# DecaYale/RNNPose

Hardware: AMD Instinct MI355X
Metric: pose-refine iters/sec (640x480, B=8, 3x8 recurrent) (higher is better)
Workload: dtype f32 (convolutions and volume build: fp16x3-split MFMA, fp32-class accuracy; LM: f64)

## Files before the change

include/rnnpose_hip.h:

```cpp
#ifndef RNNPOSE_HIP_H
#define RNNPOSE_HIP_H

#include <stddef.h>
#include <stdint.h>

#ifdef __cplusplus
extern "C" {
#endif

typedef void* rnnpose_stream_t;

#define RNNPOSE_ABI_VERSION 4
#define RNNPOSE_MAX_LEVELS 4

int rnnpose_abi_version(void);
const char* rnnpose_last_error(void);
int rnnpose_device_info(int dev, char* h_name, int name_len, int* h_cus);

int rnnpose_corr_pyramid_layout(int B, int h, int w, int levels, int64_t* h_offsets ,
                                int* h_hl , int* h_wl );
int rnnpose_corr_pyramid_f32(const float* fmap1, const float* fmap2, int B, int C, int h, int w,
                             int levels, float* pyramid, rnnpose_stream_t stream);
size_t rnnpose_corr_pyramid_f16x3_workspace_bytes(int B, int C, int h, int w);
int rnnpose_corr_pyramid_f16x3(const float* fmap1, const float* fmap2, int layout, int B, int C, int h, int w, int levels,
// ... 47 lines not shown
int rnnpose_lm_step_f32(const float* target, int target_mode, const float* weight, const float* depth,
                        float depth_eps, const float* K, float* G, int B, int H, int W, int num_iters,
                        double ep_lambda, double lm_lambda, double max_update, void* workspace,
                        size_t workspace_bytes, double* Hm, double* bv, float* xi, int* info,
                        rnnpose_stream_t stream);
int rnnpose_lm_step_io_f32(const float* target, int target_mode, const float* weight, const float* depth,
                           float depth_eps, const float* K, const float* G_in, float* G_out, int B, int H, int W,
                           int num_iters, double ep_lambda, double lm_lambda, double max_update, void* workspace,
                           size_t workspace_bytes, double* Hm, double* bv, float* xi, int* info,
                           rnnpose_stream_t stream);
int rnnpose_lm_normal_eq_rgbd_f64(const float* target, int target_mode, const float* weight, const float* depth,
                                  float depth_eps, const float* K, const float* G, int B, int H, int W,
                                  const float* obs_depth, const int* src_index, const float* theta, const float* K_obs,
                                  int S, int Ho, int Wo, float depth_weight, float depth_gate, float edge_tol,
                                  void* workspace, size_t workspace_bytes, double* Hm, double* bv, double* dstats,
                                  rnnpose_stream_t stream);
int rnnpose_lm_step_rgbd_io_f32(const float* target, int target_mode, const float* weight, const float* depth,
                                float depth_eps, const float* K, const float* G_in, float* G_out, int B, int H, int W,
                                int num_iters, double ep_lambda, double lm_lambda, double max_update,
                                const float* obs_depth, const int* src_index, const float* theta, const float* K_obs,
                                int S, int Ho, int Wo, float depth_weight, float depth_gate, float edge_tol,
                                void* workspace, size_t workspace_bytes, double* Hm, double* bv, float* xi, int* info,
                                double* dstats, rnnpose_stream_t stream);
int rnnpose_lm_step_views_io_f32(const float* target, int target_mode, const float* weight, const float* depth,
                                 float depth_eps, const float* K, const float* G_in, float* G_out, int B, int H, int W,
                                 int num_iters, double ep_lambda, double lm_lambda, double max_update,
                                 const float* obs_depth, const int* src_index, const float* theta, const float* K_obs,
                                 int S, int Ho, int Wo, float depth_weight, float depth_gate, float edge_tol,
                                 const int* group_start, int n_groups, const float* E,
                                 void* workspace, size_t workspace_bytes, double* Hm, double* bv, double* Hg, double* bg,
                                 float* xi, int* info, double* dstats, rnnpose_stream_t stream);
int rnnpose_lm_fused_tail(int enable);

int rnnpose_se3_exp_f32(const float* xi, int B, float* out, rnnpose_stream_t stream);
int rnnpose_se3_compose_f32(const float* A, const float* Bm, int B, float* out, rnnpose_stream_t stream);
int rnnpose_se3_inverse_f32(const float* A, int B, float* out, rnnpose_stream_t stream);
int rnnpose_se3_outer_update_f32(const float* Tij, const float* Ti, int B, int literal, float* Ti_out, float* Tij_out, rnnpose_stream_t stream);

int rnnpose_gru_gate_f32(const float* zr, const float* hcat, int B, int C, int Ctot, int hw, float* z_out,
                         float* rhx, rnnpose_stream_t stream);
int rnnpose_gru_update_f32(const float* z, const float* q_pre, const float* hcat, int B, int C, int Ctot_in,
                           int hw, float* hout, int Ctot_out, rnnpose_stream_t stream);

typedef struct {
  const float* ptr;
  int c_stride, c_offset, c_count;
} rnnpose_conv_src_t;

typedef struct {
  rnnpose_conv_src_t src[4];
  int n_src;
  int B, H, W;
  int kh, kw;
  int stride;
  const void* w_packed;
  const float* bias;
  int c_out;
  float a_scale, w_scale;
  int epilogue;
  float* dst;
  int dst_c_stride, dst_c_offset;
  const float* aux0;
  int aux0_c_stride, aux0_c_offset;
  const float* aux1;
  int aux1_c_stride, aux1_c_offset;
  float* dst2;
  int dst2_c_stride, dst2_c_offset;
  int gru_c;
  double* tile_stats;
  const float* add_map;
  int add_c_stride, add_c_offset;
  const float* src0_mean_rstd;
  int src_hl;
  int dst_hl;
  int dst2_hl;
  float* dst_split;
  int dst_split_c_stride, dst_split_c_offset;
  int src_bounded;
  int tile;
  void* ksplit_ws;
  size_t ksplit_ws_bytes;
  int single_product;
  int tile_stats_records;
} rnnpose_conv_desc_t;

size_t rnnpose_conv_ksplit_workspace_bytes(void);
int rnnpose_conv_ksplit(int enable);
int rnnpose_conv_ksplit_limits(int max_tiles, int max_splits);

int rnnpose_conv_tiles_per_image_desc(const rnnpose_conv_desc_t* h_desc);
int rnnpose_conv_products_desc(const rnnpose_conv_desc_t* h_desc);
int rnnpose_conv_spatial_tiles(int enable);
int rnnpose_conv_strip(int mode);
long long rnnpose_conv_packed_halfs(int c_out, int kh, int kw, const int* h_seg_counts, int n_seg);
int rnnpose_conv_pack_weights_f16x3(const float* w_oihw, int c_out, int c_in, int kh, int kw, const int* h_seg_counts,
                                    int n_seg, float w_scale, void* w_packed, rnnpose_stream_t stream);
int rnnpose_conv2d_nhwc_f16x3(const rnnpose_conv_desc_t* h_desc, rnnpose_stream_t stream);

int rnnpose_f16x3_saturation_check(int enable);
int rnnpose_f16x3_saturation_count(unsigned long long* h_count, int reset, rnnpose_stream_t stream);
int rnnpose_f16x3_saturation_peek(unsigned long long* d_count, rnnpose_stream_t stream);

long long rnnpose_stem_packed_halfs(void);
int rnnpose_stem_workgroups(int max_workgroups);
int rnnpose_stem_pack_weights_f16x3(const float* w_oihw, float w_scale, void* w_hi, void* w_lo, rnnpose_stream_t stream);
int rnnpose_stem_tiles(int H, int W, int* h_tiles_per_image, int* h_exact);
int rnnpose_stem_conv7x7_s2_f16x3(const float* img_nchw, int N, int H, int W, int normalize, const void* w_hi,
                                  const void* w_lo, const float* bias, float a_scale, float w_scale, float* out_nhwc,
                                  double* tile_stats, rnnpose_stream_t stream);

int rnnpose_corr_lookup_nhwc_f32(const float* pyramid, const float* coords, int B, int h, int w, int levels, int radius,
                                 float* out, rnnpose_stream_t stream);
int rnnpose_corr_lookup_nhwc_part_f32(const float* pyramid, const float* coords, int B, int b0, int b1, int h, int w,
                                      int levels, int radius, float* out, rnnpose_stream_t stream);
int rnnpose_corr_lookup_induced_nhwc_part_f32(const float* pyramid, const float* depth, const float* K, const float* G, int H, int W,
                                              float eps, int B, int b0, int b1, int h, int w, int levels, int radius, float* coords_out,
                                              float* out, rnnpose_stream_t stream);
int rnnpose_nchw_to_nhwc_f32(const float* src, int B, int C, int HW, float* dst, int dst_c_stride, int dst_c_offset,
                             rnnpose_stream_t stream);
int rnnpose_nhwc_to_nchw_f32(const float* src, int B, int C, int HW, int src_c_stride, int src_c_offset, float* dst,
                             rnnpose_stream_t stream);
int rnnpose_flow_prep_f32(const float* coords1, int subtract_grid, int B, int h, int w, float* flow4, float* motion,
                          int motion_c_stride, int motion_c_offset, rnnpose_stream_t stream);
int rnnpose_flow_conv7x7_relu_f32(const float* flow4, const float* w_t, const float* bias, int B, int h, int w, int c_out,
                                  float* out, int out_c_stride, int out_c_offset, rnnpose_stream_t stream);
int rnnpose_flow_features_f32(const float* coords1, int subtract_grid, const float* w_t, const float* bias, int B, int h, int w,
                              int c_out, float* out, int out_c_stride, int out_c_offset, float* motion, int motion_c_stride,
                              int motion_c_offset, int out_split, int motion_split, float a_scale, rnnpose_stream_t stream);
int rnnpose_flow_features_induced_f32(const float* depth, const float* K, const float* G, int H, int W, float eps, const float* w_t,
                                      const float* bias, int B, int h, int w, int c_out, float* out, int out_c_stride, int out_c_offset,
                                      float* motion, int motion_c_stride, int motion_c_offset, int out_split, int motion_split,
                                      float a_scale, rnnpose_stream_t stream);
int rnnpose_split_hl_f32(const float* src, int src_c_stride, int src_c_offset, long long n_pixels, int c_count, float a_scale,
                         float* dst, int dst_c_stride, int dst_c_offset, rnnpose_stream_t stream);
int rnnpose_flow_head_out_f32(const float* x, int x_c_stride, int x_c_offset, int c_in, const float* w_oihw,
                              const float* bias, const float* coords1, int B, int h, int w, float* delta,
                              float* coords1_out, float* flow_lr, rnnpose_stream_t stream);
int rnnpose_convex_upsample_nhwc_f32(const float* flow_lr, const float* mask, int B, int h, int w, float* flow_up,
                                     rnnpose_stream_t stream);
int rnnpose_maxpool2x2_nhwc_f32(const float* src, int B, int H, int W, int src_c_stride, int src_c_offset, int C, float* dst,
                                int dst_c_stride, int dst_c_offset, rnnpose_stream_t stream);
int rnnpose_upsample2x_bilinear_nhwc_f32(const float* src, int B, int h, int w, int src_c_stride, int src_c_offset, int C,
                                         const float* mean_rstd, int relu, float* dst, int dst_c_stride, int dst_c_offset,
                                         rnnpose_stream_t stream);
int rnnpose_pixel_head_nhwc_f32(const float* src, int B, int HW, int src_c_stride, int src_c_offset, int c_in,
                                const float* mean_rstd, int relu, const float* weight, const float* bias, int c_out, int mode,
                                float* dst_nchw, rnnpose_stream_t stream);
int rnnpose_point_row_sum_f32(const float* x, int n, int c, long long ldx, float* out, rnnpose_stream_t stream);
int rnnpose_kpconv_aggregate_f32(const float* q_pts, int n_q, const float* s_pts, int n_s, const int* neighbors, int width,
                                 const float* kernel_points, int K, float extent, const float* x, int c_in, long long ldx,
                                 const float* row_sum, float* wf, rnnpose_stream_t stream);
int rnnpose_point_linear_f32(const float* a, int n, int k, long long lda, const float* w, int m, const float* bias, float* out,
                             long long ldo, rnnpose_stream_t stream);
long long rnnpose_point_norm_workspace_bytes(int n, int c);
int rnnpose_point_norm_stats_f32(const float* x, int n, int c, long long ldx, float eps, void* workspace, long long workspace_bytes,
                                 float* mean_rstd, rnnpose_stream_t stream);
int rnnpose_point_norm_apply_f32(const float* x, int n, int c, long long ldx, const float* mean_rstd, const float* res, long long ldr,
                                 const float* res_mean_rstd, int leaky, float slope, float* out, long long ldo,
                                 rnnpose_stream_t stream);
int rnnpose_point_maxpool_f32(const float* x, int n_s, int c, long long ldx, const int* idx, int n_q, int width, float* out,
                              long long ldo, rnnpose_stream_t stream);
int rnnpose_point_gather_rows_f32(const float* x, int n_s, int c, long long ldx, const int* idx, int n_q, int idx_ld, float* out,
                                  long long ldo, rnnpose_stream_t stream);
int rnnpose_point_l2_normalize_f32(const float* x, int n, int c, long long ldx, float* out, long long ldo, rnnpose_stream_t stream);
int rnnpose_grid_voxel_keys_f32(const float* points, int n, float ox, float oy, float oz, float dl, long long nx, long long ny,
                                long long* keys, rnnpose_stream_t stream);
int rnnpose_radius_count_f32(const float* queries, int n_q, const float* supports, const int* q_start, const int* s_start,
                             int n_clouds, float radius, int* counts, rnnpose_stream_t stream);
int rnnpose_radius_neighbors_f32(const float* queries, int n_q, const float* supports, const int* q_start, const int* s_start,
                                 int n_clouds, float radius, const long long* offsets, int* cand_idx, float* cand_d2, int width,
                                 int* out, rnnpose_stream_t stream);
size_t rnnpose_conv1x1_resident_packed_bytes(int c_in);
int rnnpose_conv1x1_resident_pack_f16x3(const float* weight, int c_out, int c_in, float w_scale, void* packed,
                                        rnnpose_stream_t stream);
int rnnpose_conv1x1_resident_f16x3(const float* x, int x_c_stride, int x_c_offset, int c_in, const void* w_packed,
                                   const float* bias, float a_scale, float w_scale, int relu, long long n_pixels, float* dst,
                                   int dst_c_stride, int dst_c_offset, int dst_split, rnnpose_stream_t stream);
int rnnpose_corr_lookup_convc1_f16x3(const float* pyramid, const float* coords, int B, int b0, int b1, int h, int w, int levels,
                                     int radius, const void* w_packed, const float* bias, float a_scale, float w_scale, int relu,
                                     float* dst, int dst_c_stride, int dst_c_offset, int dst_split, rnnpose_stream_t stream);
size_t rnnpose_mask_upsample_packed_bytes(void);
int rnnpose_mask_upsample_pack_f16x3(const float* weight, float post_scale, float w_scale, void* packed, rnnpose_stream_t stream);
int rnnpose_mask_upsample_f16x3(const float* x, int x_c_stride, int x_c_offset, const void* w_packed, int c_out,
                                const float* bias, float a_scale, float w_scale, const float* flow_lr, int B, int h, int w,
                                float* flow_up, rnnpose_stream_t stream);

size_t rnnpose_instnorm_workspace_bytes(int B, int HW, int C);
int rnnpose_instnorm_nhwc_f32(const float* x, int B, int HW, int C, float eps, int relu, const float* residual,
                              void* workspace, size_t workspace_bytes, float* mean_rstd, float* out,
                              rnnpose_stream_t stream);
int rnnpose_instnorm_tiles_nhwc_f32(const float* x, int B, int HW, int C, float eps, int relu, const float* residual,
                                    const float* residual_mean_rstd, int residual_relu, const double* tile_stats,
                                    int tiles_per_image, float* mean_rstd, float* out,
                                    rnnpose_stream_t stream);

int rnnpose_nn_search_f32(const float* ref_pts, const float* que_pts, int* idxs, int b, int pn1, int pn2, int dim,
                          int exclude_self, rnnpose_stream_t stream);
void findNearestPointIdxLauncher(float* ref_pts, float* que_pts, int* idxs, int b, int pn1, int pn2, int dim,
                                 int exclude_self);

size_t rnnpose_pose_metrics_workspace_bytes(int B, int P);
int rnnpose_pose_metrics_f64(const float* model, int P, const float* pose_pred, const float* pose_gt, const float* K, int B,
                             int symmetric, void* workspace, size_t workspace_bytes, double* out, rnnpose_stream_t stream);

size_t rnnpose_bop_sym_dist_workspace_bytes(int B, int S);
int rnnpose_bop_sym_dist_f64(const float* model, int P, const float* sym, int S, const float* pose_est, const float* pose_gt,
                             const float* K, int B, void* workspace, size_t workspace_bytes, double* out, rnnpose_stream_t stream);
size_t rnnpose_bop_vsd_workspace_bytes(int B, int H, int W, int NT);
int rnnpose_bop_vsd_f64(const float* depth_est, const float* depth_gt, const float* depth_obs, int S_obs, const int* src_index,
                        const float* K, const float* diameter, int B, int H, int W, double delta, const double* taus, int NT,
                        void* workspace, size_t workspace_bytes, long long* counts, double* err, rnnpose_stream_t stream);

size_t rnnpose_pointcloud_depth_workspace_bytes(int B, int H, int W);
int rnnpose_pointcloud_depth_f32(const float* verts, const int* vert_offsets, int max_verts, const float* T, const float* K, int B,
                                 int H, int W, void* workspace, size_t workspace_bytes, float* out, rnnpose_stream_t stream);
int rnnpose_mask_bbox_f32(const float* depth, int B, int H, int W, int* bbox, rnnpose_stream_t stream);
int rnnpose_zoom_crop_params_f32(const int* bbox, const float* K, const float* T, int B, int H, int W, int crop_h, int crop_w,
                                 float margin_ratio, float* theta, float* K_crop, rnnpose_stream_t stream);
int rnnpose_zoom_crop_f32(const float* in, const float* theta, int B, int C, int H, int W, int crop_h, int crop_w, float* out,
                          float* grid_out, rnnpose_stream_t stream);
int rnnpose_zoom_crop_indexed_f32(const float* in, const int* src_index, const float* theta, int S, int B, int C, int H, int W,
                                  int crop_h, int crop_w, float* out, float* grid_out, rnnpose_stream_t stream);

size_t rnnpose_raster_workspace_bytes(int B, int H, int W);
int rnnpose_raster_mesh_f32(const float* verts, const int* faces, const int* vert_off, const int* face_off,
                            const int* face_cnt, int max_faces, const float* T, const float* K, int B, int H, int W,
                            float near, float pixel_center, int perspective_correct, void* workspace,
                            size_t workspace_bytes, rnnpose_stream_t stream);
int rnnpose_raster_resolve_f32(const float* verts, const int* faces, const int* vert_off, const int* face_off, const float* T,
                               const float* K, int B, int H, int W, float near, float pixel_center, int perspective_correct,
                               const void* workspace, const float* attr, const long long* attr_off, int C,
                               const float* colors, int with_color, int shade, float empty_depth, float* out_attr,
                               float* out_zbuf, float* out_vdepth, rnnpose_stream_t stream);
int rnnpose_raster_resolve_tex_f32(const float* verts, const int* faces, const int* vert_off, const int* face_off, const float* T,
                                   const float* K, int B, int H, int W, float near, float pixel_center, int perspective_correct,
                                   const void* workspace, const float* attr, const long long* attr_off, int C,
                                   const float* colors, const float* uvs, const int* face_uvs, const int* uv_off, const float* tex,
                                   const long long* tex_off, const int* tex_hw, const float* vnormals, int shade,
                                   float empty_depth, float* out_attr, float* out_zbuf, float* out_vdepth,
                                   rnnpose_stream_t stream);
int rnnpose_raster_occlusion_f32(const float* verts, const int* faces, const int* vert_off, const int* face_off,
                                 const int* face_cnt, int max_faces, const float* T, const float* K, int B, int H, int W,
                                 float near, float pixel_center, const int* pair_target, const int* pair_occluder, int P,
                                 float margin, const void* own_keys, void* workspace, size_t workspace_bytes, float* visible,
                                 int* occluder, float* depth_inout, rnnpose_stream_t stream);

#ifdef __cplusplus
}
#endif
#endif
```

rnnpose_amd/_lib.py:

```python
from __future__ import annotations

import ctypes as C
import os

_PKG = os.path.dirname(os.path.abspath(__file__))
ABI_VERSION = 4
LIB_PATH = os.environ.get("RNNPOSE_LIB") or os.path.join(_PKG, "lib", "librnnpose_hip.so")

_p = C.c_void_p
_i = C.c_int
_f = C.c_float
_d = C.c_double
_z = C.c_size_t
_ll = C.c_longlong

class ConvSrc(C.Structure):
    _fields_ = [("ptr", C.c_void_p), ("c_stride", C.c_int), ("c_offset", C.c_int), ("c_count", C.c_int)]


class ConvDesc(C.Structure):
    _fields_ = [("src", ConvSrc * 4), ("n_src", C.c_int), ("B", C.c_int), ("H", C.c_int), ("W", C.c_int),
                ("kh", C.c_int), ("kw", C.c_int), ("stride", C.c_int), ("w_packed", C.c_void_p), ("bias", C.c_void_p),
                ("c_out", C.c_int), ("a_scale", C.c_float), ("w_scale", C.c_float), ("epilogue", C.c_int),
                ("dst", C.c_void_p), ("dst_c_stride", C.c_int), ("dst_c_offset", C.c_int),
                ("aux0", C.c_void_p), ("aux0_c_stride", C.c_int), ("aux0_c_offset", C.c_int),
                ("aux1", C.c_void_p), ("aux1_c_stride", C.c_int), ("aux1_c_offset", C.c_int),
                ("dst2", C.c_void_p), ("dst2_c_stride", C.c_int), ("dst2_c_offset", C.c_int), ("gru_c", C.c_int),
                ("tile_stats", C.c_void_p), ("add_map", C.c_void_p), ("add_c_stride", C.c_int), ("add_c_offset", C.c_int),
                ("src0_mean_rstd", C.c_void_p), ("src_hl", C.c_int), ("dst_hl", C.c_int), ("dst2_hl", C.c_int),
                ("dst_split", C.c_void_p), ("dst_split_c_stride", C.c_int), ("dst_split_c_offset", C.c_int), ("src_bounded", C.c_int),
                ("tile", C.c_int), ("ksplit_ws", C.c_void_p), ("ksplit_ws_bytes", C.c_size_t), ("single_product", C.c_int),
                ("tile_stats_records", C.c_int)]


PROTOTYPES = {
    "rnnpose_abi_version": (_i, []),
    "rnnpose_last_error": (C.c_char_p, []),
    "rnnpose_device_info": (_i, [_i, C.c_char_p, _i, C.POINTER(_i)]),
    "rnnpose_corr_pyramid_layout": (_i, [_i, _i, _i, _i, C.POINTER(C.c_int64), C.POINTER(_i), C.POINTER(_i)]),
    "rnnpose_corr_pyramid_f32": (_i, [_p, _p, _i, _i, _i, _i, _i, _p, _p]),
    "rnnpose_corr_pyramid_f16x3_workspace_bytes": (_z, [_i, _i, _i, _i]),
    "rnnpose_corr_pyramid_f16x3": (_i, [_p, _p, _i, _i, _i, _i, _i, _i, _f, _p, _z, _p, _p]),
    "rnnpose_corr_pyramid_split": (_i, [_p, _p, _i, _i, _i, _i, _i, _f, _p, _p]),
    "rnnpose_corr_supertile": (_i, [_i]),
    "rnnpose_corr_variant": (_i, [_i]),
    "rnnpose_fmap_pyramid_floats": (_z, [_i, _i, _i, _i, _i]),
    "rnnpose_fmap_pyramid_f32": (_i, [_p, _i, _i, _i, _i, _i, _p, _p]),
    "rnnpose_corr_alt_lookup_f32": (_i, [_p, _p, _p, _p, _i, _i, _i, _i, _i, _i, _p, _i, _i, _p]),
    "rnnpose_corr_lookup_variant": (_i, [_i]),
    "rnnpose_corr_lookup_f32": (_i, [_p, _p, _i, _i, _i, _i, _i, _p, _p]),
    "rnnpose_context_prep_f32": (_i, [_p, _i, _i, _i, _i, _i, _i, _i, _p, _p, _p]),
    "rnnpose_flow_to_coords_f32": (_i, [_p, _i, _i, _i, _i, _i, _p, _p]),
    "rnnpose_convex_upsample_f32": (_i, [_p, _p, _i, _i, _i, _i, _p, _p]),
    "rnnpose_induced_flow_f32": (_i, [_p, _p, _p, _i, _i, _i, _f, _i, _p, _p, _p]),
    "rnnpose_induced_coords_lowres_f32": (_i, [_p, _p, _p, _i, _i, _i, _i, _i, _f, _p, _p]),
    "rnnpose_corr_weight_pairs": (_i, [_i]),
    "rnnpose_corr_weight_f32": (_i, [_p, _p, _p, _i, _p, _p, _i, _i, _i, _i, _p, _p]),
    "rnnpose_lm_workspace_bytes": (_z, [_i, _i, _i]),
    "rnnpose_lm_normal_eq_f64": (_i, [_p, _i, _p, _p, _f, _p, _p, _i, _i, _i, _p, _z, _p, _p, _p]),
    "rnnpose_lm_solve_update_f32": (_i, [_p, _p, _p, _i, _d, _d, _d, _p, _p, _p, _p]),
    "rnnpose_lm_step_f32": (_i, [_p, _i, _p, _p, _f, _p, _p, _i, _i, _i, _i, _d, _d, _d, _p, _z, _p, _p, _p, _p, _p]),
    "rnnpose_lm_step_io_f32": (_i, [_p, _i, _p, _p, _f, _p, _p, _p, _i, _i, _i, _i, _d, _d, _d, _p, _z, _p, _p, _p, _p, _p]),
    "rnnpose_lm_normal_eq_rgbd_f64": (_i, [_p, _i, _p, _p, _f, _p, _p, _i, _i, _i, _p, _p, _p, _p, _i, _i, _i, _f, _f, _f, _p, _z, _p, _p, _p, _p]),
    "rnnpose_lm_step_rgbd_io_f32": (_i, [_p, _i, _p, _p, _f, _p, _p, _p, _i, _i, _i, _i, _d, _d, _d, _p, _p, _p, _p, _i, _i, _i, _f, _f, _f,
                                         _p, _z, _p, _p, _p, _p, _p, _p]),
    "rnnpose_lm_step_views_io_f32": (_i, [_p, _i, _p, _p, _f, _p, _p, _p, _i, _i, _i, _i, _d, _d, _d, _p, _p, _p, _p, _i, _i, _i, _f, _f, _f,
                                          _p, _i, _p, _p, _z, _p, _p, _p, _p, _p, _p, _p, _p]),
    "rnnpose_lm_fused_tail": (_i, [_i]),
    "rnnpose_se3_exp_f32": (_i, [_p, _i, _p, _p]),
    "rnnpose_se3_compose_f32": (_i, [_p, _p, _i, _p, _p]),
    "rnnpose_se3_inverse_f32": (_i, [_p, _i, _p, _p]),
    "rnnpose_se3_outer_update_f32": (_i, [_p, _p, _i, _i, _p, _p, _p]),
    "rnnpose_gru_gate_f32": (_i, [_p, _p, _i, _i, _i, _i, _p, _p, _p]),
    "rnnpose_gru_update_f32": (_i, [_p, _p, _p, _i, _i, _i, _i, _p, _i, _p]),
    "rnnpose_conv_tiles_per_image_desc": (_i, [C.POINTER(ConvDesc)]),
    "rnnpose_conv_products_desc": (_i, [C.POINTER(ConvDesc)]),
    "rnnpose_conv_spatial_tiles": (_i, [_i]),
    "rnnpose_conv_strip": (_i, [_i]),
    "rnnpose_conv_ksplit": (_i, [_i]),
    "rnnpose_conv_ksplit_limits": (_i, [_i, _i]),
    "rnnpose_conv_ksplit_workspace_bytes": (_z, []),
    "rnnpose_conv_packed_halfs": (C.c_longlong, [_i, _i, _i, C.POINTER(_i), _i]),
    "rnnpose_conv_pack_weights_f16x3": (_i, [_p, _i, _i, _i, _i, C.POINTER(_i), _i, _f, _p, _p]),
    "rnnpose_conv2d_nhwc_f16x3": (_i, [C.POINTER(ConvDesc), _p]),
    "rnnpose_f16x3_saturation_check": (_i, [_i]),
    "rnnpose_f16x3_saturation_count": (_i, [C.POINTER(C.c_ulonglong), _i, _p]),
    "rnnpose_f16x3_saturation_peek": (_i, [_p, _p]),
    "rnnpose_stem_packed_halfs": (C.c_longlong, []),
    "rnnpose_stem_workgroups": (_i, [_i]),
    "rnnpose_stem_pack_weights_f16x3": (_i, [_p, _f, _p, _p, _p]),
    "rnnpose_stem_tiles": (_i, [_i, _i, C.POINTER(_i), C.POINTER(_i)]),
    "rnnpose_stem_conv7x7_s2_f16x3": (_i, [_p, _i, _i, _i, _i, _p, _p, _p, _f, _f, _p, _p, _p]),
    "rnnpose_corr_lookup_nhwc_f32": (_i, [_p, _p, _i, _i, _i, _i, _i, _p, _p]),
    "rnnpose_corr_lookup_nhwc_part_f32": (_i, [_p, _p, _i, _i, _i, _i, _i, _i, _i, _p, _p]),
    "rnnpose_nchw_to_nhwc_f32": (_i, [_p, _i, _i, _i, _p, _i, _i, _p]),
    "rnnpose_nhwc_to_nchw_f32": (_i, [_p, _i, _i, _i, _i, _i, _p, _p]),
    "rnnpose_flow_prep_f32": (_i, [_p, _i, _i, _i, _i, _p, _p, _i, _i, _p]),
    "rnnpose_flow_conv7x7_relu_f32": (_i, [_p, _p, _p, _i, _i, _i, _i, _p, _i, _i, _p]),
    "rnnpose_flow_features_f32": (_i, [_p, _i, _p, _p, _i, _i, _i, _i, _p, _i, _i, _p, _i, _i, _i, _i, _f, _p]),
    "rnnpose_flow_features_induced_f32": (_i, [_p, _p, _p, _i, _i, _f, _p, _p, _i, _i, _i, _i, _p, _i, _i, _p, _i, _i, _i, _i, _f, _p]),
    "rnnpose_corr_lookup_induced_nhwc_part_f32": (_i, [_p, _p, _p, _p, _i, _i, _f, _i, _i, _i, _i, _i, _i, _i, _p, _p, _p]),
    "rnnpose_split_hl_f32": (_i, [_p, _i, _i, _ll, _i, _f, _p, _i, _i, _p]),
    "rnnpose_maxpool2x2_nhwc_f32": (_i, [_p, _i, _i, _i, _i, _i, _i, _p, _i, _i, _p]),
    "rnnpose_upsample2x_bilinear_nhwc_f32": (_i, [_p, _i, _i, _i, _i, _i, _i, _p, _i, _p, _i, _i, _p]),
    "rnnpose_pixel_head_nhwc_f32": (_i, [_p, _i, _i, _i, _i, _i, _p, _i, _p, _p, _i, _i, _p, _p]),
    "rnnpose_point_row_sum_f32": (_i, [_p, _i, _i, _ll, _p, _p]),
    "rnnpose_kpconv_aggregate_f32": (_i, [_p, _i, _p, _i, _p, _i, _p, _i, _f, _p, _i, _ll, _p, _p, _p]),
    "rnnpose_point_linear_f32": (_i, [_p, _i, _i, _ll, _p, _i, _p, _p, _ll, _p]),
    "rnnpose_point_norm_workspace_bytes": (_ll, [_i, _i]),
    "rnnpose_point_norm_stats_f32": (_i, [_p, _i, _i, _ll, _f, _p, _ll, _p, _p]),
    "rnnpose_point_norm_apply_f32": (_i, [_p, _i, _i, _ll, _p, _p, _ll, _p, _i, _f, _p, _ll, _p]),
    "rnnpose_point_maxpool_f32": (_i, [_p, _i, _i, _ll, _p, _i, _i, _p, _ll, _p]),
    "rnnpose_point_gather_rows_f32": (_i, [_p, _i, _i, _ll, _p, _i, _i, _p, _ll, _p]),
    "rnnpose_point_l2_normalize_f32": (_i, [_p, _i, _i, _ll, _p, _ll, _p]),
    "rnnpose_grid_voxel_keys_f32": (_i, [_p, _i, _f, _f, _f, _f, _ll, _ll, _p, _p]),
    "rnnpose_radius_count_f32": (_i, [_p, _i, _p, _p, _p, _i, _f, _p, _p]),
    "rnnpose_radius_neighbors_f32": (_i, [_p, _i, _p, _p, _p, _i, _f, _p, _p, _p, _i, _p, _p]),
    "rnnpose_flow_head_out_f32": (_i, [_p, _i, _i, _i, _p, _p, _p, _i, _i, _i, _p, _p, _p, _p]),
    "rnnpose_convex_upsample_nhwc_f32": (_i, [_p, _p, _i, _i, _i, _p, _p]),
    "rnnpose_mask_upsample_f16x3": (_i, [_p, _i, _i, _p, _i, _p, _f, _f, _p, _i, _i, _i, _p, _p]),
    "rnnpose_mask_upsample_packed_bytes": (_z, []),
    "rnnpose_conv1x1_resident_packed_bytes": (_z, [_i]),
    "rnnpose_conv1x1_resident_pack_f16x3": (_i, [_p, _i, _i, _f, _p, _p]),
    "rnnpose_conv1x1_resident_f16x3": (_i, [_p, _i, _i, _i, _p, _p, _f, _f, _i, _ll, _p, _i, _i, _i, _p]),
    "rnnpose_corr_lookup_convc1_f16x3": (_i, [_p, _p, _i, _i, _i, _i, _i, _i, _i, _p, _p, _f, _f, _i, _p, _i, _i, _i, _p]),
    "rnnpose_mask_upsample_pack_f16x3": (_i, [_p, _f, _f, _p, _p]),
    "rnnpose_instnorm_workspace_bytes": (_z, [_i, _i, _i]),
    "rnnpose_instnorm_tiles_nhwc_f32": (_i, [_p, _i, _i, _i, _f, _i, _p, _p, _i, _p, _i, _p, _p, _p]),
    "rnnpose_instnorm_nhwc_f32": (_i, [_p, _i, _i, _i, _f, _i, _p, _p, _z, _p, _p, _p]),
    "rnnpose_nn_search_f32": (_i, [_p, _p, _p, _i, _i, _i, _i, _i, _p]),
    "findNearestPointIdxLauncher": (None, [_p, _p, _p, _i, _i, _i, _i, _i]),
    "rnnpose_pointcloud_depth_workspace_bytes": (_z, [_i, _i, _i]),
    "rnnpose_pointcloud_depth_f32": (_i, [_p, _p, _i, _p, _p, _i, _i, _i, _p, _z, _p, _p]),
    "rnnpose_mask_bbox_f32": (_i, [_p, _i, _i, _i, _p, _p]),
    "rnnpose_zoom_crop_params_f32": (_i, [_p, _p, _p, _i, _i, _i, _i, _i, _f, _p, _p, _p]),
    "rnnpose_zoom_crop_f32": (_i, [_p, _p, _i, _i, _i, _i, _i, _i, _p, _p, _p]),
    "rnnpose_zoom_crop_indexed_f32": (_i, [_p, _p, _p, _i, _i, _i, _i, _i, _i, _i, _p, _p, _p]),
    "rnnpose_raster_workspace_bytes": (_z, [_i, _i, _i]),
    "rnnpose_raster_mesh_f32": (_i, [_p, _p, _p, _p, _p, _i, _p, _p, _i, _i, _i, _f, _f, _i, _p, _z, _p]),
    "rnnpose_raster_resolve_f32": (_i, [_p, _p, _p, _p, _p, _p, _i, _i, _i, _f, _f, _i, _p, _p, _p, _i, _p, _i, _i, _f, _p, _p, _p, _p]),
    "rnnpose_raster_resolve_tex_f32": (_i, [_p, _p, _p, _p, _p, _p, _i, _i, _i, _f, _f, _i, _p, _p, _p, _i, _p, _p, _p, _p, _p, _p, _p, _p,
                                            _i, _f, _p, _p, _p, _p]),
    "rnnpose_raster_occlusion_f32": (_i, [_p, _p, _p, _p, _p, _i, _p, _p, _i, _i, _i, _f, _f, _p, _p, _i, _f, _p, _p, _z, _p, _p, _p, _p]),
    "rnnpose_pose_metrics_workspace_bytes": (_z, [_i, _i]),
    "rnnpose_pose_metrics_f64": (_i, [_p, _i, _p, _p, _p, _i, _i, _p, _z, _p, _p]),
    "rnnpose_bop_sym_dist_workspace_bytes": (_z, [_i, _i]),
    "rnnpose_bop_sym_dist_f64": (_i, [_p, _i, _p, _i, _p, _p, _p, _i, _p, _z, _p, _p]),
    "rnnpose_bop_vsd_workspace_bytes": (_z, [_i, _i, _i, _i]),
    "rnnpose_bop_vsd_f64": (_i, [_p, _p, _p, _i, _p, _p, _p, _i, _i, _i, _d, _p, _i, _p, _z, _p, _p, _p]),
}

_lib = None


def load() -> C.CDLL:
    global _lib
    if _lib is not None:
        return _lib
    if not os.path.exists(LIB_PATH):
        raise RuntimeError(
            f"{LIB_PATH} is missing: run `python -m rnnpose_amd.build` (hipcc, gfx950). "
            "rnnpose_amd has no CPU fallback for the refinement hot path.")
    import torch
    tl = os.path.join(os.path.dirname(torch.__file__), "lib", "libamdhip64.so")
    if os.path.exists(tl):
        C.CDLL(tl, mode=C.RTLD_GLOBAL)
    lib = C.CDLL(LIB_PATH)
    for name, (res, args) in PROTOTYPES.items():
        try:
            fn = getattr(lib, name)
        except AttributeError as e:
            raise RuntimeError(f"{LIB_PATH} does not export {name}; rebuild it") from e
        fn.restype = res
        fn.argtypes = args
    if lib.rnnpose_abi_version() != ABI_VERSION:
        raise RuntimeError("librnnpose_hip.so ABI version mismatch; rebuild it")
    _lib = lib
    return lib


def check(rc: int, name: str) -> None:
    if rc != 0:
        msg = load().rnnpose_last_error().decode(errors="replace")
        raise RuntimeError(f"{name} failed (code {rc}): {msg}")


def call(name: str, *args) -> None:
    check(getattr(load(), name)(*args), name)
```

rnnpose_amd/csrc/conv1x1_resident.hip:

```cpp
#include "resident_tile.cuh"

namespace {

using namespace rptile;
using rp::split4;

constexpr int MAX_NCB = 11;

struct RParams {
  const float* x;
  int cs, co, Cin;
  const uint4* wpk;
  TileOut out;
};

template <int NCB>
__global__ __launch_bounds__(8 * MQ) __attribute__((amdgpu_num_vgpr(160))) void conv1x1_resident_kernel(const RParams p) {
  constexpr int NCBL = NCB * 4096 >= MQ * RSF * 4 ? NCB : (MQ * RSF * 4 + 4095) / 4096;
  __shared__ __attribute__((aligned(16))) _Float16 sA[NCBL][2][MQ * 32];
  const int tid = threadIdx.x, lane = tid & 63, wave = tid >> 6;
  const long long m0 = static_cast<long long>(blockIdx.x) * MQ;

  const int c4 = tid & 7;
  float4 av[NCB];
  {
    const long long m = m0 + (tid >> 3);
    const long long mc = m < p.out.M ? m : p.out.M - 1;
    const float* src = p.x + mc * p.cs + p.co;
#pragma unroll
    for (int cb = 0; cb < NCB; ++cb) {
      const int c = cb * 32 + c4 * 4;
      av[cb] = *reinterpret_cast<const float4*>(src + (c < p.Cin ? c : 0));
    }
  }
  __builtin_amdgcn_sched_barrier(0);
  int sat_n = 0;
  const bool row_in = m0 + (tid >> 3) < p.out.M;
  {
    const int r = tid >> 3;
    const int chunk = (c4 >> 1) ^ (((r >> 2) & 1) << 1);
    const int off = r * 32 + chunk * 8 + (c4 & 1) * 4;
#pragma unroll
    for (int cb = 0; cb < NCB; ++cb) {
      const bool in = cb * 32 + c4 * 4 < p.Cin;
      const float4 v = in ? av[cb] : make_float4(0.f, 0.f, 0.f, 0.f);
      h4 hi, lo;
      split4(v, p.out.a_scale, hi, lo);
      if (p.out.sat && in && row_in) sat_n += rp::quad_saturates(v, p.out.a_scale) ? 1 : 0;
      *reinterpret_cast<h4*>(&sA[cb][0][off]) = hi;
      *reinterpret_cast<h4*>(&sA[cb][1][off]) = lo;
    }
  }
  if (p.out.sat && sat_n) atomicAdd(p.out.sat, static_cast<unsigned long long>(sat_n));
  __syncthreads();

  const int l15 = lane & 15, lq = lane >> 4;
  const int phys = lq ^ (((l15 >> 2) & 1) << 1);
  f32x4 acc[2][CT];
#pragma unroll
  for (int t = 0; t < 2; ++t)
#pragma unroll
    for (int j = 0; j < CT; ++j) acc[t][j] = f32x4{0.f, 0.f, 0.f, 0.f};
  uint4 bq[2][CT][2];
  load_weights(bq[0], p.wpk, 0, wave, lane);
  if (NCB > 1) load_weights(bq[1], p.wpk, 1, wave, lane);
  __builtin_amdgcn_sched_barrier(0);
#pragma unroll
  for (int cb = 0; cb < NCB; ++cb) {
    const int sl = cb & 1;
    block_step(acc, sA[cb][0], sA[cb][1], bq[sl], l15, phys);
    __builtin_amdgcn_sched_barrier(0);
    if (cb + 2 < NCB) load_weights(bq[sl], p.wpk, cb + 2, wave, lane);
    __builtin_amdgcn_sched_barrier(0);
  }

  __syncthreads();
  tile_epilogue(p.out, acc, reinterpret_cast<float*>(&sA[0][0][0]), m0, tid);
}

__global__ void resident_pack_kernel(const float* __restrict__ w, int Cin, int ncb, float scale, _Float16* __restrict__ pk) {
  const int i = blockIdx.x * blockDim.x + threadIdx.x;
  if (i >= ncb * 16 * 1024) return;
  const int j = i & 7, ln = (i >> 3) & 63, part = (i >> 9) & 1, ct = (i >> 10) & 15, cb = i >> 14;
  const int col = 16 * ct + (ln & 15), ch = cb * 32 + 8 * (ln >> 4) + j;
  const float v = ch < Cin ? w[col * Cin + ch] * scale : 0.f;
  const _Float16 h = static_cast<_Float16>(v);
  pk[i] = part == 0 ? h : static_cast<_Float16>(v - static_cast<float>(h));
}

}

extern "C" size_t rnnpose_conv1x1_resident_packed_bytes(int c_in) {
  if (c_in <= 0 || c_in > 32 * MAX_NCB) return 0;
  return static_cast<size_t>(rp::cdiv(c_in, 32)) * 16 * 1024 * sizeof(_Float16);
}

extern "C" int rnnpose_conv1x1_resident_pack_f16x3(const float* weight, int c_out, int c_in, float w_scale, void* packed,
                                                   rnnpose_stream_t stream) {
  const char* fn = "rnnpose_conv1x1_resident_pack_f16x3";
  RP_REQUIRE(weight && packed && reinterpret_cast<uintptr_t>(packed) % 16 == 0, fn, "null or misaligned pointer");
  RP_REQUIRE(c_out == 256 && c_in > 0 && c_in <= 32 * MAX_NCB && c_in % 4 == 0, fn, "needs c_out = 256 and c_in <= 352, c_in % 4 == 0");
  RP_REQUIRE(w_scale > 0.f, fn, "w_scale must be positive");
  const int ncb = rp::cdiv(c_in, 32), total = ncb * 16 * 1024;
  hipLaunchKernelGGL(resident_pack_kernel, dim3(rp::cdiv(total, 256)), dim3(256), 0, rp::as_stream(stream), weight, c_in, ncb, w_scale,
                     static_cast<_Float16*>(packed));
  return rp::check_launch(fn);
}

extern "C" int rnnpose_conv1x1_resident_f16x3(const float* x, int x_c_stride, int x_c_offset, int c_in, const void* w_packed,
                                              const float* bias, float a_scale, float w_scale, int relu, long long n_pixels,
                                              float* dst, int dst_c_stride, int dst_c_offset, int dst_split, rnnpose_stream_t stream) {
  const char* fn = "rnnpose_conv1x1_resident_f16x3";
  RP_REQUIRE(x && w_packed && bias && dst, fn, "null pointer");
  RP_REQUIRE(c_in > 0 && c_in <= 32 * MAX_NCB && c_in % 4 == 0, fn, "c_in must be a multiple of 4, at most 352");
  RP_REQUIRE(n_pixels > 0 && n_pixels < (1LL << 31), fn, "bad pixel count");
  RP_REQUIRE(x_c_offset >= 0 && x_c_offset % 4 == 0 && x_c_stride % 4 == 0 && x_c_offset + c_in <= x_c_stride, fn,
             "input channels must lie inside the row, 16-byte aligned");
  RP_REQUIRE(reinterpret_cast<uintptr_t>(x) % 16 == 0 && reinterpret_cast<uintptr_t>(w_packed) % 16 == 0, fn, "x / weights must be 16-byte aligned");
  if (int e = check_tile_out(fn, dst, dst_c_stride, dst_c_offset, dst_split, a_scale, w_scale)) return e;
  RParams p{};
  p.x = x; p.cs = x_c_stride; p.co = x_c_offset; p.Cin = c_in;
  p.wpk = static_cast<const uint4*>(w_packed);
  p.out = tile_out(bias, a_scale, w_scale, relu, dst, dst_c_stride, dst_c_offset, dst_split, n_pixels);
  const dim3 grid(static_cast<unsigned>(rp::cdiv(n_pixels, MQ))), block(8 * MQ);
  hipStream_t st = rp::as_stream(stream);
  switch (rp::cdiv(c_in, 32)) {
#define R_CASE(N_) case N_: hipLaunchKernelGGL(conv1x1_resident_kernel<N_>, grid, block, 0, st, p); break;
    R_CASE(1) R_CASE(2) R_CASE(3) R_CASE(4) R_CASE(5) R_CASE(6) R_CASE(7) R_CASE(8) R_CASE(9) R_CASE(10) R_CASE(11)
#undef R_CASE
    default: return rp::fail_arg(fn, "unsupported c_in");
  }
  return rp::check_launch(fn);
}
```

rnnpose_amd/csrc/conv_common.cuh:

```cuda
#pragma once
#include "common.hpp"
#include "f16x3.cuh"

namespace rpconv {

constexpr int BK = 32;
constexpr int MAX_CB = 24;

using rp::h8; using rp::h4; using rp::h2; using rp::f32x2; using rp::f32x16; using rp::u32x2; using rp::split4;

struct Seg {
  const float* ptr;
  int cstride, coff, ccount;
};

struct KParams {
  Seg seg0, seg1, seg2, seg3;
  int cb1, cb2, cb3;
  int ncb;
  int B, U, V, su, sv;
  int G, T, du0, dv0;
  int stride, Uin, Vin, gkw, dvg0;
  const uint4* wpk;
  int Npad;
  const float* bias;
  int Cout;
  float a_scale, out_scale;
  int epi;
  float* dst;
  int dst_cs, dst_co;
  const float* aux0;
  int aux0_cs, aux0_co;
  const float* aux1;
  int aux1_cs, aux1_co;
  float* dst2;
  int dst2_cs, dst2_co;
  int gru_c;
  double* tstats;
  const float* addm;
  int addm_cs, addm_co;
  int tpi;
  const float* in_mr;
  int n_mt, n_nt;
  unsigned long long* sat;
  int sp_tx, sp_ty;
  int dst_hl, dst2_hl;
  float* dsth;
  int dsth_cs, dsth_co;
  int ksplit;
  float* ks_ws;
  unsigned* ks_cnt;
  const uint4* wpk_strip;
  int single_product;
  int off32;
  int stagger;
  int n_tiles;
};

__device__ __forceinline__ void store_quad_hl(float* row, int ch, float y0, float y1, float y2, float y3, int nv, float a_scale,
                                              int& sat_n) {
  h4 hi, lo;
  const float4 v = make_float4(y0, nv > 1 ? y1 : 0.f, nv > 2 ? y2 : 0.f, nv > 3 ? y3 : 0.f);
  split4(v, a_scale, hi, lo);
  sat_n += rp::quad_saturates(v, a_scale) ? 1 : 0;
  float* ph = row + (ch & ~7) + ((ch >> 2) & 1) * 2;
  if (nv == 4) {
    *reinterpret_cast<h4*>(ph) = hi;
    *reinterpret_cast<h4*>(ph + 4) = lo;
  } else {
    _Float16* hh = reinterpret_cast<_Float16*>(ph);
    _Float16* ll = reinterpret_cast<_Float16*>(ph + 4);
    if (nv > 0) { hh[0] = hi.x; ll[0] = lo.x; }
    if (nv > 1) { hh[1] = hi.y; ll[1] = lo.y; }
    if (nv > 2) { hh[2] = hi.z; ll[2] = lo.z; }
  }
}

__device__ __forceinline__ float sigmoidf_(float v) { return 1.f / (1.f + expf(-v)); }

struct PackParams {
  int Cout, Cin, kh, kw, G, T, ncb, Npad, vertical;
  unsigned char cb_seg[MAX_CB];
  short cb_c0[MAX_CB];
  short seg_start[4];
  short seg_count[4];
  float w_scale;
};

struct ConvPolicy {
  bool spatial = true;
  bool strip = true;
  bool two_wave = true;
  int ni = 1;
  bool small = true;
  bool s2 = true;
  bool small32 = true;
  bool persist = false;
  bool ksplit = true;
  int ks_max_tiles = 24, ks_max_splits = 4;
};

struct ConvPlan {
  int rows;
  int ni, nw;
  bool spatial, wide, wide22, deep;
  int U, V, su, sv, G, T, du0, dv0, stride, Uin, Vin, gkw, dvg0;
  int Ho, Wo;
  bool per_image;
  int tiles_per_image;
  int sp_tx, sp_ty;
  int n_mt, n_nt;
  unsigned nwg;
  int products;
  bool persist;
  int ksplit;
};

int strip_waves(int c_out, int ni);
long long strip_s2_halfs(int c_in, int kh, int kw, int ncb, int Npad, int n_seg);
// ... 9 lines not shown
```

rnnpose_amd/csrc/conv_igemm.hip:

```cpp
#include "common.hpp"
#include "f16x3.cuh"
#include "conv_common.cuh"

#include <cstdlib>

namespace {

constexpr int BM = 128, BN = 128, NT = 256;
constexpr int HALO = 4;
constexpr int AROWS = BM + 2 * HALO;
constexpr int PROWS = AROWS + 1;
constexpr int RS = 40;

using namespace rpconv;


constexpr int SPR = 180, SPW = 18;
template <int NI, bool STRIDED, bool COLS4 = false, int TTS = 0, bool NORM = false, bool HLIN = false, bool DEEP = false,
          bool SPATIAL = false>
#ifndef RP_COLS4_WAVES
#define RP_COLS4_WAVES 2
#endif
#ifndef RP_SP_SINGLE
#define RP_SP_SINGLE 0
// ... 599 lines not shown
        double* t = TS + (wave * F4 + lane) * 8;
        t[0] = ts0; t[1] = ts1; t[2] = ts2; t[3] = ts3; t[4] = tq0; t[5] = tq1; t[6] = tq2; t[7] = tq3;
      }
      __syncthreads();
      if (wm == 0 && lane < F4) {
        const double* t0 = TS + (wave * F4 + lane) * 8;
        const double* t1 = TS + ((wave + 2) * F4 + lane) * 8;
        const int col = colw + lane * 4;
#pragma unroll
        for (int e = 0; e < 4; ++e)
          if (col + e < p.Cout) {
            double* o = p.tstats + (static_cast<long long>(mt_i) * p.Cout + col + e) * 2;
            o[0] = t0[e] + t1[e];
            o[1] = t0[4 + e] + t1[4 + e];
          }
      }
    }
  }
}

__global__ void pack_weights_kernel(const float* __restrict__ w, _Float16* __restrict__ pk, const PackParams q) {
  const long long total = static_cast<long long>(q.G) * q.T * q.ncb * q.Npad * BK * 2;
  const long long i = static_cast<long long>(blockIdx.x) * blockDim.x + threadIdx.x;
  if (i >= total) return;
  const int j8 = static_cast<int>(i % 8);
  const int ln = static_cast<int>((i / 8) % 64);
  const int part = static_cast<int>((i / 512) % 4);
  const int kk = part & 1;
  const int nt32 = q.Npad / 32;
  const int ntl = static_cast<int>((i / 2048) % nt32);
  const long long st = i / (2048LL * nt32);
  const int t = static_cast<int>(st % q.T);
  const int cb = static_cast<int>((st / q.T) % q.ncb);
  const int g = static_cast<int>(st / (static_cast<long long>(q.T) * q.ncb));
  const int k = kk * 16 + (ln >> 5) * 8 + j8;
  const int n = ntl * 32 + (ln & 31);
  const int s = q.cb_seg[cb];
  const int cl = q.cb_c0[cb] + k;
  float v = 0.f;
  if (n < q.Cout && cl < q.seg_count[s]) {
    const int ci = q.seg_start[s] + cl;
    const int ky = q.vertical ? t : g, kx = q.vertical ? 0 : t;
    v = w[((static_cast<long long>(n) * q.Cin + ci) * q.kh + ky) * q.kw + kx] * q.w_scale;
  }
  const _Float16 h = static_cast<_Float16>(v);
  pk[i] = part < 2 ? h : static_cast<_Float16>(v - static_cast<float>(h));
}

int fill_cb_tables(const int* counts, int n, unsigned char* cb_seg, short* cb_c0) {
  int ncb = 0;
  for (int s = 0; s < n; ++s)
    for (int c = 0; c < counts[s]; c += BK) {
      if (ncb >= MAX_CB) return -1;
      cb_seg[ncb] = static_cast<unsigned char>(s);
      cb_c0[ncb] = static_cast<short>(c);
      ++ncb;
    }
  return ncb;
}

}

using namespace rpconv;

static ConvPolicy g_policy;
constexpr int KS_MAX_WG = 192;
constexpr size_t KS_CNT_BYTES = 1024;

extern "C" {

static bool plan_conv(const rnnpose_conv_desc_t* d, const ConvPolicy& pol, ConvPlan* out) {
  ConvPlan& pl = *out;
  pl = ConvPlan{};
  if (!d || d->H <= 0 || d->W <= 0 || (d->stride != 1 && d->stride != 2) || d->c_out <= 0 || d->B < 1 || d->n_src < 1 || d->n_src > 4) return false;
  const bool tile_ok = d->tile >= 0 && d->tile <= 7;
  const bool k33 = d->kh == 3 && d->kw == 3, k11 = d->kh == 1 && d->kw == 1, vertical = d->kw == 1 && d->kh > 1;
  const bool norm = d->src0_mean_rstd != nullptr, hlin = d->src_hl != 0;
  const int H = d->H, W = d->W, Npad = rp::cdiv(d->c_out, BN) * BN;
  int ncb = 0;
  for (int s = 0; s < d->n_src; ++s) ncb += rp::cdiv(d->src[s].c_count, BK);
  pl.stride = d->stride;
  pl.Ho = d->stride == 2 ? (H + 1) / 2 : H; pl.Wo = d->stride == 2 ? (W + 1) / 2 : W;
  pl.products = 3; pl.ksplit = 1;
  if (tile_ok && (d->tile >= 5 || (d->tile == 0 && pol.strip))) {
    const bool s2_ok = d->n_src == 1 && d->src[0].c_count % 32 == 0 && !hlin && !norm && 4 * (d->src[0].c_count / 32) <= MAX_CB && (k33 || k11);
    if (d->stride == 1 || s2_ok)
      pl.rows = strip_rows(pol, H, W, d->kh, d->kw, d->stride, d->c_out, d->B, d->tile == 5 ? 160 : d->tile == 6 ? 32 : d->tile == 7 ? 96 : 0);
    if (d->tile == 0) {
      for (int s = 0; s < d->n_src; ++s)
        if (d->src[s].c_count % 32 != 0) pl.rows = 0;
      if (norm && !k33) pl.rows = 0;
    }
  }
  if (pl.rows) {
    const int cfg = strip_waves(d->c_out, pol.ni);
    pl.ni = cfg >> 4; pl.nw = cfg & 15;
    pl.spatial = k33 || d->stride == 2;
    if (d->stride == 2) {
      pl.U = pl.Ho; pl.V = pl.Wo; pl.su = 2 * W; pl.sv = 2; pl.Uin = H; pl.Vin = W;
      pl.G = 1; pl.T = 4; pl.du0 = 0; pl.dv0 = 0; pl.gkw = d->kw; pl.dvg0 = -(d->kw / 2);
    } else if (vertical) {
      pl.U = pl.Uin = W; pl.V = pl.Vin = H; pl.su = 1; pl.sv = W;
      pl.G = 1; pl.T = d->kh; pl.du0 = 0; pl.dv0 = -(d->kh / 2);
    } else {
      pl.U = pl.Uin = H; pl.V = pl.Vin = W; pl.su = W; pl.sv = 1;
      pl.G = d->kh; pl.T = k33 ? 9 : d->kw; pl.du0 = -(d->kh / 2); pl.dv0 = k33 ? 0 : -(d->kw / 2);
    }
    pl.per_image = pl.spatial || d->tile_stats || norm;
    if (pl.spatial) {
      pl.sp_tx = rp::cdiv(pl.Wo, 16); pl.sp_ty = rp::cdiv(pl.Ho, pl.rows / 16);
      pl.tiles_per_image = pl.sp_tx * pl.sp_ty;
    } else {
      pl.tiles_per_image = rp::cdiv(static_cast<long long>(H) * W, pl.rows);
    }
    pl.n_mt = pl.per_image ? d->B * pl.tiles_per_image : rp::cdiv(static_cast<long long>(d->B) * H * W, pl.rows);
    pl.n_nt = rp::cdiv(d->c_out, 32 * pl.ni * pl.nw);
    pl.nwg = static_cast<unsigned>(pl.n_mt) * pl.n_nt;
    if (d->single_product && pl.rows == 160 && pl.ni == 1 && d->stride == 1) pl.products = 1;
    pl.persist = pol.persist && !hlin && pl.ni == 1 && pl.spatial && d->stride == 1 && pl.rows == 160 && !d->single_product;
    return true;
  }
  pl.spatial = pol.spatial && k33 && d->stride == 1;
  if (d->stride == 2) {
    pl.U = pl.Ho; pl.V = pl.Wo; pl.su = W; pl.sv = 1; pl.Uin = H; pl.Vin = W;
    pl.G = d->kh * d->kw; pl.T = 1; pl.du0 = -(d->kh / 2); pl.dv0 = 0; pl.gkw = d->kw; pl.dvg0 = -(d->kw / 2);
  } else if (vertical) {
    pl.U = pl.Uin = W; pl.V = pl.Vin = H; pl.su = 1; pl.sv = W;
    pl.G = 1; pl.T = d->kh; pl.du0 = 0; pl.dv0 = -(d->kh / 2);
  } else {
    pl.U = pl.Uin = H; pl.V = pl.Vin = W; pl.su = W; pl.sv = 1;
    pl.G = pl.spatial ? 1 : d->kh; pl.T = pl.spatial ? 9 : d->kw; pl.du0 = pl.spatial ? 0 : -(d->kh / 2); pl.dv0 = pl.spatial ? 0 : -(d->kw / 2);
  }
  pl.per_image = pl.spatial || d->tile_stats || norm;
  if (pl.spatial) {
    pl.sp_tx = rp::cdiv(W, 16); pl.sp_ty = rp::cdiv(H, 8);
    pl.tiles_per_image = pl.sp_tx * pl.sp_ty;
  } else {
    pl.tiles_per_image = rp::cdiv(static_cast<long long>(pl.Ho) * pl.Wo, BM);
  }
  pl.n_mt = pl.per_image ? d->B * pl.tiles_per_image : rp::cdiv(static_cast<long long>(d->B) * pl.Ho * pl.Wo, BM);
  pl.wide22 = d->tile == 3 && hlin && !pl.spatial;
  pl.deep = d->tile == 4 && hlin && !pl.spatial && (pl.T == 3 || pl.T == 5);
  if (pl.spatial) pl.wide = d->tile == 2 && d->c_out % 128 == 0 && !norm;
  else if (d->tile == 2) pl.wide = !norm;
  else pl.wide = d->tile != 1 && d->tile != 4 && !pl.wide22 && !norm && (d->c_out % 128 == 0) && (static_cast<long long>(pl.n_mt) * (d->c_out / 128) >= 512);
  pl.n_nt = pl.wide || pl.wide22 ? Npad / 128 : rp::cdiv(d->c_out, 64);
  const int tiles = pl.n_mt * pl.n_nt, nit = pl.G * ncb;
  if (!pl.wide && !pl.wide22 && !pl.deep && d->stride == 1 && pol.ksplit && d->ksplit_ws && tiles <= pol.ks_max_tiles && nit >= 4) {
    int ksn = pol.ks_max_splits;
    if (ksn > nit / 2) ksn = nit / 2;
    if (ksn * tiles > KS_MAX_WG) ksn = KS_MAX_WG / tiles;
    const size_t need = KS_CNT_BYTES + static_cast<size_t>(tiles) * ksn * (NT * 32) * sizeof(float);
    if (ksn >= 2 && d->ksplit_ws_bytes >= need && reinterpret_cast<uintptr_t>(d->ksplit_ws) % 16 == 0) pl.ksplit = ksn;
  }
  pl.nwg = static_cast<unsigned>(pl.n_mt) * pl.n_nt * pl.ksplit;
  return tile_ok && d->tile < 5;
}

int rnnpose_conv_spatial_tiles(int enable) {
  g_policy.spatial = enable != 0;
  return 0;
}

int rnnpose_conv_strip(int mode) {
  if (mode < 0 || mode > 7) {
    rp::set_error("rnnpose_conv_strip: mode 0..7");
    return 1;
  }
  static const struct { bool strip, two_wave; int ni; bool small, s2, small32, persist; } modes[8] = {
      {false, true, 1, true, true, true, false},
      {true, true, 1, true, true, true, false},
      {true, false, 1, true, true, true, false},
      {true, true, 2, true, true, true, false},
      {true, true, 1, false, true, true, false},
      {true, true, 1, true, false, true, false},
      {true, true, 1, true, true, false, false},
      {true, true, 1, true, true, true, true}};
  const auto& m = modes[mode];
  g_policy.strip = m.strip; g_policy.two_wave = m.two_wave; g_policy.ni = m.ni; g_policy.small = m.small;
  g_policy.s2 = m.s2; g_policy.small32 = m.small32; g_policy.persist = m.persist;
  return 0;
}

int rnnpose_conv_ksplit(int enable) {
  g_policy.ksplit = enable != 0;
  return 0;
}

int rnnpose_conv_ksplit_limits(int max_tiles, int max_splits) {
  if (max_tiles < 1 || max_tiles > 96 || max_splits < 2 || max_splits > 8) {
    rp::set_error("rnnpose_conv_ksplit_limits: max_tiles 1..96, max_splits 2..8");
    return 1;
  }
  g_policy.ks_max_tiles = max_tiles; g_policy.ks_max_splits = max_splits;
  return 0;
}

size_t rnnpose_conv_ksplit_workspace_bytes(void) {
  return KS_CNT_BYTES + static_cast<size_t>(KS_MAX_WG) * (NT * 32) * sizeof(float);
}

int rnnpose_conv_tiles_per_image_desc(const rnnpose_conv_desc_t* d) {
  ConvPlan pl;
  return plan_conv(d, g_policy, &pl) ? pl.tiles_per_image : -1;
}

int rnnpose_conv_products_desc(const rnnpose_conv_desc_t* d) {
  ConvPlan pl;
  return plan_conv(d, g_policy, &pl) ? pl.products : -1;
}

long long rnnpose_conv_packed_halfs(int c_out, int kh, int kw, const int* h_seg_counts, int n_seg) {
  if (c_out <= 0 || kh <= 0 || kw <= 0 || !h_seg_counts || n_seg < 1 || n_seg > 4) return -1;
  unsigned char cs[MAX_CB];
  short c0[MAX_CB];
  const int ncb = fill_cb_tables(h_seg_counts, n_seg, cs, c0);
  if (ncb < 0) return -1;
  const long long Npad = static_cast<long long>(rp::cdiv(c_out, BN)) * BN;
  return 2 * static_cast<long long>(kh) * kw * ncb * Npad * BK * 2 + strip_s2_halfs(h_seg_counts[0], kh, kw, ncb, static_cast<int>(Npad), n_seg);
}

int rnnpose_conv_pack_weights_f16x3(const float* w_oihw, int c_out, int c_in, int kh, int kw, const int* h_seg_counts,
                                    int n_seg, float w_scale, void* w_packed, rnnpose_stream_t stream) {
  const char* fn = "rnnpose_conv_pack_weights_f16x3";
  RP_REQUIRE(w_oihw && w_packed && h_seg_counts, fn, "null pointer");
  RP_REQUIRE(n_seg >= 1 && n_seg <= 4, fn, "1..4 source segments");
  RP_REQUIRE((kh & 1) && (kw & 1) && kh <= 7 && kw <= 7, fn, "odd kernel sizes up to 7");
  PackParams q{};
  int tot = 0;
  for (int s = 0; s < n_seg; ++s) {
    RP_REQUIRE(h_seg_counts[s] > 0 && h_seg_counts[s] % 4 == 0, fn, "segment channel counts must be positive multiples of 4");
    q.seg_start[s] = static_cast<short>(tot);
    q.seg_count[s] = static_cast<short>(h_seg_counts[s]);
    tot += h_seg_counts[s];
  }
  RP_REQUIRE(tot == c_in, fn, "segment channel counts must sum to c_in");
  q.ncb = fill_cb_tables(h_seg_counts, n_seg, q.cb_seg, q.cb_c0);
  RP_REQUIRE(q.ncb > 0, fn, "too many channel blocks");
  q.Cout = c_out; q.Cin = c_in; q.kh = kh; q.kw = kw;
  q.vertical = (kw == 1 && kh > 1) ? 1 : 0;
  q.G = q.vertical ? 1 : kh;
  q.T = q.vertical ? kh : kw;
  q.Npad = rp::cdiv(c_out, BN) * BN;
  q.w_scale = w_scale;
  const long long total = static_cast<long long>(q.G) * q.T * q.ncb * q.Npad * BK * 2;
  hipLaunchKernelGGL(pack_weights_kernel, dim3(rp::cdiv(total, 256)), dim3(256), 0, rp::as_stream(stream), w_oihw,
                     static_cast<_Float16*>(w_packed), q);
  strip_pack(w_oihw, static_cast<_Float16*>(w_packed) + total, q, rp::as_stream(stream));
  return rp::check_launch(fn);
}

int rnnpose_conv2d_nhwc_f16x3(const rnnpose_conv_desc_t* d, rnnpose_stream_t stream) {
  const char* fn = "rnnpose_conv2d_nhwc_f16x3";
  RP_REQUIRE(d, fn, "null descriptor");
  RP_REQUIRE(d->n_src >= 1 && d->n_src <= 4, fn, "1..4 sources");
  RP_REQUIRE(d->B > 0 && d->H > 0 && d->W > 0 && d->c_out > 0, fn, "bad size");
  RP_REQUIRE((d->kh & 1) && (d->kw & 1) && d->kh <= 7 && d->kw <= 7, fn, "odd kernel sizes up to 7");
  RP_REQUIRE(d->w_packed && d->bias && d->dst, fn, "null pointer");
  RP_REQUIRE(reinterpret_cast<uintptr_t>(d->w_packed) % 16 == 0, fn, "packed weights must be 16-byte aligned");
  RP_REQUIRE(d->epilogue >= 0 && d->epilogue <= 3, fn, "epilogue must be 0..3");
  RP_REQUIRE(d->stride == 1 || d->stride == 2, fn, "stride must be 1 or 2");
  RP_REQUIRE(d->a_scale > 0.f && d->w_scale > 0.f, fn, "scales must be positive");
  if (d->epilogue == 2) RP_REQUIRE(d->aux0 && d->dst2 && d->gru_c > 0 && d->c_out == 2 * d->gru_c, fn, "gru_zr needs aux0 (h), dst2 (r*h), c_out == 2*gru_c");
  if (d->epilogue == 3) RP_REQUIRE(d->aux0 && d->aux1, fn, "gru_q needs aux0 (h) and aux1 (z)");
  RP_REQUIRE(d->dst_c_stride % 4 == 0 && d->dst_c_offset % 4 == 0 && reinterpret_cast<uintptr_t>(d->dst) % 16 == 0, fn,
             "dst: 16-byte aligned, channel stride/offset multiples of 4");
  if (d->epilogue >= 2) {
    RP_REQUIRE(d->c_out % 4 == 0 && d->gru_c % 4 == 0, fn, "GRU epilogues need c_out % 4 == 0");
    RP_REQUIRE(d->aux0_c_stride % 4 == 0 && d->aux0_c_offset % 4 == 0 && reinterpret_cast<uintptr_t>(d->aux0) % 16 == 0, fn,
               "aux0: 16-byte aligned, channel stride/offset multiples of 4");
  }
  if (d->epilogue == 2) RP_REQUIRE(d->dst2_c_stride % 4 == 0 && d->dst2_c_offset % 4 == 0 && reinterpret_cast<uintptr_t>(d->dst2) % 16 == 0, fn, "dst2 alignment");
  if (d->epilogue == 3) RP_REQUIRE(d->aux1_c_stride % 4 == 0 && d->aux1_c_offset % 4 == 0 && reinterpret_cast<uintptr_t>(d->aux1) % 16 == 0, fn, "aux1 alignment");
  KParams p{};
  int counts[4];
  for (int s = 0; s < d->n_src; ++s) {
    const rnnpose_conv_src_t& sr = d->src[s];
    RP_REQUIRE(sr.ptr && sr.c_count > 0 && sr.c_count % 4 == 0 && sr.c_stride % 4 == 0 && sr.c_offset % 4 == 0 &&
                   sr.c_offset + sr.c_count <= sr.c_stride && reinterpret_cast<uintptr_t>(sr.ptr) % 16 == 0,
               fn, "source: 16-byte aligned pointer, channel stride/offset/count multiples of 4");
    RP_REQUIRE(static_cast<long long>(d->B) * d->H * d->W * sr.c_stride < (1LL << 31), fn,
               "source tensor too large for 32-bit element offsets (B*H*W*c_stride must be < 2^31)");
    const Seg sg{sr.ptr, sr.c_stride, sr.c_offset, sr.c_count};
    (s == 0 ? p.seg0 : s == 1 ? p.seg1 : s == 2 ? p.seg2 : p.seg3) = sg;
    counts[s] = sr.c_count;
  }
  {
    unsigned char cs[MAX_CB];
    short c0[MAX_CB];
    p.ncb = fill_cb_tables(counts, d->n_src, cs, c0);
    RP_REQUIRE(p.ncb > 0, fn, "too many channel blocks");
    int st[5] = {0, p.ncb, p.ncb, p.ncb, p.ncb};
    for (int s = 1; s < d->n_src; ++s) st[s] = st[s - 1] + rp::cdiv(counts[s - 1], BK);
    p.cb1 = st[1]; p.cb2 = st[2]; p.cb3 = st[3];
  }
  ConvPlan pl;
  const bool planned = plan_conv(d, g_policy, &pl);
  const bool hlin = d->src_hl != 0;
  RP_REQUIRE(pl.spatial || (pl.T / 2 <= HALO && (pl.stride == 2 || pl.T == 1 || pl.T == 3 || pl.T == 5 || pl.T == 7)), fn, "kernel too wide for the staged halo");
  if (d->add_map) RP_REQUIRE(d->c_out % 4 == 0 && d->add_c_stride % 4 == 0 && d->add_c_offset % 4 == 0 &&
                                 reinterpret_cast<uintptr_t>(d->add_map) % 16 == 0, fn, "add_map: c_out % 4 == 0, 16-byte aligned, stride/offset multiples of 4");
  if (hlin) {
    RP_REQUIRE(d->stride == 1 && !d->src0_mean_rstd && (pl.T == 1 || pl.T == 3 || pl.T == 5 || pl.spatial), fn,
               "split-tensor sources: stride 1, 1/3/5 taps per group, no fused normalisation");
    for (int s = 0; s < d->n_src; ++s)
      RP_REQUIRE(d->src[s].c_count % 8 == 0 && d->src[s].c_offset % 8 == 0 && d->src[s].c_stride % 8 == 0 &&
                     reinterpret_cast<uintptr_t>(d->src[s].ptr) % 32 == 0, fn,
                 "split-tensor source: channel stride/offset/count multiples of 8, 32-byte aligned");
  }
  if (d->dst_hl) RP_REQUIRE(d->dst_c_stride % 8 == 0 && reinterpret_cast<uintptr_t>(d->dst) % 32 == 0 && !d->tile_stats, fn,
                            "split-form dst: channel stride multiple of 8, 32-byte aligned, no tile statistics");
  if (d->dst2_hl) RP_REQUIRE(d->epilogue == 2 && d->dst2_c_stride % 8 == 0 && reinterpret_cast<uintptr_t>(d->dst2) % 32 == 0, fn,
                             "split-form dst2: GRU z|r epilogue, channel stride multiple of 8, 32-byte aligned");
  if (d->dst_split) RP_REQUIRE(d->epilogue != 2 && d->dst_split_c_stride % 8 == 0 && d->dst_split_c_offset % 4 == 0 &&
                                   reinterpret_cast<uintptr_t>(d->dst_split) % 32 == 0, fn,
                               "dst_split: not with the GRU z|r epilogue; channel stride multiple of 8, offset of 4, 32-byte aligned");
  RP_REQUIRE(d->tile >= 0 && d->tile <= 7, fn, "tile must be 0 (auto), 1 (128x64), 2 (128x128, 4 column waves), 3 (128x128, 2x2 waves), 4 (128x64, deep pipeline), 5 / 6 / 7 (strips of 160 / 32 / 96 rows)");
  if (d->tile_stats) RP_REQUIRE(d->epilogue == 0, fn, "tile_stats needs the linear epilogue");
  RP_REQUIRE(static_cast<long long>(d->B) * pl.Ho * pl.Wo < (1LL << 31) - 256 && static_cast<long long>(d->B) * d->H * d->W < (1LL << 31) - 256, fn, "too many pixels");
  if (d->tile_stats)
    RP_REQUIRE(planned && static_cast<long long>(d->tile_stats_records) == static_cast<long long>(d->B) * pl.tiles_per_image, fn,
               "tile_stats_records must equal B * rnnpose_conv_tiles_per_image_desc(desc) (a consumer derives the tiling from the record count: "
               "an oversized buffer would make it sum records this launch never writes): size the statistics buffer with that call");
  if (d->tile >= 5) RP_REQUIRE(planned, fn, "strip kernels: stride 1, 3x3 / 1x5 / 5x1, c_out > 32 (32-row strips: one column tile per wave)");
  p.B = d->B;
  p.U = pl.U; p.V = pl.V; p.su = pl.su; p.sv = pl.sv;
  p.G = pl.G; p.T = pl.T; p.du0 = pl.du0; p.dv0 = pl.dv0;
  p.stride = pl.stride; p.Uin = pl.Uin; p.Vin = pl.Vin; p.gkw = pl.gkw; p.dvg0 = pl.dvg0;
  p.tpi = pl.per_image ? pl.tiles_per_image : 0;
  p.n_mt = pl.n_mt; p.n_nt = pl.n_nt; p.sp_tx = pl.sp_tx; p.sp_ty = pl.sp_ty;
  p.wpk = static_cast<const uint4*>(d->w_packed);
  p.Npad = rp::cdiv(d->c_out, BN) * BN;
  p.bias = d->bias; p.Cout = d->c_out;
  p.a_scale = d->a_scale;
  p.out_scale = 1.0f / (d->a_scale * d->w_scale);
  p.epi = d->epilogue;
  p.dst = d->dst; p.dst_cs = d->dst_c_stride; p.dst_co = d->dst_c_offset;
  p.aux0 = d->aux0; p.aux0_cs = d->aux0_c_stride; p.aux0_co = d->aux0_c_offset;
  p.aux1 = d->aux1; p.aux1_cs = d->aux1_c_stride; p.aux1_co = d->aux1_c_offset;
  p.dst2 = d->dst2; p.dst2_cs = d->dst2_c_stride; p.dst2_co = d->dst2_c_offset;
  p.gru_c = d->gru_c;
  p.tstats = d->tile_stats;
  p.in_mr = d->src0_mean_rstd;
  p.addm = d->add_map; p.addm_cs = d->add_c_stride; p.addm_co = d->add_c_offset;
  p.sat = d->src_bounded ? nullptr : rp::sat_counter();
  p.dst_hl = d->dst_hl; p.dst2_hl = d->dst2_hl;
  p.dsth = d->dst_split; p.dsth_cs = d->dst_split_c_stride; p.dsth_co = d->dst_split_c_offset;
  p.single_product = d->single_product != 0;
  p.ksplit = pl.ksplit; p.ks_ws = nullptr; p.ks_cnt = nullptr;
  if (pl.ksplit > 1) {
    p.ks_cnt = static_cast<unsigned*>(d->ksplit_ws);
    p.ks_ws = reinterpret_cast<float*>(static_cast<char*>(d->ksplit_ws) + KS_CNT_BYTES);
  }
  const long long first = static_cast<long long>(d->kh) * d->kw * p.ncb * p.Npad * BK * 2;
  p.wpk_strip = reinterpret_cast<const uint4*>(static_cast<const _Float16*>(d->w_packed) + first);
  if (pl.rows) {
    if (d->stride == 2 && d->kh == 3) {
      const rnnpose_conv_src_t& sr = d->src[0];
      const int nb = sr.c_count / BK;
      for (int k = 0; k < 4; ++k) {
        const Seg sg{sr.ptr + (static_cast<long long>(k >> 1) * d->W + (k & 1)) * sr.c_stride, sr.c_stride, sr.c_offset, sr.c_count};
        (k == 0 ? p.seg0 : k == 1 ? p.seg1 : k == 2 ? p.seg2 : p.seg3) = sg;
      }
      p.cb1 = nb; p.cb2 = 2 * nb; p.cb3 = 3 * nb; p.ncb = 4 * nb;
      p.wpk_strip = reinterpret_cast<const uint4*>(reinterpret_cast<const _Float16*>(p.wpk_strip) + static_cast<long long>(nb) * 2 * 9 * p.Npad * 32);
    }
    return strip_launch(p, pl, d->kh, d->kw, hlin, rp::as_stream(stream));
  }
  if (d->src0_mean_rstd)
    RP_REQUIRE(d->n_src == 1 && d->stride == 1 && d->kh == 3 && d->kw == 3 && reinterpret_cast<uintptr_t>(d->src0_mean_rstd) % 16 == 0,
               fn, "src0_mean_rstd (fused instance norm + ReLU of the input) needs one source, a 3x3 stride-1 kernel, 16-byte alignment");
  const dim3 block(NT), grid(pl.nwg);
  hipStream_t st = rp::as_stream(stream);
#define RP_LAUNCH_T(NI_, COLS4_, HL_)                                                                                   \
  switch (p.T) {                                                                                                         \
    case 1: hipLaunchKernelGGL((conv_igemm_f16x3_kernel<NI_, false, COLS4_, 1, false, HL_>), grid, block, 0, st, p); break;    \
    case 3: hipLaunchKernelGGL((conv_igemm_f16x3_kernel<NI_, false, COLS4_, 3, false, HL_>), grid, block, 0, st, p); break;    \
    case 5: hipLaunchKernelGGL((conv_igemm_f16x3_kernel<NI_, false, COLS4_, 5, false, HL_>), grid, block, 0, st, p); break;    \
    default:                                                                                                             \
      if constexpr (!(HL_)) hipLaunchKernelGGL((conv_igemm_f16x3_kernel<NI_, false, COLS4_, 7, false, false>), grid, block, 0, st, p); \
      break;                                                                                                             \
  }
  if (pl.spatial) {
    if (pl.wide) {
      if (hlin) hipLaunchKernelGGL((conv_igemm_f16x3_kernel<1, false, true, 9, false, true, false, true>), grid, block, 0, st, p);
      else hipLaunchKernelGGL((conv_igemm_f16x3_kernel<1, false, true, 9, false, false, false, true>), grid, block, 0, st, p);
    } else {
      if (d->src0_mean_rstd && p.sat) hipLaunchKernelGGL((conv_igemm_f16x3_kernel<1, false, false, -9, true, false, false, true>), grid, block, 0, st, p);
      else if (d->src0_mean_rstd) hipLaunchKernelGGL((conv_igemm_f16x3_kernel<1, false, false, 9, true, false, false, true>), grid, block, 0, st, p);
      else if (hlin) hipLaunchKernelGGL((conv_igemm_f16x3_kernel<1, false, false, 9, false, true, false, true>), grid, block, 0, st, p);
      else hipLaunchKernelGGL((conv_igemm_f16x3_kernel<1, false, false, 9, false, false, false, true>), grid, block, 0, st, p);
    }
  } else if (pl.deep) {
    if (p.T == 3) hipLaunchKernelGGL((conv_igemm_f16x3_kernel<1, false, false, 3, false, true, true>), grid, block, 0, st, p);
    else hipLaunchKernelGGL((conv_igemm_f16x3_kernel<1, false, false, 5, false, true, true>), grid, block, 0, st, p);
  } else if (pl.wide22) {
    RP_LAUNCH_T(2, false, true)
  } else if (pl.wide) {
    if (p.stride == 2) {
      hipLaunchKernelGGL((conv_igemm_f16x3_kernel<1, true, true>), grid, block, 0, st, p);
    } else if (hlin) {
      RP_LAUNCH_T(1, true, true)
    } else {
      RP_LAUNCH_T(1, true, false)
    }
  } else {
    if (p.stride == 2) {
      hipLaunchKernelGGL((conv_igemm_f16x3_kernel<1, true, false>), grid, block, 0, st, p);
    } else if (d->src0_mean_rstd && p.sat) {
      hipLaunchKernelGGL((conv_igemm_f16x3_kernel<1, false, false, -3, true>), grid, block, 0, st, p);
    } else if (d->src0_mean_rstd) {
      hipLaunchKernelGGL((conv_igemm_f16x3_kernel<1, false, false, 3, true>), grid, block, 0, st, p);
    } else if (hlin) {
      RP_LAUNCH_T(1, false, true)
    } else {
      RP_LAUNCH_T(1, false, false)
    }
  }
#undef RP_LAUNCH_T
  return rp::check_launch(fn);
}

}
```

rnnpose_amd/csrc/conv_strip_kernel.cuh:

```cuda
#pragma once
#include "common.hpp"
#include "f16x3.cuh"
#include "conv_common.cuh"

namespace {

using namespace rpconv;

constexpr int SHALO = 4;
constexpr int SPW = 16;
constexpr int SHW = SPW + 2;

__device__ __attribute__((aligned(64))) const unsigned char g_zero_page[64] = {0};

__device__ __forceinline__ void glds16(const void* g, unsigned dst) {
  unsigned keep;
  asm volatile(
      "s_mov_b32 %0, m0\n\t"
      "s_mov_b32 m0, %2\n\t"
      "s_nop 0\n\t"
      "global_load_lds_dwordx4 %1, off\n\t"
      "s_mov_b32 m0, %0"
      : "=&s"(keep)
      : "v"(g), "s"(dst)
// ... 157 lines not shown
    if constexpr (EV == 1) {
      ts0 += static_cast<double>((y[0].x + y[1].x) + (y[2].x + y[3].x));
      ts1 += static_cast<double>((y[0].y + y[1].y) + (y[2].y + y[3].y));
      ts2 += static_cast<double>((y[0].z + y[1].z) + (y[2].z + y[3].z));
      ts3 += static_cast<double>((y[0].w + y[1].w) + (y[2].w + y[3].w));
      tq0 += static_cast<double>(fmaf(y[0].x, y[0].x, y[1].x * y[1].x) + fmaf(y[2].x, y[2].x, y[3].x * y[3].x));
      tq1 += static_cast<double>(fmaf(y[0].y, y[0].y, y[1].y * y[1].y) + fmaf(y[2].y, y[2].y, y[3].y * y[3].y));
      tq2 += static_cast<double>(fmaf(y[0].z, y[0].z, y[1].z * y[1].z) + fmaf(y[2].z, y[2].z, y[3].z * y[3].z));
      tq3 += static_cast<double>(fmaf(y[0].w, y[0].w, y[1].w * y[1].w) + fmaf(y[2].w, y[2].w, y[3].w * y[3].w));
    }
    if constexpr (EV <= 2) {
#pragma unroll
      for (int k = 0; k < 4; ++k) y[k] = make_float4(fmaxf(y[k].x, lo_), fmaxf(y[k].y, lo_), fmaxf(y[k].z, lo_), fmaxf(y[k].w, lo_));
    } else if constexpr (EV == 3) {
      if (zside) {
#pragma unroll
        for (int k = 0; k < 4; ++k) y[k] = make_float4(fast_sigmoid(y[k].x), fast_sigmoid(y[k].y), fast_sigmoid(y[k].z), fast_sigmoid(y[k].w));
      } else {
#pragma unroll
        for (int k = 0; k < 4; ++k)
          y[k] = make_float4(fast_sigmoid(y[k].x) * hv[k].x, fast_sigmoid(y[k].y) * hv[k].y, fast_sigmoid(y[k].z) * hv[k].z, fast_sigmoid(y[k].w) * hv[k].w);
      }
    } else {
#pragma unroll
      for (int k = 0; k < 4; ++k) {
        const float4 z = zv[k], h = hv[k];
        y[k] = make_float4((1.f - z.x) * h.x + z.x * fast_tanh(y[k].x), (1.f - z.y) * h.y + z.y * fast_tanh(y[k].y),
                           (1.f - z.z) * h.z + z.z * fast_tanh(y[k].z), (1.f - z.w) * h.w + z.w * fast_tanh(y[k].w));
      }
    }
    if (mi + 1 < NBLK) {
#pragma unroll
      for (int k = 0; k < 4; ++k) pixn[k] = pixel(mi + 1, k);
      request(pixn);
    }
    if constexpr (EV == 0 || EV == 1 || EV == 4) {
#pragma unroll
      for (int k = 0; k < 4; ++k) *reinterpret_cast<float4*>(p.dst + eoff(pix[k], p.dst_cs, p.dst_co + colq)) = y[k];
    }
    if constexpr (EV == 2) {
#pragma unroll
      for (int k = 0; k < 4; ++k) store_quad_hl(p.dst + eoff(pix[k], p.dst_cs, 0), p.dst_co + colq, y[k].x, y[k].y, y[k].z, y[k].w, 4, p.a_scale, sat_n);
    }
    if constexpr (EV == 3) {
      if (zside) {
#pragma unroll
        for (int k = 0; k < 4; ++k) *reinterpret_cast<float4*>(p.dst + eoff(pix[k], p.dst_cs, p.dst_co + colq)) = y[k];
      } else {
#pragma unroll
        for (int k = 0; k < 4; ++k) store_quad_hl(p.dst2 + eoff(pix[k], p.dst2_cs, 0), p.dst2_co + c2, y[k].x, y[k].y, y[k].z, y[k].w, 4, p.a_scale, sat_n);
      }
    }
    if constexpr (EV == 4) {
#pragma unroll
      for (int k = 0; k < 4; ++k) store_quad_hl(p.dsth + eoff(pix[k], p.dsth_cs, 0), p.dsth_co + colq, y[k].x, y[k].y, y[k].z, y[k].w, 4, p.a_scale, sat_n);
    }
#pragma unroll
    for (int k = 0; k < 4; ++k) pix[k] = pixn[k];
  }
}

#ifndef RS_MINW3
#define RS_MINW3 0
#endif
template <int NW, int TT, int MODE, int NI, int SMI, bool P1 = false, bool PERSIST = false>
__global__ __launch_bounds__(NW * 64, NI == 2 ? 1 : ((RS_MINW3 && NW == 2 && SMI == 3 && TT == 9) ? 3 : 2)) void conv_strip_f16x3_kernel(const KParams p) {
  constexpr bool SPATIAL = TT == 9 || TT == 4;
  constexpr bool S2 = TT == 4;
  constexpr int SM = 32 * SMI;
  constexpr int SPH = 2 * SMI;
  constexpr int SHR = (SPH + 2) * SHW;
  constexpr int BREC = 2048 * NI;
  constexpr bool RING3 = RS_RING3 && TT == 9 && NW == 2 && NI == 1 && (SMI == 5 || (RS_MINW3 && SMI == 3));
  constexpr int NBST = SPATIAL ? (RING3 ? 3 : (S2 ? 4 : 6)) : 5;
  static_assert((2 * TT) % NBST == 0 && NBST - 2 < TT - 1, "ring period");
  constexpr int NT_ = NW * 64;
  constexpr int ARV = SPATIAL ? SHR : SM + 2 * SHALO;
  constexpr int AR = (ARV + 31) / 32 * 32;
  constexpr int PLANE = AR * 32;
  constexpr int ASLOT = 2 * PLANE;
  constexpr int NPP = AR / 32, NPIECE = 2 * NPP;
  constexpr int PA = (NPIECE + NW - 1) / NW;
  constexpr int NQ = (ARV * 4 + NT_ - 1) / NT_;
  constexpr int PAW = MODE == 0 ? PA : (MODE == 1 ? NQ : NQ + 2);
  constexpr int ZROW = ARV * 32;
  constexpr int BOFF = 2 * ASLOT;
  constexpr int LDSB = BOFF + NW * NBST * BREC;
  static_assert(PAW + 2 * NI * (NBST - 3) <= 63, "vmcnt is a 6-bit counter");
  static_assert(ZROW + 32 <= PLANE, "a zero row behind the data rows");
  __shared__ __attribute__((aligned(1024))) unsigned char lds[LDSB];

  const int tid = threadIdx.x, lane = tid & 63;
  const int wave = __builtin_amdgcn_readfirstlane(tid >> 6);
  const int l31 = lane & 31, lh = lane >> 5;
  RS_CLK(0)

  const int t_ntl = PERSIST ? p.n_tiles : static_cast<int>(gridDim.x);
  const int t_per = t_ntl >> 3, t_rem = t_ntl & 7, t_xcd = static_cast<int>(blockIdx.x) & 7;
  const int t_base = t_xcd * t_per + (t_xcd < t_rem ? t_xcd : t_rem), t_cnt = t_per + (t_xcd < t_rem ? 1 : 0);
  const int t_step = PERSIST ? static_cast<int>(gridDim.x) >> 3 : 0x40000000;
  int t_idx = static_cast<int>(blockIdx.x) >> 3;
  if constexpr (PERSIST) {
    if (p.stagger > 0) {
      const unsigned long long t_end = wall_clock64() + static_cast<unsigned long long>(((static_cast<int>(blockIdx.x) >> 3) >> 5) * p.stagger);
      while (wall_clock64() < t_end) __builtin_amdgcn_s_sleep(32);
    }
  }
  const int UV = p.U * p.V;
  const int Mtot = p.B * UV;
  int nt_i, mt_i, img_, py0_, px0_, m0, mend, ct32;
  int e_mt_i, e_img, e_py0, e_px0, e_m0, e_mend, e_ct32;
#define RS_TILE_GEOM(BID_)                                                                                   \
  {                                                                                                          \
    const int bid_ = (BID_);                                                                                 \
    nt_i = bid_ % p.n_nt; mt_i = bid_ / p.n_nt;                                                              \
    img_ = p.tpi > 0 ? mt_i / p.tpi : 0;                                                                     \
    const int pt_ = p.tpi > 0 ? mt_i - img_ * p.tpi : 0;                                                     \
    py0_ = SPATIAL ? (pt_ / p.sp_tx) * SPH : 0; px0_ = SPATIAL ? (pt_ % p.sp_tx) * SPW : 0;                  \
    m0 = p.tpi > 0 ? img_ * UV + pt_ * SM : mt_i * SM;                                                       \
    mend = p.tpi > 0 ? (img_ + 1) * UV : Mtot;                                                               \
    ct32 = (nt_i * NW + wave) * NI;                                    \
  }
  RS_TILE_GEOM(t_base + t_idx)
  const int ntiles32 = p.Npad >> 5;
  unsigned char* const sB = lds + BOFF + wave * (NBST * BREC);
  const unsigned lds0 = static_cast<unsigned>(reinterpret_cast<size_t>((__attribute__((address_space(3))) unsigned char*)lds));
  const unsigned sB0 = lds0 + BOFF + wave * (NBST * BREC);

#define RS_ROW_PIXEL(OUT_, J_)                                                                               \
  {                                                                                                          \
    const int j_ = (J_);                                                                                     \
    if (SPATIAL) {                                                                                           \
      const int hy_ = j_ / SHW, y_ = py0_ - 1 + hy_, x_ = px0_ - 1 + (j_ - hy_ * SHW);                       \
      const bool ok_ = j_ < SHR && static_cast<unsigned>(y_) < static_cast<unsigned>(p.U) &&                 \
                       static_cast<unsigned>(x_) < static_cast<unsigned>(p.V);                               \
      OUT_ = ok_ ? img_ * (p.Uin * p.Vin) + y_ * p.su + x_ * p.sv : -1;     \
    } else {                                                                                                 \
      const int m_ = m0 - SHALO + j_;                                                                        \
      const bool ok_ = j_ < ARV && m_ >= 0 && m_ < Mtot;                                                     \
      const int mm_ = ok_ ? m_ : 0;                                                                          \
      const int q_ = mm_ / p.V, v_ = mm_ - q_ * p.V;                                                         \
      const int b_ = q_ / p.U, u_ = q_ - b_ * p.U;                                                           \
      OUT_ = ok_ ? b_ * UV + u_ * p.su + v_ * p.sv : -1;                                                     \
    }                                                                                                        \
  }
#define RS_SWZ(J_) (SPATIAL ? (((J_) / SHW) & 1) : (((J_) >> 3) & 1))
  int apix[PA > NQ ? PA : NQ];
  int asrc[MODE == 0 ? PA : 1];
#define RS_TILE_ROWS()                                                                                       \
  {                                                                                                          \
    if constexpr (MODE == 0) {                                                                               \
      _Pragma("unroll") for (int i = 0; i < PA; ++i) {                                                       \
        const int q = wave + NW * i < NPIECE ? wave + NW * i : NPIECE - 1;       \
        const int plane = q / NPP, j = (q - plane * NPP) * 32 + (lane >> 1);                                 \
        RS_ROW_PIXEL(apix[i], j)                                                                             \
        asrc[i] = (((lane & 1) ^ RS_SWZ(j)) << 5) + (plane << 4);                                            \
      }                                                                                                      \
    } else {         \
      _Pragma("unroll") for (int i = 0; i < NQ; ++i) {                                                       \
        const int idx = tid + NT_ * i;                                                                       \
        RS_ROW_PIXEL(apix[i], idx >> 2)                                                                      \
      }                                                                                                      \
    }                                                                                                        \
  }
  RS_TILE_ROWS()
  int aad[SMI][SPATIAL ? 2 : TT];
#define RS_TILE_FRAG_ADDR()      \
  {                                                                                                          \
    _Pragma("unroll") for (int mi = 0; mi < SMI; ++mi) {                                                     \
      const int r = mi * 32 + l31;                                                                           \
      if constexpr (SPATIAL) {                                                                               \
        const int hyc = (r >> 4) + 1, xc = (r & 15) + 1;                                                     \
        aad[mi][0] = ((hyc - 1) * SHW + xc - 1) * 32 + ((lh ^ ((hyc - 1) & 1)) << 4);                        \
        aad[mi][1] = (hyc * SHW + xc - 1) * 32 + ((lh ^ (hyc & 1)) << 4);                                    \
      } else {                                                                                               \
        const int m = m0 + r;                                                                                \
        const int fv = m < mend ? m % p.V : -1000;                                 \
        _Pragma("unroll") for (int t = 0; t < TT; ++t) {                                                     \
          const int dv = p.dv0 + t, row = r + SHALO + dv;                                                    \
          const bool ok = static_cast<unsigned>(fv + dv) < static_cast<unsigned>(p.V);                       \
          aad[mi][t] = ok ? row * 32 + ((lh ^ ((row >> 3) & 1)) << 4) : ZROW + (lh << 4);                    \
        }                                                                                                    \
      }                                                                                                      \
    }                                                                                                        \
  }
  RS_TILE_FRAG_ADDR()
  const int boff = l31 * 32 + ((lh ^ ((l31 >> 3) & 1)) << 4);
  const unsigned lane16 = lane * 16;

  f32x16 acc[SMI][NI];

  const int NHB = 2 * p.ncb;
  const int S = NHB * TT;
  float4 areg[MODE == 0 ? 1 : NQ];
  float4 nrm01 = make_float4(0.f, 1.f, 0.f, 1.f), nrm23 = nrm01;
  int sat_n = 0;
  bool sat_here = MODE != 0 && p.sat != nullptr && nt_i == 0;

  int a_next = 0;
  int a_seg_end = 0;
  const unsigned char* asp[MODE == 0 ? PA : NQ];
  unsigned ainc[MODE == 0 ? PA : NQ];
  const float* nsp = p.in_mr;
#define RS_A_REBUILD()                                                                                       \
  {                                                                                                          \
    Seg sg_ = p.seg0;                                                                                        \
    int cb0_ = 0, cbe_ = p.cb1;                                                                              \
    const int blk_ = a_next >> 1;                                                                            \
    if (blk_ >= p.cb1) { sg_ = p.seg1; cb0_ = p.cb1; cbe_ = p.cb2; }                                         \
    if (blk_ >= p.cb2) { sg_ = p.seg2; cb0_ = p.cb2; cbe_ = p.cb3; }                                         \
    if (blk_ >= p.cb3) { sg_ = p.seg3; cb0_ = p.cb3; cbe_ = p.ncb; }                                         \
    a_seg_end = 2 * (cbe_ < p.ncb ? cbe_ : p.ncb);                                                           \
    const int cl_ = (blk_ - cb0_) * BK + (a_next & 1) * 16 + (MODE == 0 ? 0 : (tid & 3) * 4);                \
    const unsigned char* sb_ = reinterpret_cast<const unsigned char*>(sg_.ptr + sg_.coff + cl_);            \
    _Pragma("unroll") for (int i = 0; i < (MODE == 0 ? PA : NQ); ++i) {                                      \
      const bool ok_ = apix[i] >= 0;                                                                         \
      const unsigned eo_ = static_cast<unsigned>(apix[i]) * static_cast<unsigned>(sg_.cstride);              \
      if (MODE == 0) asp[i] = ok_ ? sb_ + (static_cast<size_t>(eo_) * 4 + asrc[i]) : g_zero_page + ((lane & 3) << 4); \
      else asp[i] = ok_ ? sb_ + static_cast<size_t>(eo_) * 4 : g_zero_page;                                  \
      ainc[i] = ok_ ? 64u : 0u;                                                                              \
    }                                                                                                        \
    if (MODE == 2) nsp = p.in_mr + (static_cast<long long>(img_) * sg_.cstride + sg_.coff + cl_) * 2;        \
  }
#define RS_A_ADVANCE()                                                                                       \
  {                                                                                                          \
    if (a_next + 1 < NHB) {                                                                                  \
      ++a_next;                                                                                              \
      if (a_next == a_seg_end) {                                                                             \
        RS_A_REBUILD()                                                                                       \
      } else {                                                                                               \
        _Pragma("unroll") for (int i = 0; i < (MODE == 0 ? PA : NQ); ++i) asp[i] += ainc[i];                 \
        if (MODE == 2) nsp += 32;                                                                            \
      }                                                                                                      \
    }                                                                                                        \
  }
#define RS_ISSUE_A(SLOT_)                                                                                    \
  {                                                                                                          \
    _Pragma("unroll") for (int i = 0; i < PA; ++i) {                                                         \
      const int q_ = wave + NW * i < NPIECE ? wave + NW * i : NPIECE - 1;                                    \
      glds16(asp[i], __builtin_amdgcn_readfirstlane(lds0 + (SLOT_) * ASLOT + q_ * 1024));                    \
    }                                                                                                        \
    RS_A_ADVANCE()                                                                                           \
  }
#define RS_LOAD_A()                                                                                          \
  {                                                                                                          \
    if (MODE == 2) {                                                                                         \
      nrm01 = *reinterpret_cast<const float4*>(nsp);                                                         \
      nrm23 = *reinterpret_cast<const float4*>(nsp + 4);                                                     \
    }                                                                                                        \
    _Pragma("unroll") for (int i = 0; i < NQ; ++i) areg[i] = *reinterpret_cast<const float4*>(asp[i]);       \
    RS_A_ADVANCE()                                                                                           \
  }
#define RS_STORE_A(SLOT_)                                                                                    \
  {                                                                                                          \
    _Pragma("unroll") for (int i = 0; i < NQ; ++i) {                                                         \
      const int idx_ = tid + NT_ * i, row_ = idx_ >> 2, quad_ = idx_ & 3;                                    \
      if (row_ < ARV) {                                                                                      \
        float4 xv_ = areg[i];                                                                                \
        if (MODE == 2) xv_ = make_float4(fmaxf((xv_.x - nrm01.x) * nrm01.y, 0.f), fmaxf((xv_.y - nrm01.z) * nrm01.w, 0.f), \
                                         fmaxf((xv_.z - nrm23.x) * nrm23.y, 0.f), fmaxf((xv_.w - nrm23.z) * nrm23.w, 0.f)); \
        const bool in_ = apix[i] >= 0;                                                                       \
        if (sat_here) sat_n += (in_ && rp::quad_saturates(xv_, p.a_scale)) ? 1 : 0;                          \
        h4 hi_, lo_;                                                                                         \
        split4(in_ ? xv_ : make_float4(0.f, 0.f, 0.f, 0.f), p.a_scale, hi_, lo_);                            \
        const int ad_ = (SLOT_) * ASLOT + row_ * 32 + (((quad_ >> 1) ^ RS_SWZ(row_)) << 4) + (quad_ & 1) * 8; \
        *reinterpret_cast<h4*>(lds + ad_) = hi_;                                                             \
        *reinterpret_cast<h4*>(lds + ad_ + PLANE) = lo_;                                                     \
      }                                                                                                      \
    }                                                                                                        \
  }
  const unsigned char* wptr;
  const size_t wstep = static_cast<size_t>(ntiles32) * 2048;
  int b_left;
#define RS_ISSUE_B(SL_)                                                                                      \
  {                                                                                                          \
    glds_rec<NI>(wptr, lane16, __builtin_amdgcn_readfirstlane(sB0 + (SL_) * BREC));                          \
    if (b_left > 0) { wptr += wstep; --b_left; }                                                             \
  }
  h8 fa_h[2][SMI], fa_l[2][SMI], fb_h[2][NI], fb_l[2][NI];
  constexpr int NRD = P1 ? NI + SMI : 2 * NI + 2 * SMI;
  constexpr int NMM = (P1 ? 1 : 3) * SMI * NI;
#define RS_READ1(K_, SET_, TN_, AS_, BS_)                                                                    \
  {                                                                                                          \
    if ((K_) < NI) fb_h[SET_][(K_)] = *reinterpret_cast<const h8*>(sB + (BS_) * BREC + (K_) * 2048 + boff);  \
    else if (P1) {                                  \
      const int mi_ = (K_) - NI;                                                                             \
      const int tn9_ = S2 ? ((TN_) >> 1) * 3 + ((TN_) & 1) : (TN_);      \
      const int dyq_ = tn9_ / 3;                                                                             \
      const int ad_ = SPATIAL ? aad[mi_][dyq_ == 1 ? 1 : 0] + (dyq_ == 2 ? 2 * SHW * 32 : 0) + (tn9_ - 3 * dyq_) * 32 \
                              : aad[mi_][SPATIAL ? 0 : (TN_)];                                               \
      fa_h[SET_][mi_] = *reinterpret_cast<const h8*>(lds + (AS_) * ASLOT + ad_);                             \
    }                                                                                                        \
    else if ((K_) >= NI + SMI && (K_) < 2 * NI + SMI)                                                        \
      fb_l[SET_][(K_) - NI - SMI] = *reinterpret_cast<const h8*>(sB + (BS_) * BREC + ((K_) - NI - SMI) * 2048 + 1024 + boff); \
    else {                                                                                                   \
      const bool lo_ = (K_) < NI + SMI;                                                                      \
      const int mi_ = lo_ ? (K_) - NI : (K_) - 2 * NI - SMI;                                                 \
      const int tn9_ = S2 ? ((TN_) >> 1) * 3 + ((TN_) & 1) : (TN_);                                          \
      const int dyq_ = tn9_ / 3;                                                                             \
      const int ad_ = SPATIAL ? aad[mi_][dyq_ == 1 ? 1 : 0] + (dyq_ == 2 ? 2 * SHW * 32 : 0) + (tn9_ - 3 * dyq_) * 32 \
                              : aad[mi_][SPATIAL ? 0 : (TN_)];                                               \
      if (lo_) fa_l[SET_][mi_] = *reinterpret_cast<const h8*>(lds + (AS_) * ASLOT + PLANE + ad_);            \
      else fa_h[SET_][mi_] = *reinterpret_cast<const h8*>(lds + (AS_) * ASLOT + ad_);                        \
    }                                                                                                        \
  }
#define RS_MMA1(K_, SET_)                                                                                    \
  {                                                                                                          \
    const int term_ = P1 ? 2 : (K_) / (SMI * NI), idx_ = (K_) % (SMI * NI), mi_ = idx_ % SMI, ni_ = idx_ / SMI; \
    if (term_ == 0) acc[mi_][ni_] = __builtin_amdgcn_mfma_f32_32x32x16_f16(fa_l[SET_][mi_], fb_h[SET_][ni_], acc[mi_][ni_], 0, 0, 0);       \
    else if (term_ == 1) acc[mi_][ni_] = __builtin_amdgcn_mfma_f32_32x32x16_f16(fa_h[SET_][mi_], fb_l[SET_][ni_], acc[mi_][ni_], 0, 0, 0);  \
    else acc[mi_][ni_] = __builtin_amdgcn_mfma_f32_32x32x16_f16(fa_h[SET_][mi_], fb_h[SET_][ni_], acc[mi_][ni_], 0, 0, 0);  \
  }

  float4 areg0[MODE == 0 ? 1 : NQ];
  float4 n01 = nrm01, n23 = nrm23;
#define RS_PRO_LOADS()                                                                                       \
  {                                                                                                          \
    RS_LOAD_A()                                                                                              \
    n01 = nrm01; n23 = nrm23;                                                                                \
    _Pragma("unroll") for (int i = 0; i < NQ; ++i) areg0[i] = areg[i];                                       \
    RS_LOAD_A()                                                                                              \
  }
  bool first_tile = true;
  for (;;) {
#pragma unroll
  for (int i = 0; i < SMI; ++i)
#pragma unroll
    for (int j = 0; j < NI; ++j)
#pragma unroll
      for (int r = 0; r < 16; ++r) acc[i][j][r] = 0.f;
  wptr = reinterpret_cast<const unsigned char*>(p.wpk_strip) + static_cast<size_t>(ct32) * 2048;
  b_left = S - 1;
  e_mt_i = mt_i; e_img = img_; e_py0 = py0_; e_px0 = px0_; e_m0 = m0; e_mend = mend; e_ct32 = ct32;
  RS_CLK(5)
  if (!first_tile) wg_barrier();
  if constexpr (MODE != 0) {
    if (tid < 8) *reinterpret_cast<uint4*>(lds + (tid >> 2) * ASLOT + ((tid >> 1) & 1) * PLANE + ZROW + (tid & 1) * 16) = make_uint4(0u, 0u, 0u, 0u);
  }
  a_next = 0;
  RS_A_REBUILD()
  if constexpr (MODE == 0) {
    RS_ISSUE_A(0)
    RS_ISSUE_A(1)
  }
#pragma unroll
  for (int i = 0; i < NBST - 1; ++i) RS_ISSUE_B(i)
  if constexpr (MODE != 0) {
    RS_PRO_LOADS()
    {
      float4 areg1[NQ];
      const float4 m01 = nrm01, m23 = nrm23;
#pragma unroll
      for (int i = 0; i < NQ; ++i) { areg1[i] = areg[i]; areg[i] = areg0[i]; }
      nrm01 = n01; nrm23 = n23;
      RS_STORE_A(0)
#pragma unroll
      for (int i = 0; i < NQ; ++i) areg[i] = areg1[i];
      nrm01 = m01; nrm23 = m23;
      RS_STORE_A(1)
    }
  }
  RS_CLK(6)
  wait_vm<0>();
  wg_barrier();
  RS_CLK(1)
#pragma unroll
  for (int k = 0; k < NRD; ++k) RS_READ1(k, 0, 0, 0, 0)

#define RS_STEP(H_, T_)                                                                                      \
  {                                                                                                          \
    constexpr int q_ = (H_) * TT + (T_);                        \
    constexpr int set_ = q_ & 1, sl_ = q_ % NBST;                                                            \
    constexpr bool last_ = (T_) == TT - 1;                                                                   \
    constexpr int tn_ = last_ ? 0 : (T_) + 1, asn_ = last_ ? 1 - (H_) : (H_);                                \
     \
    if (!(RS_ABL & 64)) wait_vm<RING3 ? ((T_) == 0 ? PAW : 0) : 2 * NI * (NBST - 3) + ((T_) <= NBST - 4 ? PAW : 0)>();  \
    if constexpr (MODE != 0 && (T_) == NBST - 2) { RS_STORE_A(1 - (H_)) }     \
    if constexpr (last_ && !(RS_VAR & 8)) {                                                                  \
      wait_lds();                                                                                            \
      if (!(RS_ABL & 32)) wg_barrier();                                                                      \
      if (RS_VAR & 16) {           \
        unsigned long long t_;                                                                               \
        asm volatile("s_memrealtime %0\n\ts_waitcnt lgkmcnt(0)" : "=s"(t_)::"memory");                       \
        if (((static_cast<unsigned>(t_) >> RS_SLICE_BITS) ^ slotpar_) & 1u) __builtin_amdgcn_s_setprio(2);   \
        else __builtin_amdgcn_s_setprio(0);                                                                  \
      }                                                                                                      \
      if constexpr (RING3) { RS_ISSUE_B((sl_ + NBST - 1) % NBST) }      \
      if (!(RS_ABL & 2)) { if constexpr (MODE == 0) { RS_ISSUE_A(H_) } else { RS_LOAD_A() } }    \
    }                                                                                                        \
    if (!(RS_ABL & 1) && !(RS_VAR & 8) && !(RING3 && last_)) RS_ISSUE_B((sl_ + NBST - 1) % NBST)             \
    __builtin_amdgcn_sched_barrier(0);                                                                       \
    if (RS_VAR & 2) {                  \
      _Pragma("unroll") for (int k = 0; k < NRD; ++k) RS_READ1(k, 1 - set_, tn_, asn_, (sl_ + 1) % NBST)     \
      __builtin_amdgcn_sched_barrier(0);                                                                     \
    }                                                                                                        \
    if (RS_VAR & 1) __builtin_amdgcn_s_setprio(1);                                                           \
     \
    if (S2 && RS_S2_SKIP) {                                                                                  \
      _Pragma("unroll") for (int k = 0; k < NRD; ++k) RS_READ1(k, 1 - set_, tn_, asn_, (sl_ + 1) % NBST)     \
      __builtin_amdgcn_sched_barrier(0);                                                                     \
    }                                                                                                        \
    if (!(S2 && RS_S2_SKIP) || ((s2_taps_ >> (T_)) & 1u)) {                                                  \
    _Pragma("unroll") for (int k = 0; k < NMM; ++k) {                                                        \
      if (!(RS_ABL & 8)) RS_MMA1(k, set_)                                                                    \
      if (RS_VAR & 8) {             \
        if (last_ && k == 2 * SMI * NI) { if (!(RS_ABL & 32)) wg_barrier(); }        \
        if (last_ && k == 2 * SMI * NI + 1) { if (!(RS_ABL & 2)) { if constexpr (MODE == 0) { RS_ISSUE_A(H_) } else { RS_LOAD_A() } } } \
        if (k == 2 * SMI * NI + 2) { if (!(RS_ABL & 1)) RS_ISSUE_B((sl_ + NBST - 1) % NBST) }                \
      }                                                                                                      \
      if (!(RS_VAR & 2) && !(S2 && RS_S2_SKIP)) {                                                           \
        constexpr int kr0_ = (RS_VAR & 4) ? 2 : 0;         \
        const bool isb_ = (k - kr0_ < NI) || (k - kr0_ >= NI + SMI && k - kr0_ < 2 * NI + SMI);              \
        if (k >= kr0_ && k - kr0_ < NRD && !(RS_ABL & 4) && !((RS_ABL & 128) && !isb_) && !((RS_ABL & 256) && isb_)) \
          RS_READ1(k - kr0_, 1 - set_, tn_, asn_, (sl_ + 1) % NBST)                                          \
      }                                                                                                      \
      __builtin_amdgcn_sched_barrier(0);                                                                     \
    }                                                                                                        \
    }                                                                                                        \
    if constexpr (NRD > NMM && !(RS_VAR & 2) && !(S2 && RS_S2_SKIP)) {         \
      _Pragma("unroll") for (int k = NMM; k < NRD; ++k) { if (!(RS_ABL & 4)) RS_READ1(k, 1 - set_, tn_, asn_, (sl_ + 1) % NBST) } \
      __builtin_amdgcn_sched_barrier(0);                                                                     \
    }                                                                                                        \
    if (RS_VAR & 1) __builtin_amdgcn_s_setprio(0);                                                           \
  }
  const unsigned slotpar_ = __builtin_amdgcn_s_getreg(6148) & 1u;
  unsigned s2_taps_ = 15u;
  const int s2_nb_ = S2 ? (p.cb1 < p.ncb ? p.cb1 : p.ncb) : 1;
  for (int hbp = 0; hbp < NHB; hbp += 2) {
    if constexpr (S2) {
      const int plane_ = (hbp >> 1) / s2_nb_;
      const unsigned rows_ = (plane_ >> 1) ? 3u : 2u, cols_ = (plane_ & 1) ? 3u : 2u;
      s2_taps_ = p.gkw == 1 ? 8u : ((((rows_ & 1u) && (cols_ & 1u)) ? 1u : 0u) | ((rows_ & 1u) ? 2u : 0u) | ((cols_ & 1u) ? 4u : 0u) | 8u);
    }
    if constexpr (TT == 5) {
      RS_STEP(0, 0) RS_STEP(0, 1) RS_STEP(0, 2) RS_STEP(0, 3) RS_STEP(0, 4)
      RS_STEP(1, 0) RS_STEP(1, 1) RS_STEP(1, 2) RS_STEP(1, 3) RS_STEP(1, 4)
    } else if constexpr (TT == 4) {
      RS_STEP(0, 0) RS_STEP(0, 1) RS_STEP(0, 2) RS_STEP(0, 3)
      RS_STEP(1, 0) RS_STEP(1, 1) RS_STEP(1, 2) RS_STEP(1, 3)
    } else {
      RS_STEP(0, 0) RS_STEP(0, 1) RS_STEP(0, 2) RS_STEP(0, 3) RS_STEP(0, 4) RS_STEP(0, 5) RS_STEP(0, 6) RS_STEP(0, 7) RS_STEP(0, 8)
      RS_STEP(1, 0) RS_STEP(1, 1) RS_STEP(1, 2) RS_STEP(1, 3) RS_STEP(1, 4) RS_STEP(1, 5) RS_STEP(1, 6) RS_STEP(1, 7) RS_STEP(1, 8)
    }
  }
  wait_vm<0>();
  wait_lds();
  RS_CLK(2)
  constexpr int ES = 32 * NI + 4, F4 = 8 * NI, KG = 4 * NI;
  int tid_e_ = tid;
  if constexpr (PERSIST) asm volatile("" : "+v"(tid_e_));
  bool more_ = false;
  {
  const int tid = tid_e_, lane = tid & 63, l31 = lane & 31, lh = lane >> 5;
  (void)l31; (void)lh;
  float* S_ = reinterpret_cast<float*>(sB);
  constexpr bool EPI_IN_ASLOTS = NBST * BREC < 2 * 32 * ES * 4;
  if constexpr (EPI_IN_ASLOTS) {
    wg_barrier();
    S_ = reinterpret_cast<float*>(lds + wave * (2 * 32 * ES * 4));
    static_assert(!EPI_IN_ASLOTS || NW * 2 * 32 * (32 * NI + 4) * 4 <= LDSB, "epilogue staging inside the workgroup's LDS block");
// ... 126 lines not shown
      const float4 a4 = *reinterpret_cast<const float4*>(S_ + rl * ES + c);
      float y[4] = {a4.x, a4.y, a4.z, a4.w};
#pragma unroll
      for (int e = 0; e < 4; ++e) y[e] += (e < nv) ? bq[e] : 0.f;
      if (p.addm) { y[0] += am[k].x; y[1] += am[k].y; y[2] += am[k].z; y[3] += am[k].w; }
      float* drow = p.dst + pix * p.dst_cs;
      int dch = p.dst_co + colq;
      int dhl = p.dst_hl;
      if (p.tstats) {
        const double y0 = y[0], y1 = y[1], y2 = y[2], y3 = y[3];
        if (nv > 0) { ts0 += y0; tq0 += y0 * y0; }
        if (nv > 1) { ts1 += y1; tq1 += y1 * y1; }
        if (nv > 2) { ts2 += y2; tq2 += y2 * y2; }
        if (nv > 3) { ts3 += y3; tq3 += y3 * y3; }
      }
      if (p.epi == 1) {
#pragma unroll
        for (int e = 0; e < 4; ++e) y[e] = fmaxf(y[e], 0.f);
      } else if (p.epi == 2) {
        if (colq < p.gru_c) {
#pragma unroll
          for (int e = 0; e < 4; ++e) y[e] = sigmoidf_(y[e]);
        } else {
          y[0] = sigmoidf_(y[0]) * hv[k].x; y[1] = sigmoidf_(y[1]) * hv[k].y;
          y[2] = sigmoidf_(y[2]) * hv[k].z; y[3] = sigmoidf_(y[3]) * hv[k].w;
          drow = p.dst2 + pix * p.dst2_cs;
          dch = p.dst2_co + c2;
          dhl = p.dst2_hl;
        }
      } else if (p.epi == 3) {
        const float4 z = zv[k], h4_ = hv[k];
        y[0] = (1.f - z.x) * h4_.x + z.x * tanhf(y[0]); y[1] = (1.f - z.y) * h4_.y + z.y * tanhf(y[1]);
        y[2] = (1.f - z.z) * h4_.z + z.z * tanhf(y[2]); y[3] = (1.f - z.w) * h4_.w + z.w * tanhf(y[3]);
      }
      if (dhl) {
        store_quad_hl(drow, dch, y[0], y[1], y[2], y[3], nv, p.a_scale, sat_n);
      } else if (nv == 4) {
        *reinterpret_cast<float4*>(drow + dch) = make_float4(y[0], y[1], y[2], y[3]);
      } else {
#pragma unroll
        for (int e = 0; e < 3; ++e)
          if (e < nv) drow[dch + e] = y[e];
      }
      if (p.dsth) store_quad_hl(p.dsth + pix * p.dsth_cs, p.dsth_co + colq, y[0], y[1], y[2], y[3], nv, p.a_scale, sat_n);
    }
  }
  }
  if (p.tstats) {
#pragma unroll
    for (int o = F4; o < 64; o <<= 1) {
      ts0 += rp::shfl_xor_f64(ts0, o); ts1 += rp::shfl_xor_f64(ts1, o); ts2 += rp::shfl_xor_f64(ts2, o); ts3 += rp::shfl_xor_f64(ts3, o);
      tq0 += rp::shfl_xor_f64(tq0, o); tq1 += rp::shfl_xor_f64(tq1, o); tq2 += rp::shfl_xor_f64(tq2, o); tq3 += rp::shfl_xor_f64(tq3, o);
    }
    if (lane < F4) {
      const int col = colw + lane * 4;
      const double ts[4] = {ts0, ts1, ts2, ts3}, tq[4] = {tq0, tq1, tq2, tq3};
#pragma unroll
      for (int e = 0; e < 4; ++e)
        if (col + e < p.Cout) {
          double* o = p.tstats + (static_cast<long long>(e_mt_i) * p.Cout + col + e) * 2;
          o[0] = ts[e];
          o[1] = tq[e];
        }
    }
  }
  RS_CLK(3)
  }
  first_tile = false;
  if constexpr (!PERSIST) break;
  if (!more_) break;
  RS_TILE_GEOM(t_base + t_idx)
  RS_TILE_ROWS()
  if constexpr (!SPATIAL) { RS_TILE_FRAG_ADDR() }
  sat_here = MODE != 0 && p.sat != nullptr && nt_i == 0;
  }
  if (p.sat && sat_n) atomicAdd(p.sat, static_cast<unsigned long long>(sat_n));
}

template <int SMI_, bool P1_ = false>
int strip_launch_height(const KParams& p, int nw, int ni, bool spatial, bool hlin, bool norm, unsigned nwg, hipStream_t st) {
  const dim3 grid(nwg), block(nw * 64);
  if (p.stride == 2) {
    if constexpr (!P1_) {
      if (ni != 1 || hlin || norm || !spatial) return 1;
      if (nw == 2) hipLaunchKernelGGL((conv_strip_f16x3_kernel<2, 4, 1, 1, SMI_, false>), grid, block, 0, st, p);
      else if (nw == 3) hipLaunchKernelGGL((conv_strip_f16x3_kernel<3, 4, 1, 1, SMI_, false>), grid, block, 0, st, p);
      else hipLaunchKernelGGL((conv_strip_f16x3_kernel<4, 4, 1, 1, SMI_, false>), grid, block, 0, st, p);
      return 0;
    } else {
      return 1;
    }
  }
#define RS_LAUNCH(NW_, NI_)                                                                                               \
  if (spatial) {                                                                                                          \
    if (norm) {                                                                                                           \
      if constexpr (NI_ == 1 && SMI_ == 5 && !P1_) {                                                                      \
        if (p.n_tiles > 0) hipLaunchKernelGGL((conv_strip_f16x3_kernel<NW_, 9, 2, NI_, SMI_, P1_, true>), grid, block, 0, st, p);   \
        else hipLaunchKernelGGL((conv_strip_f16x3_kernel<NW_, 9, 2, NI_, SMI_, P1_>), grid, block, 0, st, p);             \
      } else hipLaunchKernelGGL((conv_strip_f16x3_kernel<NW_, 9, 2, NI_, SMI_, P1_>), grid, block, 0, st, p);             \
    }                                                                                                                     \
    else if (hlin) hipLaunchKernelGGL((conv_strip_f16x3_kernel<NW_, 9, 0, NI_, SMI_, P1_>), grid, block, 0, st, p);            \
    else {                                                                                                                \
      if constexpr (NI_ == 1 && SMI_ == 5 && !P1_) {                                                                      \
        if (p.n_tiles > 0) hipLaunchKernelGGL((conv_strip_f16x3_kernel<NW_, 9, 1, NI_, SMI_, P1_, true>), grid, block, 0, st, p);   \
        else hipLaunchKernelGGL((conv_strip_f16x3_kernel<NW_, 9, 1, NI_, SMI_, P1_>), grid, block, 0, st, p);             \
      } else hipLaunchKernelGGL((conv_strip_f16x3_kernel<NW_, 9, 1, NI_, SMI_, P1_>), grid, block, 0, st, p);             \
    }                                                                                                                     \
  } else {                                                                                                                \
    if (hlin) hipLaunchKernelGGL((conv_strip_f16x3_kernel<NW_, 5, 0, NI_, SMI_, P1_>), grid, block, 0, st, p);                 \
    else hipLaunchKernelGGL((conv_strip_f16x3_kernel<NW_, 5, 1, NI_, SMI_, P1_>), grid, block, 0, st, p);                      \
  }
  if (ni == 2) {
    if constexpr (SMI_ == 5 && !P1_) {
      if (nw == 4) { RS_LAUNCH(4, 2) } else if (nw == 3) { RS_LAUNCH(3, 2) } else { RS_LAUNCH(2, 2) }
    } else {
      return 1;
    }
  } else {
    if (nw == 2) { RS_LAUNCH(2, 1) } else if (nw == 3) { RS_LAUNCH(3, 1) } else { RS_LAUNCH(4, 1) }
  }
#undef RS_LAUNCH
  return 0;
}

}
```

rnnpose_amd/engine.py:

```python
from __future__ import annotations

import torch

from . import env, ops, streams


class UpdateEngine:
    def __init__(self, update_block):
        self.blk = update_block
        self._key = None
        self._w = None
        self._buf_key = None
        self._b = None
        self._sets = {}
        self.epoch = 0
        self._ksws = {}
        self.split_batch = env.flag("RNNPOSE_SPLIT_BATCH", True)
        self.side_stream = env.flag("RNNPOSE_SIDE_STREAM", False)
        self.parts = env.number("RNNPOSE_PARTS", 2)
        self.parts_forced = env.text("RNNPOSE_PARTS") is not None
        self.fused_mask = env.flag("RNNPOSE_FUSED_MASK", True)
        self.resident_1x1 = env.flag("RNNPOSE_RESIDENT_1X1", True)
        self.fused_lookup = env.flag("RNNPOSE_FUSED_LOOKUP", False)
        self.fused_induced = env.flag("RNNPOSE_FUSED_INDUCED", False)
# ... 179 lines not shown
        tl = self.tile.get
        R = ops.EPI_RELU

        ks_main = b.get("_ksws")
        ks_side = b.get("_ksws_side") if side is not None else ks_main

        def c(name, srcs, dst, epi, hl_out=False, ks=None, **kw):
            ops.conv2d_nhwc(W[name], srcs, dst, epi, src_hl=hl, dst_hl=hl and hl_out, tile=tl(name, 0),
                            ksplit_ws=ks_main if ks is None else ks, single_product=self.single_product, **kw)
        def flow_chain():
            if induced is not None:
                ops.flow_features_induced(induced, W["convf1_wt"], W["convf1_b"], b["flo1"], b["motion"], 126, out_split=hl, motion_split=hl,
                                          a_scale=ops.A_SCALE)
            else:
                ops.flow_features(coords1, W["convf1_wt"], W["convf1_b"], b["flo1"], b["motion"], 126, subtract_grid=not flow_is_delta,
                                  out_split=hl, motion_split=hl, a_scale=ops.A_SCALE)
            yield
            c("convf2", [(b["flo1"], 0)], (b["corflo"], 192), R, hl_out=True, ks=ks_side)
            yield

        join = None
        if side is None:
            yield from flow_chain()
        else:
            join = streams.side_branch(main, side, lambda: streams.drain(flow_chain()))
        if have_cor1:
            pass
        elif self.resident_1x1 and W["convc1r"] is not None:
            ops.conv1x1_resident(W["convc1r"], (b["corr"], 0), (b["cor1"], 0), relu=True, dst_split=hl)
            yield
        else:
            ops.conv2d_nhwc(W["convc1"], [(b["corr"], 0)], (b["cor1"], 0), R, dst_hl=hl, single_product=self.single_product)
            yield
        c("convc2", [(b["cor1"], 0)], (b["corflo"], 0), R, hl_out=True)
        yield
        if join is not None:
            main.wait_event(join)
        c("conv", [(b["corflo"], 0)], (b["motion"], 0), R, hl_out=True)
        yield
        hs = (lambda k: b[k + "_s"]) if hl else (lambda k: b[k])
        hx = lambda hbuf: [(hbuf, 0), (b["motion"], 0)]
        sp = (lambda k: dict(dst_split=(b[k + "_s"], 0))) if hl else (lambda k: {})
        c("zr", hx(hs("hA")), (b["z"], 0), ops.EPI_GRU_ZR, aux0=(b["hA"], 0), dst2=(b["rh"], 0), dst2_hl=hl, gru_c=128, add_map=(b["inp1"], 0))
        yield
        c("q", hx(b["rh"]), (b["hB"], 0), ops.EPI_GRU_Q, aux0=(b["hA"], 0), aux1=(b["z"], 0), add_map=(b["inp1"], 256), **sp("hB"))
        yield
        c("zr2", hx(hs("hB")), (b["z"], 0), ops.EPI_GRU_ZR, aux0=(b["hB"], 0), dst2=(b["rh"], 0), dst2_hl=hl, gru_c=128, add_map=(b["inp2"], 0))
        yield
        c("q2", hx(b["rh"]), (b["hA"], 0), ops.EPI_GRU_Q, aux0=(b["hB"], 0), aux1=(b["z"], 0), add_map=(b["inp2"], 256), **sp("hA"))
        yield
        c("heads", [(hs("hA"), 0)], (b["heads"], 0), R)
        yield
        head = lambda: ops.flow_head_out(b["heads"], 0, 256, W["flow2_w"], W["flow2_b"], coords1, b["delta"], b["coords1"],
                                         b["flow_lr"])
        if side is None:
            head()
            yield
            if mask_here:
                ops.conv2d_nhwc(W["mask2"], [(b["heads"], 256)], (b["mask"], 0), ops.EPI_LINEAR, single_product=self.single_product)
                yield
            return
        join2 = streams.side_branch(main, side, head)
        if mask_here:
            ops.conv2d_nhwc(W["mask2"], [(b["heads"], 256)], (b["mask"], 0), ops.EPI_LINEAR, single_product=self.single_product)
        main.wait_event(join2)
        yield


class EncoderEngine:

    def __init__(self, fnet):
        self.fnet = fnet
        self._key = None
        self._w = None
        self._ksws = {}
        self.resident_1x1 = env.flag("RNNPOSE_RESIDENT_1X1", True)
        self.ksplit = env.flag("RNNPOSE_KSPLIT", True)
        self.single_product = False
        self.split_batch = env.flag("RNNPOSE_SPLIT_ENCODER", True)
        self.parts = env.number("RNNPOSE_ENCODER_PARTS", 1)
        self.merge_sets = env.flag("RNNPOSE_ENCODER_MERGE", None)

    MIN_SET_PIXELS = 800_000

    def _mine(self):
        f = self.fnet
        convs = {}
        for li, layer in enumerate((f.layer1, f.layer2, f.layer3), start=1):
            for bi, blk in enumerate(layer):
                convs[f"l{li}.{bi}.c1"] = blk.conv1
                convs[f"l{li}.{bi}.c2"] = blk.conv2
                if blk.downsample is not None:
                    convs[f"l{li}.{bi}.down"] = blk.downsample[0]
        convs["out"] = f.conv2
        return convs

    def refresh(self):
        self._weights()
        return self._key

    def _weights(self):
        convs = self._mine()
        convs["stem"] = self.fnet.conv1
        key = ops.param_key(convs.values())
        if key != self._key:
            stem = convs.pop("stem")
            self._w = {k: ops.PackedConv(m.weight, m.bias, [m.weight.shape[1]]) for k, m in convs.items()}
            self._w["stem"] = ops.PackedStem(stem.weight, stem.bias)
            oc = convs["out"]
            self._w["outr"] = ops.PackedConv1x1(oc.weight, oc.bias) if ops.PackedConv1x1.fits(oc.weight) else None
            self._key = key
        return self._w

    @staticmethod
    def _conv(pc, x, stride=1, stats=True, in_norm=None, ks=None, sp=False):
        return ops.conv2d_nhwc_new(pc, x, ops.EPI_LINEAR, stride, stats, in_norm, src_bounded=True, ksplit_ws=ks, single_product=sp)

    @staticmethod
    def _block_gen(W, name, blk, x, x_norm=None, ks=None, sp=False):
        E = EncoderEngine
        st = blk.conv1.stride[0]
        c1, ts1 = E._conv(W[name + ".c1"], x, st, in_norm=None if x_norm is None else x_norm[0], ks=ks, sp=sp)
        yield
        mr1 = ops.instnorm_tiles_nhwc(c1, ts1, stats_only=True)
        yield
        res, res_norm = x, x_norm
        if blk.downsample is not None:
            assert x_norm is None
            res, tsd = E._conv(W[name + ".down"], x, st, ks=ks, sp=sp)
            yield
            res_norm = (ops.instnorm_tiles_nhwc(res, tsd, stats_only=True), False)
            yield
        c2, ts2 = E._conv(W[name + ".c2"], c1, in_norm=mr1, ks=ks, sp=sp)
        yield
        out = ops.instnorm_tiles_nhwc(c2, ts2, relu=True, residual=res, residual_norm=None if res_norm is None else res_norm[0],
                                      residual_relu=bool(res_norm and res_norm[1]))
        yield
        return out

    @torch.no_grad()
    def __call__(self, images, normalize=True, split_out=False):
        W = self._weights()
        imgs = [images] if torch.is_tensor(images) else list(images)
        imgs = [ops._chk(t, "image") for t in imgs]
        merge = self.merge_sets
        if merge is None and len(imgs) > 1:
            merge = min(t.shape[0] * t.shape[2] * t.shape[3] for t in imgs) < self.MIN_SET_PIXELS
        if merge and len(imgs) > 1:
            imgs = [torch.cat(imgs, 0)]
        _, _, H, Wd = imgs[0].shape
        N = sum(t.shape[0] for t in imgs)
        dev = imgs[0].device
        H8, W8 = ((H + 1) // 2 + 1) // 2, ((Wd + 1) // 2 + 1) // 2
        H8, W8 = (H8 + 1) // 2, (W8 + 1) // 2
        if split_out:
            out = torch.empty(N, H8, W8, self.fnet.conv2.out_channels, device=dev, dtype=torch.float32)
        else:
            out = torch.empty(N, self.fnet.conv2.out_channels, H8, W8, device=dev, dtype=torch.float32)
        if len(imgs) > 1:
            cuts = [sum(t.shape[0] for t in imgs[:i]) for i in range(len(imgs) + 1)]
            jobs = [(t, a, b) for t, a, b in zip(imgs, cuts[:-1], cuts[1:])]
        else:
            parts = max(1, min(self.parts if self.split_batch else 1, N))
            cuts = [N * i // parts for i in range(parts + 1)]
            jobs = [(imgs[0][a:b], a, b) for a, b in zip(cuts[:-1], cuts[1:])]
        main = torch.cuda.current_stream()

        def job(x_part, b0, b1, ji):
            yield from self._forward_gen(W, x_part, out[b0:b1], normalize, split_out, ks=self._ksplit_ws(ji, x_part))

        streams.run_interleaved([(job(x_part, b0, b1, i), main if i == 0 else streams.helper_stream(dev, (i - 1) % 3))
                                 for i, (x_part, b0, b1) in enumerate(jobs)], main)
        return ops.SplitTensor(out, ops.A_SCALE) if split_out else out

    def _ksplit_ws(self, ji, x_part):
        n, _, H, Wd = x_part.shape
        return ops.ksplit_workspace_in(self._ksws, (ji, str(x_part.device)), self.ksplit, n * ((H + 7) // 8) * ((Wd + 7) // 8), x_part.device)

    def _forward_gen(self, W, x_nchw, out, normalize, split_out=False, ks=None):
        E = EncoderEngine
        f = self.fnet
        x, ts = ops.stem_conv(W["stem"], x_nchw, normalize)
        yield
        if ts is not None:
            x_norm = (ops.instnorm_tiles_nhwc(x, ts, stats_only=True), True)
        else:
            x, x_norm = ops.instnorm_nhwc(x, relu=True), None
        yield
        for li, layer in enumerate((f.layer1, f.layer2, f.layer3), start=1):
            for bi, blk in enumerate(layer):
                x = yield from E._block_gen(W, f"l{li}.{bi}", blk, x, x_norm, ks=ks, sp=self.single_product)
                x_norm = None
        if W["outr"] is not None and self.resident_1x1:
            if split_out:
                ops.conv1x1_resident(W["outr"], (x, 0), (out, 0), relu=False, dst_split=True)
                yield
                return
            o = torch.empty(*x.shape[:3], 256, device=x.device, dtype=torch.float32)
            ops.conv1x1_resident(W["outr"], (x, 0), (o, 0), relu=False)
        else:
            o, _ = E._conv(W["out"], x, stats=False, ks=ks, sp=self.single_product)
        yield
        if split_out:
            ops.split_hl(o, dst=out, a_scale=ops.A_SCALE)
        else:
            ops.nhwc_to_nchw(o, out=out)
        yield
```

rnnpose_amd/ops.py:

```python
from __future__ import annotations

import ctypes as C
from contextlib import contextmanager

import torch

from . import _lib, env

F32 = torch.float32
F64 = torch.float64

_prof = None


_event_pool = []


@contextmanager
def profile(names=None):
    global _prof
    prev = _prof
    rec = {"_only": set(names) if names else None, "_next": 0}
    _prof = rec
    try:
        yield rec
    finally:
        _prof = prev


def profile_begin(names=None):
    global _prof
    rec = {"_only": set(names) if names else None, "_next": 0, "_prev": _prof}
    _prof = rec
    return rec


def profile_end(rec):
    global _prof
    _prof = rec.get("_prev")


def profiling() -> bool:
    return _prof is not None


def summarize(rec) -> dict:
    torch.cuda.synchronize()
    out = {}
    for k, evs in rec.items():
        if k.startswith("_"):
            continue
        ms = [a.elapsed_time(b) for a, b, _, _ in evs]
        out[k] = (len(ms), sum(ms) / max(len(ms), 1), sum(ms), sum(w for _, _, w, _ in evs), sum(n for _, _, _, n in evs))
    return out


def _launch(name, *args, work=0, nbytes=0, products=3):
    rec = _prof
    if rec is not None and (rec["_only"] is None or name in rec["_only"]):
        ex = rec.setdefault("_exec", {})
        ex[name] = ex.get(name, 0.0) + products * work
        i = rec["_next"]
        rec["_next"] = i + 2
        while len(_event_pool) < i + 2:
            _event_pool.append(torch.cuda.Event(enable_timing=True))
        a, b = _event_pool[i], _event_pool[i + 1]
        a.record()
        _lib.call(name, *args)
        b.record()
        rec.setdefault(name, []).append((a, b, work, nbytes))
    else:
        _lib.call(name, *args)


def _stream():
    return C.c_void_p(torch.cuda.current_stream().cuda_stream)


def _chk(t: torch.Tensor, name: str, dtype=F32) -> torch.Tensor:
    if not isinstance(t, torch.Tensor):
        raise TypeError(f"{name} must be a torch.Tensor")
    if not t.is_cuda:
        raise RuntimeError(f"{name} must live on the GPU (got {t.device}); rnnpose_amd has no CPU path")
    if t.dtype != dtype:
        t = t.to(dtype)
    return t.contiguous()
# ... 554 lines not shown
    return out.reshape(*sh, 4, 4)


def se3_compose(A, Bm):
    A, Bm = _chk(A, "A"), _chk(Bm, "B")
    if A.shape != Bm.shape:
        raise ValueError("se3_compose needs equal shapes")
    out = torch.empty_like(A)
    _launch("rnnpose_se3_compose_f32", _ptr(A), _ptr(Bm), A.numel() // 16, _ptr(out), _stream())
    return out


def se3_outer_update(Tij, Ti, literal: bool = True):
    Tij, Ti = _chk(Tij, "Tij"), _chk(Ti, "Ti")
    if Tij.shape != Ti.shape:
        raise ValueError("se3_outer_update needs equal shapes")
    Ti_new, Tij_new = torch.empty_like(Ti), torch.empty_like(Tij)
    _launch("rnnpose_se3_outer_update_f32", _ptr(Tij), _ptr(Ti), Ti.numel() // 16, int(bool(literal)), _ptr(Ti_new), _ptr(Tij_new), _stream())
    return Ti_new, Tij_new


def se3_inverse(A):
    A = _chk(A, "A")
    out = torch.empty_like(A)
    _launch("rnnpose_se3_inverse_f32", _ptr(A), A.numel() // 16, _ptr(out), _stream())
    return out


def gru_gate(zr, hcat, z_out, rhx, C: int = 128):
    B, Ctot = hcat.shape[0], hcat.shape[1]
    hw = hcat.shape[2] * hcat.shape[3]
    _launch("rnnpose_gru_gate_f32", _ptr(zr), _ptr(hcat), B, C, Ctot, hw, _ptr(z_out), _ptr(rhx), _stream())


def gru_update(z, q_pre, hcat, hout, C: int = 128):
    B = hcat.shape[0]
    hw = hcat.shape[2] * hcat.shape[3]
    _launch("rnnpose_gru_update_f32", _ptr(z), _ptr(q_pre), _ptr(hcat), B, C, hcat.shape[1], hw, _ptr(hout), hout.shape[1],
            _stream())


EPI_LINEAR, EPI_RELU, EPI_GRU_ZR, EPI_GRU_Q = 0, 1, 2, 3
A_SCALE = 8.0


class PackedConv:

    def __init__(self, weight, bias, seg_counts=None, post_scale: float = 1.0, a_scale: float = A_SCALE):
        import math
        range_guard_arm(weight.device)
        w = _chk(weight.detach(), "weight") * post_scale
        b = _chk(bias.detach(), "bias") * post_scale
        self.c_out, self.c_in, self.kh, self.kw = w.shape
        self.c_in_real = self.c_in
        self.seg_counts = [int(c) for c in (seg_counts or [self.c_in])]
        if sum(self.seg_counts) != self.c_in:
            raise ValueError("seg_counts must sum to the input channels")
        wmax = float(w.abs().max())
        self.w_scale = float(2.0 ** math.floor(math.log2(1024.0 / wmax))) if wmax > 0 else 1.0
        self.a_scale = float(a_scale)
        segs = (C.c_int * len(self.seg_counts))(*self.seg_counts)
        n = int(_lib.load().rnnpose_conv_packed_halfs(self.c_out, self.kh, self.kw, segs, len(self.seg_counts)))
        if n <= 0:
            raise ValueError("unsupported convolution shape")
        self.w_packed = torch.empty(n, device=w.device, dtype=torch.float16)
        self.bias = b.contiguous()
        _lib.call("rnnpose_conv_pack_weights_f16x3", _ptr(w), self.c_out, self.c_in, self.kh, self.kw, segs,
                  len(self.seg_counts), self.w_scale, _ptr(self.w_packed), _stream())


def param_key(modules):
    return tuple((m.weight._version, m.weight.data_ptr(), m.bias._version, m.bias.data_ptr()) for m in modules)


def _nhwc(t, name):
    if not (t.is_cuda and t.dtype == F32 and t.is_contiguous() and t.dim() == 4):
        raise ValueError(f"{name} must be a contiguous fp32 CUDA tensor shaped (B,H,W,C)")
    return t


def conv2d_nhwc(pc: PackedConv, srcs, dst, epilogue: int = EPI_LINEAR, aux0=None, aux1=None, dst2=None, gru_c: int = 0,
                stride: int = 1, tile_stats=None, add_map=None, in_norm=None, src_hl: bool = False, dst_hl: bool = False,
                dst2_hl: bool = False, dst_split=None, tile: int = 0, src_bounded: bool = False, ksplit_ws=None,
                single_product=None):
    _apply_conv_env()
    d = _lib.ConvDesc()
    if len(srcs) != len(pc.seg_counts):
        raise ValueError("number of sources differs from the packed segment list")
    B, H, W, _ = srcs[0][0].shape
    for i, ((t, off), cnt) in enumerate(zip(srcs, pc.seg_counts)):
        _nhwc(t, f"src{i}")
        if t.shape[:3] != (B, H, W):
            raise ValueError("sources must share (B,H,W)")
        d.src[i] = _lib.ConvSrc(t.data_ptr(), t.shape[3], off, cnt)
    d.n_src = len(srcs)
    d.B, d.H, d.W, d.kh, d.kw, d.stride = B, H, W, pc.kh, pc.kw, stride
    d.w_packed, d.bias = pc.w_packed.data_ptr(), pc.bias.data_ptr()
    d.c_out, d.a_scale, d.w_scale, d.epilogue = pc.c_out, pc.a_scale, pc.w_scale, epilogue

    def put(prefix, spec):
        if spec is None:
            return
        t, off = spec
        _nhwc(t, prefix)
        setattr(d, prefix, t.data_ptr())
        setattr(d, prefix + "_c_stride", t.shape[3])
        setattr(d, prefix + "_c_offset", off)

    put("dst", dst)
    put("aux0", aux0)
    put("aux1", aux1)
    put("dst2", dst2)
    if add_map is not None:
        t, off = add_map
        _nhwc(t, "add_map")
        d.add_map, d.add_c_stride, d.add_c_offset = t.data_ptr(), t.shape[3], off
    d.gru_c = gru_c
    if in_norm is not None:
        if not (in_norm.is_cuda and in_norm.dtype == F32 and in_norm.is_contiguous() and tuple(in_norm.shape) == (B, srcs[0][0].shape[3], 2)):
            raise ValueError("in_norm must be a contiguous fp32 CUDA tensor of (B, C_source, 2)")
        d.src0_mean_rstd = in_norm.data_ptr()
    d.src_hl, d.dst_hl, d.dst2_hl, d.tile = int(bool(src_hl)), int(bool(dst_hl)), int(bool(dst2_hl)), int(tile)
    if tile_stats is not None:
        tpi = int(_lib.load().rnnpose_conv_tiles_per_image_desc(C.byref(d)))
        if not (tile_stats.is_cuda and tile_stats.dtype == F64 and tile_stats.is_contiguous()
                and tile_stats.numel() == B * tpi * pc.c_out * 2):
            raise ValueError("tile_stats must be a contiguous FP64 CUDA tensor of (B * conv_tiles_per_image(H, W, kh, kw, stride, c_out, tile, B, "
                             f"src_counts, fused_norm) = {B * tpi}, c_out, 2): the tile count depends on the kernel the launch takes")
        d.tile_stats, d.tile_stats_records = tile_stats.data_ptr(), B * tpi
    d.src_bounded = int(bool(src_bounded))
    if dst_split is not None:
        t, off = dst_split
        _nhwc(t, "dst_split")
        d.dst_split, d.dst_split_c_stride, d.dst_split_c_offset = t.data_ptr(), t.shape[3], off
    if ksplit_ws is not None:
        d.ksplit_ws, d.ksplit_ws_bytes = ksplit_ws.data_ptr(), ksplit_ws.numel() * ksplit_ws.element_size()
    d.single_product = int(_single_product if single_product is None else bool(single_product))
    Ho, Wo = -(-H // stride), -(-W // stride)
    nb = B * H * W * pc.c_in_real + pc.c_out * pc.c_in_real * pc.kh * pc.kw + B * Ho * Wo * pc.c_out
    nb += B * Ho * Wo * pc.c_out * (add_map is not None) + B * Ho * Wo * (gru_c if epilogue == EPI_GRU_ZR else 0)
    nb += 2 * B * Ho * Wo * pc.c_out * (epilogue == EPI_GRU_Q) + B * Ho * Wo * pc.c_out * (dst_split is not None)
    products = 3
    if d.single_product and _prof is not None:
        products = int(_lib.load().rnnpose_conv_products_desc(C.byref(d)))
    _launch("rnnpose_conv2d_nhwc_f16x3", C.byref(d), _stream(),
            work=2.0 * B * Ho * Wo * pc.c_out * pc.c_in_real * pc.kh * pc.kw, nbytes=4.0 * nb, products=products)


_single_product = False


def single_product(enable=None) -> bool:
    global _single_product
    if enable is not None:
        _single_product = bool(enable)
    return _single_product


def conv_tiles_per_image(H, W, kh, kw, stride=1, c_out=None, tile: int = 0, batch: int = 1, src_counts=None, fused_norm: bool = False) -> int:
    _apply_conv_env()
    if c_out is None:
        c_out, tile = 64, 1
    elif src_counts is None and stride == 2 and tile not in (1, 2, 3, 4):
        raise ValueError("conv_tiles_per_image: whether a stride-2 launch takes the strip kernels depends on its sources: pass src_counts")
    d = _lib.ConvDesc()
    for i, c in enumerate(src_counts or [32]):
        d.src[i] = _lib.ConvSrc(None, int(c), 0, int(c))
    d.n_src = len(src_counts or [32])
    d.B, d.H, d.W, d.kh, d.kw, d.stride, d.c_out, d.tile = int(batch), int(H), int(W), int(kh), int(kw), int(stride), int(c_out), int(tile)
    d.src0_mean_rstd = 16 if fused_norm else None
    return int(_lib.load().rnnpose_conv_tiles_per_image_desc(C.byref(d)))


_conv_env_applied = False


def _apply_conv_env():
    global _conv_env_applied
    if not _conv_env_applied:
        _conv_env_applied = True
        for name, entry, read in (("RNNPOSE_SPATIAL_TILES", "rnnpose_conv_spatial_tiles", env.flag),
                                  ("RNNPOSE_KSPLIT", "rnnpose_conv_ksplit", env.flag),
                                  ("RNNPOSE_LOOKUP_VARIANT", "rnnpose_corr_lookup_variant", env.flag),
                                  ("RNNPOSE_STRIP", "rnnpose_conv_strip", env.number),
                                  ("RNNPOSE_CORR_VARIANT", "rnnpose_corr_variant", env.number)):
            v = read(name, None)
            if v is not None:
                _lib.call(entry, int(v))
        v = env.text("RNNPOSE_KSPLIT_LIMITS")
        if v:
            a, b = (int(t) for t in v.split(","))
            _lib.call("rnnpose_conv_ksplit_limits", a, b)


def conv_spatial_tiles(enable: bool = True):
    _lib.call("rnnpose_conv_spatial_tiles", int(bool(enable)))


def conv_strip(mode=True):
    _apply_conv_env()
    _lib.call("rnnpose_conv_strip", int(mode))


def conv_ksplit(enable: bool = True):
    _lib.call("rnnpose_conv_ksplit", int(bool(enable)))


def conv_ksplit_workspace(device):
    n = int(_lib.load().rnnpose_conv_ksplit_workspace_bytes())
    return torch.zeros((n + 3) // 4, device=device, dtype=torch.int32)


KSPLIT_MAX_PIXELS = 96 * 128


def ksplit_workspace_in(reg, key, enabled, pixels, device, keep=None):
    if not enabled or pixels > KSPLIT_MAX_PIXELS:
        return None
    if key not in reg:
        for k in [k for k in reg if keep is not None and not keep(k)]:
            del reg[k]
        reg[key] = conv_ksplit_workspace(device)
    return reg[key]


def conv2d_nhwc_new(pc: PackedConv, x, epilogue: int = EPI_LINEAR, stride: int = 1, stats: bool = False, in_norm=None, tile: int = 0, **kw):
    B, H, W, _ = x.shape
    out = torch.empty(B, -(-H // stride), -(-W // stride), pc.c_out, device=x.device, dtype=F32)
    ts = None
    if stats:
        tpi = conv_tiles_per_image(H, W, pc.kh, pc.kw, stride, pc.c_out, tile, B, src_counts=pc.seg_counts, fused_norm=in_norm is not None)
        ts = torch.empty(B * tpi, pc.c_out, 2, device=x.device, dtype=F64)
    conv2d_nhwc(pc, [(x, 0)], (out, 0), epilogue, stride=stride, tile_stats=ts, in_norm=in_norm, tile=tile, **kw)
    return out, ts


_nchw_pc = {}


def conv2d_nchw(weight, bias, x, relu: bool = False):
    x = _chk(x, "x")
    B, Cin, H, W = x.shape
    Cout, Cin_w, kh, kw = weight.shape
    if Cin_w != Cin:
        raise ValueError(f"weight expects {Cin_w} input channels, got {Cin}")
    cin_p, cout_p = -(-Cin // 4) * 4, -(-Cout // 4) * 4
    key = (weight.data_ptr(), weight._version, bias.data_ptr(), bias._version, tuple(weight.shape))
    ent = _nchw_pc.get(key)
    pc = ent[0] if (ent is not None and ent[1] is weight and ent[2] is bias) else None
    if pc is None:
        w = _chk(weight.detach(), "weight")
        if cin_p != Cin:
            w = torch.nn.functional.pad(w, (0, 0, 0, 0, 0, cin_p - Cin))
        pc = PackedConv(w, bias, [cin_p])
        pc.c_in_real = Cin
        if len(_nchw_pc) >= 64:
            _nchw_pc.pop(next(iter(_nchw_pc)))
        _nchw_pc[key] = (pc, weight, bias)
    xn = (torch.zeros if cin_p != Cin else torch.empty)(B, H, W, cin_p, device=x.device, dtype=F32)
    nchw_to_nhwc(x, xn)
    out = torch.empty(B, H, W, cout_p, device=x.device, dtype=F32)
    conv2d_nhwc(pc, [(xn, 0)], (out, 0), EPI_RELU if relu else EPI_LINEAR)
    return nhwc_to_nchw(out, 0, Cout)


def corr_lookup_nhwc(pyramid_buf, coords, out=None, levels: int = 4, radius: int = 4):
    coords = _chk(coords, "coords")
    B, _, h, w = coords.shape
    if out is None:
        out = torch.empty(B, h, w, levels * (2 * radius + 1) ** 2, device=coords.device, dtype=F32)
    _launch("rnnpose_corr_lookup_nhwc_f32", _ptr(pyramid_buf), _ptr(coords), B, h, w, levels, radius, _ptr(out), _stream(),
            nbytes=_lookup_bytes(B, h, w, levels, radius))
    return out


def corr_lookup_nhwc_part(pyramid_buf, coords, out, B, b0, b1, levels: int = 4, radius: int = 4):
    coords = _chk(coords, "coords")
    n, _, h, w = coords.shape
    if n != b1 - b0:
        raise ValueError("coords must hold the b1 - b0 images of the part")
    _launch("rnnpose_corr_lookup_nhwc_part_f32", _ptr(pyramid_buf), _ptr(coords), B, b0, b1, h, w, levels, radius, _ptr(out),
            _stream(), nbytes=_lookup_bytes(b1 - b0, h, w, levels, radius))
    return out


class InducedCoords:

    def __init__(self, depth, K, G, h, w, eps, out):
        self.depth, self.K, self.G = _chk(depth, "depth"), _chk(K, "K"), _chk(G, "G")
        self.h, self.w, self.eps, self.out = int(h), int(w), float(eps), out
        self.H, self.W = int(depth.shape[-2]), int(depth.shape[-1])
        n = depth.shape[0]
        if tuple(K.shape[-2:]) != (3, 3) or tuple(G.shape[-2:]) != (4, 4) or K.reshape(-1, 3, 3).shape[0] != n or G.reshape(-1, 4, 4).shape[0] != n:
            raise ValueError("K (n,3,3) and G (n,4,4) must match depth (n,1,H,W)")
        if tuple(out.shape) != (n, 2, self.h, self.w) or not out.is_contiguous():
            raise ValueError("out must be a contiguous (n,2,h,w) tensor")


def corr_lookup_induced_nhwc_part(pyramid_buf, ic: InducedCoords, out, B, b0, b1, levels: int = 4, radius: int = 4):
    if ic.depth.shape[0] != b1 - b0:
        raise ValueError("the coordinate source must hold the b1 - b0 images of the part")
    _launch("rnnpose_corr_lookup_induced_nhwc_part_f32", _ptr(pyramid_buf), _ptr(ic.depth), _ptr(ic.K), _ptr(ic.G), ic.H, ic.W, ic.eps, B, b0, b1,
            ic.h, ic.w, levels, radius, _ptr(ic.out), _ptr(out), _stream(), nbytes=_lookup_bytes(b1 - b0, ic.h, ic.w, levels, radius))
    return out


def flow_features_induced(ic: InducedCoords, w_t, bias, out, motion, motion_c_offset, out_c_offset=0, out_split: bool = False,
                          motion_split: bool = False, a_scale: float = 8.0):
    B, c_out = ic.depth.shape[0], w_t.shape[1]
    _launch("rnnpose_flow_features_induced_f32", _ptr(ic.depth), _ptr(ic.K), _ptr(ic.G), ic.H, ic.W, ic.eps, _ptr(w_t), _ptr(bias), B, ic.h, ic.w,
            c_out, _ptr(out), out.shape[-1], out_c_offset, _ptr(motion), motion.shape[3], motion_c_offset, int(bool(out_split)),
            int(bool(motion_split)), float(a_scale), _stream(), work=2.0 * 98 * c_out * B * ic.h * ic.w)
    return out

# ... 14 lines not shown
    _launch("rnnpose_nhwc_to_nchw_f32", _ptr(src), B, c_count, H * W, Cs, c_offset, _ptr(dst), _stream())
    return dst


def flow_prep(coords1, flow4, motion, motion_c_offset, subtract_grid: bool = True):
    B, _, h, w = coords1.shape
    _launch("rnnpose_flow_prep_f32", _ptr(coords1), int(subtract_grid), B, h, w, _ptr(flow4), _ptr(motion), motion.shape[3],
            motion_c_offset, _stream())


def flow_conv7x7_relu(flow4, w_t, bias, out, out_c_offset=0):
    B, h, w, _ = flow4.shape
    c_out = w_t.shape[1]
    _launch("rnnpose_flow_conv7x7_relu_f32", _ptr(flow4), _ptr(w_t), _ptr(bias), B, h, w, c_out, _ptr(out), out.shape[-1],
            out_c_offset, _stream(), work=2.0 * 98 * c_out * B * h * w)
    return out


def flow_features(coords1, w_t, bias, out, motion, motion_c_offset, out_c_offset=0, subtract_grid: bool = True,
                  out_split: bool = False, motion_split: bool = False, a_scale: float = 8.0):
    B, _, h, w = coords1.shape
    c_out = w_t.shape[1]
    _launch("rnnpose_flow_features_f32", _ptr(coords1), int(subtract_grid), _ptr(w_t), _ptr(bias), B, h, w, c_out, _ptr(out),
            out.shape[-1], out_c_offset, _ptr(motion), motion.shape[3], motion_c_offset, int(bool(out_split)), int(bool(motion_split)),
            float(a_scale), _stream(), work=2.0 * 98 * c_out * B * h * w)
    return out


def split_hl(src, dst=None, src_c_offset: int = 0, c_count: int | None = None, dst_c_offset: int = 0, a_scale: float = 8.0):
    _nhwc(src, "src")
    B, H, W, Cs = src.shape
    c_count = Cs - src_c_offset if c_count is None else c_count
    if dst is None:
        dst = torch.empty(B, H, W, c_count, device=src.device, dtype=F32)
    _lib.call("rnnpose_split_hl_f32", _ptr(src), Cs, int(src_c_offset), B * H * W, int(c_count), float(a_scale), _ptr(dst),
              dst.shape[3], int(dst_c_offset), _stream())
    return dst


def unsplit_hl(t, a_scale: float = 8.0):
    sh = t.shape
    v = t.contiguous().view(torch.float16).view(*sh[:-1], sh[-1] // 8, 2, 8).float()
    return ((v[..., 0, :] + v[..., 1, :]) / a_scale).reshape(sh)


def flow_head_out(x, x_c_offset, c_in, weight, bias, coords1, delta, coords1_out, flow_lr):
    B, h, w, cs = x.shape
    _launch("rnnpose_flow_head_out_f32", _ptr(x), cs, x_c_offset, c_in, _ptr(weight), _ptr(bias), _ptr(coords1), B, h, w,
            _ptr(delta), _ptr(coords1_out), _ptr(flow_lr), _stream())


def convex_upsample_nhwc(flow_lr, mask, out=None):
    B, h, w, _ = mask.shape
    if out is None:
        out = torch.empty(B, 2, 8 * h, 8 * w, device=mask.device, dtype=F32)
    _launch("rnnpose_convex_upsample_nhwc_f32", _ptr(flow_lr), _ptr(mask), B, h, w, _ptr(out), _stream(),
            nbytes=4.0 * B * h * w * (576 + 2 + 128))
    return out


class PackedConv1x1:

    @staticmethod
    def fits(weight) -> bool:
        s = tuple(weight.shape)
        return len(s) == 4 and s[0] == 256 and s[2:] == (1, 1) and s[1] % 4 == 0 and s[1] <= 352

    def __init__(self, weight, bias, a_scale: float = A_SCALE):
        import math
        range_guard_arm(weight.device)
        w = _chk(weight.detach(), "weight")
        if not self.fits(w):
            raise ValueError("needs a (256, c_in <= 352, 1, 1) weight with c_in % 4 == 0")
        self.c_in = int(w.shape[1])
        wmax = float(w.abs().max())
        self.w_scale = float(2.0 ** math.floor(math.log2(1024.0 / wmax))) if wmax > 0 else 1.0
        self.a_scale = float(a_scale)
        self.bias = _chk(bias.detach(), "bias").contiguous()
        n = int(_lib.load().rnnpose_conv1x1_resident_packed_bytes(self.c_in))
        self.w_packed = torch.empty(n // 2, device=w.device, dtype=torch.float16)
        _lib.call("rnnpose_conv1x1_resident_pack_f16x3", _ptr(w), 256, self.c_in, self.w_scale, _ptr(self.w_packed), _stream())


def conv1x1_resident(pc: PackedConv1x1, src, dst, relu: bool = True, dst_split: bool = False):
    x, xo = src
    y, yo = dst
    _nhwc(x, "src"); _nhwc(y, "dst")
    n = x.shape[0] * x.shape[1] * x.shape[2]
    if y.shape[:3] != x.shape[:3]:
        raise ValueError("src and dst must share (B,h,w)")
    _launch("rnnpose_conv1x1_resident_f16x3", _ptr(x), x.shape[3], int(xo), pc.c_in, _ptr(pc.w_packed), _ptr(pc.bias), pc.a_scale,
            pc.w_scale, int(bool(relu)), n, _ptr(y), y.shape[3], int(yo), int(bool(dst_split)), _stream(), work=2.0 * n * 256 * pc.c_in)


def corr_lookup_convc1(pc: PackedConv1x1, pyramid_buf, coords, dst, B_total, b0, b1, levels=4, radius=4, relu: bool = True,
                       dst_split: bool = False):
    y, yo = dst
    _nhwc(y, "dst")
    coords = _chk(coords, "coords")
    nb, two, h, w = coords.shape
    if pc.c_in != 324 or two != 2 or nb != b1 - b0 or tuple(y.shape[:3]) != (nb, h, w):
        raise ValueError("corr_lookup_convc1: weights packed for c_in = 324, coords (b1-b0,2,h,w), dst (b1-b0,h,w,C)")
    n = nb * h * w
    _launch("rnnpose_corr_lookup_convc1_f16x3", _ptr(pyramid_buf), _ptr(coords), int(B_total), int(b0), int(b1), h, w, int(levels), int(radius),
            _ptr(pc.w_packed), _ptr(pc.bias), pc.a_scale, pc.w_scale, int(bool(relu)), _ptr(y), y.shape[3], int(yo), int(bool(dst_split)),
            _stream(), work=2.0 * n * 256 * 324, nbytes=4.0 * n * (levels * 100 + 2 + 256))


class PackedMaskHead:

    def __init__(self, weight, bias, post_scale: float = 0.25, a_scale: float = A_SCALE):
        import math
        range_guard_arm(weight.device)
        w = _chk(weight.detach(), "weight")
        if tuple(w.shape) != (576, 256, 1, 1):
            raise ValueError("mask.2 weight must be (576,256,1,1)")
        wmax = float(w.abs().max()) * post_scale
        self.w_scale = float(2.0 ** math.floor(math.log2(1024.0 / wmax))) if wmax > 0 else 1.0
        self.a_scale = float(a_scale)
        self.bias = (_chk(bias.detach(), "bias") * post_scale).contiguous()
        n = int(_lib.load().rnnpose_mask_upsample_packed_bytes())
        self.w_packed = torch.empty(n // 2, device=w.device, dtype=torch.float16)
        _lib.call("rnnpose_mask_upsample_pack_f16x3", _ptr(w), float(post_scale), self.w_scale, _ptr(self.w_packed), _stream())


def mask_upsample(pm: PackedMaskHead, x, x_c_offset, flow_lr, out=None):
    _nhwc(x, "x")
    B, h, w, cs = x.shape
    if out is None:
        out = torch.empty(B, 2, 8 * h, 8 * w, device=x.device, dtype=F32)
    _launch("rnnpose_mask_upsample_f16x3", _ptr(x), cs, int(x_c_offset), _ptr(pm.w_packed), 576, _ptr(pm.bias), pm.a_scale,
            pm.w_scale, _ptr(_chk(flow_lr, "flow_lr")), B, h, w, _ptr(out), _stream(), work=2.0 * B * h * w * 576 * 256,
            nbytes=4.0 * B * h * w * (256 + 2 + 128))
    return out


_guard_env = env.flag("RNNPOSE_RANGE_GUARD", True)
_guard_on = False
_guard_devices = set()


def range_guard_arm(device=None):
    global _guard_on
    if not _guard_env:
        return
    dev = torch.cuda.current_device() if device is None else torch.device(device).index
    if dev in _guard_devices and _guard_on:
        return
    with torch.cuda.device(dev):
        _lib.call("rnnpose_f16x3_saturation_check", 1)
    _guard_devices.add(dev)
    _guard_on = True


def range_guard_state() -> bool:
    return _guard_on


def saturation_check(enable: bool = True):
    global _guard_on
    _lib.call("rnnpose_f16x3_saturation_check", int(bool(enable)))
    _guard_on = bool(enable)
    if enable:
        _guard_devices.add(torch.cuda.current_device())


def saturation_events(out=None):
    if out is None:
        out = torch.zeros(1, device="cuda", dtype=torch.int64)
    _lib.call("rnnpose_f16x3_saturation_peek", _ptr(out), _stream())
    return out


def saturation_count(reset: bool = True) -> int:
    n = C.c_ulonglong(0)
# ... 636 lines not shown
```

Baseline: 765.7.

## Defer residual-block output norm+add into the consuming stride-2 conv and 1x1 conv

The last residual block of each encoder layer no longer materialises its normalized, residual-added output. It hands a lazy record (conv2 output, its statistics, and the residual with optional norm and ReLU) to the next consumer. That consumer, either the stride-2 strip conv in a new MODE 3 or the resident 1x1 output conv, applies instnorm, ReLU and the residual add while loading its input. This removes a full-resolution elementwise pass and its write and read of the activation. In exchange the loaders get extra loads of the residual and statistics, more LDS and register pressure, and GRU operand slots reused through unions.

```diff
diff --git a/include/rnnpose_hip.h b/include/rnnpose_hip.h
--- a/include/rnnpose_hip.h
+++ b/include/rnnpose_hip.h
@@ -153,6 +153,10 @@
   size_t ksplit_ws_bytes;
   int single_product;
   int tile_stats_records;
+  const float* src0_residual;
+  int src0_residual_c_stride, src0_residual_c_offset;
+  const float* src0_residual_mean_rstd;
+  int src0_residual_relu;
 } rnnpose_conv_desc_t;
 
 size_t rnnpose_conv_ksplit_workspace_bytes(void);
@@ -161,6 +165,7 @@
 
 int rnnpose_conv_tiles_per_image_desc(const rnnpose_conv_desc_t* h_desc);
 int rnnpose_conv_products_desc(const rnnpose_conv_desc_t* h_desc);
+int rnnpose_conv_lazy_residual_desc(const rnnpose_conv_desc_t* h_desc);
 int rnnpose_conv_spatial_tiles(int enable);
 int rnnpose_conv_strip(int mode);
 long long rnnpose_conv_packed_halfs(int c_out, int kh, int kw, const int* h_seg_counts, int n_seg);
@@ -241,12 +246,21 @@
 int rnnpose_radius_neighbors_f32(const float* queries, int n_q, const float* supports, const int* q_start, const int* s_start,
                                  int n_clouds, float radius, const long long* offsets, int* cand_idx, float* cand_d2, int width,
                                  int* out, rnnpose_stream_t stream);
+typedef struct {
+  const float* x_mean_rstd;
+  const float* residual;
+  int c_stride, c_offset;
+  const float* mean_rstd;
+  int relu;
+  int pixels_per_image;
+} rnnpose_lazy_residual_t;
 size_t rnnpose_conv1x1_resident_packed_bytes(int c_in);
 int rnnpose_conv1x1_resident_pack_f16x3(const float* weight, int c_out, int c_in, float w_scale, void* packed,
                                         rnnpose_stream_t stream);
 int rnnpose_conv1x1_resident_f16x3(const float* x, int x_c_stride, int x_c_offset, int c_in, const void* w_packed,
                                    const float* bias, float a_scale, float w_scale, int relu, long long n_pixels, float* dst,
-                                   int dst_c_stride, int dst_c_offset, int dst_split, rnnpose_stream_t stream);
+                                   int dst_c_stride, int dst_c_offset, int dst_split, const rnnpose_lazy_residual_t* h_lazy,
+                                   rnnpose_stream_t stream);
 int rnnpose_corr_lookup_convc1_f16x3(const float* pyramid, const float* coords, int B, int b0, int b1, int h, int w, int levels,
                                      int radius, const void* w_packed, const float* bias, float a_scale, float w_scale, int relu,
                                      float* dst, int dst_c_stride, int dst_c_offset, int dst_split, rnnpose_stream_t stream);
diff --git a/rnnpose_amd/_lib.py b/rnnpose_amd/_lib.py
--- a/rnnpose_amd/_lib.py
+++ b/rnnpose_amd/_lib.py
@@ -30,7 +30,14 @@
                 ("src0_mean_rstd", C.c_void_p), ("src_hl", C.c_int), ("dst_hl", C.c_int), ("dst2_hl", C.c_int),
                 ("dst_split", C.c_void_p), ("dst_split_c_stride", C.c_int), ("dst_split_c_offset", C.c_int), ("src_bounded", C.c_int),
                 ("tile", C.c_int), ("ksplit_ws", C.c_void_p), ("ksplit_ws_bytes", C.c_size_t), ("single_product", C.c_int),
-                ("tile_stats_records", C.c_int)]
+                ("tile_stats_records", C.c_int),
+                ("src0_residual", C.c_void_p), ("src0_residual_c_stride", C.c_int), ("src0_residual_c_offset", C.c_int),
+                ("src0_residual_mean_rstd", C.c_void_p), ("src0_residual_relu", C.c_int)]
+
+
+class LazyResidual(C.Structure):
+    _fields_ = [("x_mean_rstd", C.c_void_p), ("residual", C.c_void_p), ("c_stride", C.c_int), ("c_offset", C.c_int),
+                ("mean_rstd", C.c_void_p), ("relu", C.c_int), ("pixels_per_image", C.c_int)]
 
 
 PROTOTYPES = {
@@ -75,6 +82,7 @@
     "rnnpose_gru_update_f32": (_i, [_p, _p, _p, _i, _i, _i, _i, _p, _i, _p]),
     "rnnpose_conv_tiles_per_image_desc": (_i, [C.POINTER(ConvDesc)]),
     "rnnpose_conv_products_desc": (_i, [C.POINTER(ConvDesc)]),
+    "rnnpose_conv_lazy_residual_desc": (_i, [C.POINTER(ConvDesc)]),
     "rnnpose_conv_spatial_tiles": (_i, [_i]),
     "rnnpose_conv_strip": (_i, [_i]),
     "rnnpose_conv_ksplit": (_i, [_i]),
@@ -122,7 +130,7 @@
     "rnnpose_mask_upsample_packed_bytes": (_z, []),
     "rnnpose_conv1x1_resident_packed_bytes": (_z, [_i]),
     "rnnpose_conv1x1_resident_pack_f16x3": (_i, [_p, _i, _i, _f, _p, _p]),
-    "rnnpose_conv1x1_resident_f16x3": (_i, [_p, _i, _i, _i, _p, _p, _f, _f, _i, _ll, _p, _i, _i, _i, _p]),
+    "rnnpose_conv1x1_resident_f16x3": (_i, [_p, _i, _i, _i, _p, _p, _f, _f, _i, _ll, _p, _i, _i, _i, C.POINTER(LazyResidual), _p]),
     "rnnpose_corr_lookup_convc1_f16x3": (_i, [_p, _p, _i, _i, _i, _i, _i, _i, _i, _p, _p, _f, _f, _i, _p, _i, _i, _i, _p]),
     "rnnpose_mask_upsample_pack_f16x3": (_i, [_p, _f, _f, _p, _p]),
     "rnnpose_instnorm_workspace_bytes": (_z, [_i, _i, _i]),
diff --git a/rnnpose_amd/csrc/conv1x1_resident.hip b/rnnpose_amd/csrc/conv1x1_resident.hip
--- a/rnnpose_amd/csrc/conv1x1_resident.hip
+++ b/rnnpose_amd/csrc/conv1x1_resident.hip
@@ -12,9 +12,14 @@
   int cs, co, Cin;
   const uint4* wpk;
   TileOut out;
+  const float* xmr;
+  const float* res;
+  int rcs, rco;
+  const float* rmr;
+  int rrelu, hw;
 };
 
-template <int NCB>
+template <int NCB, bool LAZY = false>
 __global__ __launch_bounds__(8 * MQ) __attribute__((amdgpu_num_vgpr(160))) void conv1x1_resident_kernel(const RParams p) {
   constexpr int NCBL = NCB * 4096 >= MQ * RSF * 4 ? NCB : (MQ * RSF * 4 + 4095) / 4096;
   __shared__ __attribute__((aligned(16))) _Float16 sA[NCBL][2][MQ * 32];
@@ -31,6 +36,35 @@
     for (int cb = 0; cb < NCB; ++cb) {
       const int c = cb * 32 + c4 * 4;
       av[cb] = *reinterpret_cast<const float4*>(src + (c < p.Cin ? c : 0));
+    }
+    if constexpr (LAZY) {
+      float4 rv[NCB], m01[NCB], m23[NCB], q01[NCB], q23[NCB];
+      const long long b = mc / p.hw;
+      const float* rsrc = p.res + mc * p.rcs + p.rco;
+      const float* msrc = p.xmr + (b * p.cs + p.co) * 2;
+      const float* qsrc = p.rmr ? p.rmr + (b * p.rcs + p.rco) * 2 : msrc;
+#pragma unroll
+      for (int cb = 0; cb < NCB; ++cb) {
+        const int c = cb * 32 + c4 * 4 < p.Cin ? cb * 32 + c4 * 4 : 0;
+        rv[cb] = *reinterpret_cast<const float4*>(rsrc + c);
+        m01[cb] = *reinterpret_cast<const float4*>(msrc + c * 2);
+        m23[cb] = *reinterpret_cast<const float4*>(msrc + c * 2 + 4);
+        q01[cb] = *reinterpret_cast<const float4*>(qsrc + c * 2);
+        q23[cb] = *reinterpret_cast<const float4*>(qsrc + c * 2 + 4);
+      }
+      __builtin_amdgcn_sched_barrier(0);
+#pragma unroll
+      for (int cb = 0; cb < NCB; ++cb) {
+        const float4 v = av[cb];
+        float4 y = make_float4(fmaxf((v.x - m01[cb].x) * m01[cb].y, 0.f), fmaxf((v.y - m01[cb].z) * m01[cb].w, 0.f),
+                               fmaxf((v.z - m23[cb].x) * m23[cb].y, 0.f), fmaxf((v.w - m23[cb].z) * m23[cb].w, 0.f));
+        float4 r = rv[cb];
+        if (p.rmr) {
+          r = make_float4((r.x - q01[cb].x) * q01[cb].y, (r.y - q01[cb].z) * q01[cb].w, (r.z - q23[cb].x) * q23[cb].y, (r.w - q23[cb].z) * q23[cb].w);
+          if (p.rrelu) r = make_float4(fmaxf(r.x, 0.f), fmaxf(r.y, 0.f), fmaxf(r.z, 0.f), fmaxf(r.w, 0.f));
+        }
+        av[cb] = make_float4(fmaxf(r.x + y.x, 0.f), fmaxf(r.y + y.y, 0.f), fmaxf(r.z + y.z, 0.f), fmaxf(r.w + y.w, 0.f));
+      }
     }
   }
   __builtin_amdgcn_sched_barrier(0);
@@ -109,7 +143,8 @@
 
 extern "C" int rnnpose_conv1x1_resident_f16x3(const float* x, int x_c_stride, int x_c_offset, int c_in, const void* w_packed,
                                               const float* bias, float a_scale, float w_scale, int relu, long long n_pixels,
-                                              float* dst, int dst_c_stride, int dst_c_offset, int dst_split, rnnpose_stream_t stream) {
+                                              float* dst, int dst_c_stride, int dst_c_offset, int dst_split,
+                                              const rnnpose_lazy_residual_t* h_lazy, rnnpose_stream_t stream) {
   const char* fn = "rnnpose_conv1x1_resident_f16x3";
   RP_REQUIRE(x && w_packed && bias && dst, fn, "null pointer");
   RP_REQUIRE(c_in > 0 && c_in <= 32 * MAX_NCB && c_in % 4 == 0, fn, "c_in must be a multiple of 4, at most 352");
@@ -124,6 +159,25 @@
   p.out = tile_out(bias, a_scale, w_scale, relu, dst, dst_c_stride, dst_c_offset, dst_split, n_pixels);
   const dim3 grid(static_cast<unsigned>(rp::cdiv(n_pixels, MQ))), block(8 * MQ);
   hipStream_t st = rp::as_stream(stream);
+  if (h_lazy) {
+    const rnnpose_lazy_residual_t& z = *h_lazy;
+    RP_REQUIRE(z.x_mean_rstd && z.residual && z.pixels_per_image > 0 && n_pixels % z.pixels_per_image == 0, fn,
+               "lazy residual: needs the statistics of x, the residual, and whole images of pixels_per_image pixels");
+    RP_REQUIRE(c_in <= 128, fn, "lazy residual: c_in <= 128");
+    RP_REQUIRE(z.c_offset >= 0 && z.c_offset % 4 == 0 && z.c_stride % 4 == 0 && z.c_offset + c_in <= z.c_stride &&
+                   reinterpret_cast<uintptr_t>(z.residual) % 16 == 0 && reinterpret_cast<uintptr_t>(z.x_mean_rstd) % 16 == 0 &&
+                   reinterpret_cast<uintptr_t>(z.mean_rstd) % 16 == 0, fn,
+               "lazy residual: channels inside the row, 16-byte aligned (statistics too)");
+    p.xmr = z.x_mean_rstd; p.res = z.residual; p.rcs = z.c_stride; p.rco = z.c_offset; p.rmr = z.mean_rstd; p.rrelu = z.relu != 0;
+    p.hw = z.pixels_per_image;
+    switch (rp::cdiv(c_in, 32)) {
+      case 1: hipLaunchKernelGGL((conv1x1_resident_kernel<1, true>), grid, block, 0, st, p); break;
+      case 2: hipLaunchKernelGGL((conv1x1_resident_kernel<2, true>), grid, block, 0, st, p); break;
+      case 3: hipLaunchKernelGGL((conv1x1_resident_kernel<3, true>), grid, block, 0, st, p); break;
+      default: hipLaunchKernelGGL((conv1x1_resident_kernel<4, true>), grid, block, 0, st, p); break;
+    }
+    return rp::check_launch(fn);
+  }
   switch (rp::cdiv(c_in, 32)) {
 #define R_CASE(N_) case N_: hipLaunchKernelGGL(conv1x1_resident_kernel<N_>, grid, block, 0, st, p); break;
     R_CASE(1) R_CASE(2) R_CASE(3) R_CASE(4) R_CASE(5) R_CASE(6) R_CASE(7) R_CASE(8) R_CASE(9) R_CASE(10) R_CASE(11)
diff --git a/rnnpose_amd/csrc/conv_common.cuh b/rnnpose_amd/csrc/conv_common.cuh
--- a/rnnpose_amd/csrc/conv_common.cuh
+++ b/rnnpose_amd/csrc/conv_common.cuh
@@ -31,10 +31,12 @@
   int dst_cs, dst_co;
   const float* aux0;
   int aux0_cs, aux0_co;
-  const float* aux1;
-  int aux1_cs, aux1_co;
-  float* dst2;
-  int dst2_cs, dst2_co;
+  union { const float* aux1; const float* res; };
+  union { int aux1_cs; int res_cs; };
+  union { int aux1_co; int res_co; };
+  union { float* dst2; const float* res_mr; };
+  union { int dst2_cs; int res_relu; };
+  int dst2_co;
   int gru_c;
   double* tstats;
   const float* addm;
diff --git a/rnnpose_amd/csrc/conv_igemm.hip b/rnnpose_amd/csrc/conv_igemm.hip
--- a/rnnpose_amd/csrc/conv_igemm.hip
+++ b/rnnpose_amd/csrc/conv_igemm.hip
@@ -705,14 +705,15 @@
   pl.stride = d->stride;
   pl.Ho = d->stride == 2 ? (H + 1) / 2 : H; pl.Wo = d->stride == 2 ? (W + 1) / 2 : W;
   pl.products = 3; pl.ksplit = 1;
+  const bool lazy = norm && d->src0_residual != nullptr;
   if (tile_ok && (d->tile >= 5 || (d->tile == 0 && pol.strip))) {
-    const bool s2_ok = d->n_src == 1 && d->src[0].c_count % 32 == 0 && !hlin && !norm && 4 * (d->src[0].c_count / 32) <= MAX_CB && (k33 || k11);
+    const bool s2_ok = d->n_src == 1 && d->src[0].c_count % 32 == 0 && !hlin && (!norm || lazy) && 4 * (d->src[0].c_count / 32) <= MAX_CB && (k33 || k11);
     if (d->stride == 1 || s2_ok)
       pl.rows = strip_rows(pol, H, W, d->kh, d->kw, d->stride, d->c_out, d->B, d->tile == 5 ? 160 : d->tile == 6 ? 32 : d->tile == 7 ? 96 : 0);
     if (d->tile == 0) {
       for (int s = 0; s < d->n_src; ++s)
         if (d->src[s].c_count % 32 != 0) pl.rows = 0;
-      if (norm && !k33) pl.rows = 0;
+      if (norm && !k33 && !(lazy && d->stride == 2)) pl.rows = 0;
     }
   }
   if (pl.rows) {
@@ -826,6 +827,12 @@
 int rnnpose_conv_tiles_per_image_desc(const rnnpose_conv_desc_t* d) {
   ConvPlan pl;
   return plan_conv(d, g_policy, &pl) ? pl.tiles_per_image : -1;
+}
+
+int rnnpose_conv_lazy_residual_desc(const rnnpose_conv_desc_t* d) {
+  ConvPlan pl;
+  if (!plan_conv(d, g_policy, &pl)) return -1;
+  return pl.rows != 0 && d->stride == 2 && d->src0_mean_rstd && d->src0_residual ? 1 : 0;
 }
 
 int rnnpose_conv_products_desc(const rnnpose_conv_desc_t* d) {
@@ -965,6 +972,20 @@
   p.gru_c = d->gru_c;
   p.tstats = d->tile_stats;
   p.in_mr = d->src0_mean_rstd;
+  if (d->src0_residual) {
+    RP_REQUIRE(d->src0_mean_rstd && pl.rows && d->stride == 2, fn,
+               "src0_residual needs src0_mean_rstd and a launch that takes the stride-2 strip form (rnnpose_conv_lazy_residual_desc answers 1)");
+    RP_REQUIRE(d->epilogue <= 1 && !d->aux1 && !d->dst2, fn, "src0_residual: linear / ReLU epilogue only (its fields travel in the GRU operands' slots)");
+    RP_REQUIRE(d->src0_residual_c_stride % 4 == 0 && d->src0_residual_c_offset % 4 == 0 && d->src0_residual_c_offset >= 0 &&
+                   d->src0_residual_c_offset + d->src[0].c_count <= d->src0_residual_c_stride &&
+                   reinterpret_cast<uintptr_t>(d->src0_residual) % 16 == 0 && reinterpret_cast<uintptr_t>(d->src0_residual_mean_rstd) % 16 == 0 &&
+                   reinterpret_cast<uintptr_t>(d->src0_mean_rstd) % 16 == 0, fn,
+               "src0_residual: 16-byte aligned (its statistics too), channel stride/offset multiples of 4, the source's channels inside the row");
+    RP_REQUIRE(static_cast<long long>(d->B) * d->H * d->W * d->src0_residual_c_stride < (1LL << 31), fn,
+               "residual tensor too large for 32-bit element offsets (B*H*W*c_stride must be < 2^31)");
+    p.res = d->src0_residual; p.res_cs = d->src0_residual_c_stride; p.res_co = d->src0_residual_c_offset;
+    p.res_mr = d->src0_residual_mean_rstd; p.res_relu = d->src0_residual_relu != 0;
+  }
   p.addm = d->add_map; p.addm_cs = d->add_c_stride; p.addm_co = d->add_c_offset;
   p.sat = d->src_bounded ? nullptr : rp::sat_counter();
   p.dst_hl = d->dst_hl; p.dst2_hl = d->dst2_hl;
diff --git a/rnnpose_amd/csrc/conv_strip_kernel.cuh b/rnnpose_amd/csrc/conv_strip_kernel.cuh
--- a/rnnpose_amd/csrc/conv_strip_kernel.cuh
+++ b/rnnpose_amd/csrc/conv_strip_kernel.cuh
@@ -263,10 +263,14 @@
   constexpr int NPP = AR / 32, NPIECE = 2 * NPP;
   constexpr int PA = (NPIECE + NW - 1) / NW;
   constexpr int NQ = (ARV * 4 + NT_ - 1) / NT_;
-  constexpr int PAW = MODE == 0 ? PA : (MODE == 1 ? NQ : NQ + 2);
+  constexpr int PAW = MODE == 0 ? PA : (MODE == 1 ? NQ : (MODE == 2 ? NQ + 2 : 2 * NQ));
+  static_assert(MODE != 3 || TT == 4, "the lazy residual is built for the stride-2 form");
   constexpr int ZROW = ARV * 32;
   constexpr int BOFF = 2 * ASLOT;
-  constexpr int LDSB = BOFF + NW * NBST * BREC;
+  constexpr int RBUF = BOFF + NW * NBST * BREC;
+  constexpr int RSTAT = RBUF + (MODE == 3 ? NQ * NT_ * 16 : 0);
+  constexpr int RSTAT_F4 = MAX_CB / 4 * 32 / 2;
+  constexpr int LDSB = RSTAT + (MODE == 3 ? 2 * RSTAT_F4 * 16 : 0);
   static_assert(PAW + 2 * NI * (NBST - 3) <= 63, "vmcnt is a 6-bit counter");
   static_assert(ZROW + 32 <= PLANE, "a zero row behind the data rows");
   __shared__ __attribute__((aligned(1024))) unsigned char lds[LDSB];
@@ -375,6 +379,9 @@
   const int S = NHB * TT;
   float4 areg[MODE == 0 ? 1 : NQ];
   float4 nrm01 = make_float4(0.f, 1.f, 0.f, 1.f), nrm23 = nrm01;
+  float4 rreg[MODE == 3 ? NQ : 1];
+  float4 rnm01 = nrm01, rnm23 = nrm01;
+  int scl = 0, scl_next = 0;
   int sat_n = 0;
   bool sat_here = MODE != 0 && p.sat != nullptr && nt_i == 0;
 
@@ -383,6 +390,7 @@
   const unsigned char* asp[MODE == 0 ? PA : NQ];
   unsigned ainc[MODE == 0 ? PA : NQ];
   const float* nsp = p.in_mr;
+  const unsigned char* rsp[MODE == 3 ? NQ : 1];
 #define RS_A_REBUILD()                                                                                       \
   {                                                                                                          \
     Seg sg_ = p.seg0;                                                                                        \
@@ -402,6 +410,14 @@
       ainc[i] = ok_ ? 64u : 0u;                                                                              \
     }                                                                                                        \
     if (MODE == 2) nsp = p.in_mr + (static_cast<long long>(img_) * sg_.cstride + sg_.coff + cl_) * 2;        \
+    if constexpr (MODE == 3) {       \
+      const int si_ = blk_ >= p.cb3 ? 3 : (blk_ >= p.cb2 ? 2 : (blk_ >= p.cb1 ? 1 : 0));                     \
+      const unsigned po_ = static_cast<unsigned>((si_ >> 1) * p.Vin + (si_ & 1));                            \
+      const unsigned char* rb_ = reinterpret_cast<const unsigned char*>(p.res + p.res_co + cl_);             \
+      _Pragma("unroll") for (int i = 0; i < NQ; ++i)                                                         \
+        rsp[i] = apix[i] >= 0 ? rb_ + static_cast<size_t>((static_cast<unsigned>(apix[i]) + po_) * static_cast<unsigned>(p.res_cs)) * 4 : g_zero_page + ((lane & 3) << 4); \
+      scl_next = cl_ >> 1;                                                                                   \
+    }                                                                                                        \
   }
 #define RS_A_ADVANCE()                                                                                       \
   {                                                                                                          \
@@ -412,6 +428,10 @@
       } else {                                                                                               \
         _Pragma("unroll") for (int i = 0; i < (MODE == 0 ? PA : NQ); ++i) asp[i] += ainc[i];                 \
         if (MODE == 2) nsp += 32;                                                                            \
+        if constexpr (MODE == 3) {                                                                           \
+          _Pragma("unroll") for (int i = 0; i < NQ; ++i) rsp[i] += ainc[i];                                  \
+          scl_next += 8;                                                                                     \
+        }                                                                                                    \
       }                                                                                                      \
     }                                                                                                        \
   }
@@ -429,8 +449,25 @@
       nrm01 = *reinterpret_cast<const float4*>(nsp);                                                         \
       nrm23 = *reinterpret_cast<const float4*>(nsp + 4);                                                     \
     }                                                                                                        \
+    {       \
+      [[maybe_unused]] constexpr int PAW_REG = MODE == 3 ? NQ : PAW;                                         \
+      [[maybe_unused]] constexpr int PAW = PAW_REG;                                                          \
     _Pragma("unroll") for (int i = 0; i < NQ; ++i) areg[i] = *reinterpret_cast<const float4*>(asp[i]);       \
+    }                                                                                                        \
+    if constexpr (MODE == 3) {       \
+      _Pragma("unroll") for (int i = 0; i < NQ; ++i)                                                         \
+        glds16(rsp[i], __builtin_amdgcn_readfirstlane(lds0 + RBUF + (wave * 64 + NT_ * i) * 16));            \
+      scl = scl_next;                                                                                        \
+    }                                                                                                        \
     RS_A_ADVANCE()                                                                                           \
+  }
+#define RS_FETCH_R(RREGS_)                                                                                   \
+  {                                                                                                          \
+    const float4* st_ = reinterpret_cast<const float4*>(lds + RSTAT) + scl;                                  \
+    nrm01 = st_[0]; nrm23 = st_[1]; rnm01 = st_[RSTAT_F4]; rnm23 = st_[RSTAT_F4 + 1];                        \
+    if (!(RREGS_)) {                                                                                         \
+      _Pragma("unroll") for (int i = 0; i < NQ; ++i) rreg[i] = *reinterpret_cast<const float4*>(lds + RBUF + (tid + NT_ * i) * 16); \
+    }                                                                                                        \
   }
 #define RS_STORE_A(SLOT_)                                                                                    \
   {                                                                                                          \
@@ -438,8 +475,16 @@
       const int idx_ = tid + NT_ * i, row_ = idx_ >> 2, quad_ = idx_ & 3;                                    \
       if (row_ < ARV) {                                                                                      \
         float4 xv_ = areg[i];                                                                                \
-        if (MODE == 2) xv_ = make_float4(fmaxf((xv_.x - nrm01.x) * nrm01.y, 0.f), fmaxf((xv_.y - nrm01.z) * nrm01.w, 0.f), \
+        if (MODE >= 2) xv_ = make_float4(fmaxf((xv_.x - nrm01.x) * nrm01.y, 0.f), fmaxf((xv_.y - nrm01.z) * nrm01.w, 0.f), \
                                          fmaxf((xv_.z - nrm23.x) * nrm23.y, 0.f), fmaxf((xv_.w - nrm23.z) * nrm23.w, 0.f)); \
+        if constexpr (MODE == 3) {       \
+          float4 rv_ = rreg[i];                                                                              \
+          if (p.res_mr) {                                                                                    \
+            rv_ = make_float4((rv_.x - rnm01.x) * rnm01.y, (rv_.y - rnm01.z) * rnm01.w, (rv_.z - rnm23.x) * rnm23.y, (rv_.w - rnm23.z) * rnm23.w); \
+            if (p.res_relu) rv_ = make_float4(fmaxf(rv_.x, 0.f), fmaxf(rv_.y, 0.f), fmaxf(rv_.z, 0.f), fmaxf(rv_.w, 0.f)); \
+          }                                                                                                  \
+          xv_ = make_float4(fmaxf(rv_.x + xv_.x, 0.f), fmaxf(rv_.y + xv_.y, 0.f), fmaxf(rv_.z + xv_.z, 0.f), fmaxf(rv_.w + xv_.w, 0.f)); \
+        }                                                                                                    \
         const bool in_ = apix[i] >= 0;                                                                       \
         if (sat_here) sat_n += (in_ && rp::quad_saturates(xv_, p.a_scale)) ? 1 : 0;                          \
         h4 hi_, lo_;                                                                                         \
@@ -526,7 +571,43 @@
   }
 #pragma unroll
   for (int i = 0; i < NBST - 1; ++i) RS_ISSUE_B(i)
-  if constexpr (MODE != 0) {
+  if constexpr (MODE == 3) {
+    RS_LOAD_A()
+    const int scl0 = scl, scl1 = scl_next;
+#pragma unroll
+    for (int i = 0; i < NQ; ++i) areg0[i] = areg[i];
+    float4 rreg1[NQ];
+#pragma unroll
+    for (int i = 0; i < NQ; ++i) {
+      areg[i] = *reinterpret_cast<const float4*>(asp[i]);
+      rreg1[i] = *reinterpret_cast<const float4*>(rsp[i]);
+    }
+    RS_A_ADVANCE()
+    {
+      const int nf4_ = p.seg0.ccount >> 1;
+      const float4* xs_ = reinterpret_cast<const float4*>(p.in_mr + (static_cast<long long>(img_) * p.seg0.cstride + p.seg0.coff) * 2);
+      const float4* rs_ = p.res_mr ? reinterpret_cast<const float4*>(p.res_mr + (static_cast<long long>(img_) * p.res_cs + p.res_co) * 2) : xs_;
+      float4* st_ = reinterpret_cast<float4*>(lds + RSTAT);
+      for (int i = tid; i < nf4_; i += NT_) { st_[i] = xs_[i]; st_[RSTAT_F4 + i] = rs_[i]; }
+    }
+    wait_vm<0>();
+    wait_lds();
+    wg_barrier();
+    {
+      float4 areg1[NQ];
+#pragma unroll
+      for (int i = 0; i < NQ; ++i) { areg1[i] = areg[i]; areg[i] = areg0[i]; }
+      scl = scl0;
+      RS_FETCH_R(0)
+      RS_STORE_A(0)
+#pragma unroll
+      for (int i = 0; i < NQ; ++i) { areg[i] = areg1[i]; rreg[i] = rreg1[i]; }
+      scl = scl1;
+      RS_FETCH_R(1)
+      RS_STORE_A(1)
+      wait_lds();
+    }
+  } else if constexpr (MODE != 0) {
     RS_PRO_LOADS()
     {
       float4 areg1[NQ];
@@ -556,7 +637,9 @@
     constexpr int tn_ = last_ ? 0 : (T_) + 1, asn_ = last_ ? 1 - (H_) : (H_);                                \
      \
     if (!(RS_ABL & 64)) wait_vm<RING3 ? ((T_) == 0 ? PAW : 0) : 2 * NI * (NBST - 3) + ((T_) <= NBST - 4 ? PAW : 0)>();  \
-    if constexpr (MODE != 0 && (T_) == NBST - 2) { RS_STORE_A(1 - (H_)) }     \
+         \
+    if constexpr (MODE == 3 && (T_) == NBST - 2) { if ((H_) != 0 || hbp != 0) { RS_FETCH_R(0) RS_STORE_A(1 - (H_)) } } \
+    if constexpr (MODE != 0 && MODE != 3 && (T_) == NBST - 2) { RS_STORE_A(1 - (H_)) }     \
     if constexpr (last_ && !(RS_VAR & 8)) {                                                                  \
       wait_lds();                                                                                            \
       if (!(RS_ABL & 32)) wg_barrier();                                                                      \
@@ -849,7 +932,13 @@
   const dim3 grid(nwg), block(nw * 64);
   if (p.stride == 2) {
     if constexpr (!P1_) {
-      if (ni != 1 || hlin || norm || !spatial) return 1;
+      if (ni != 1 || hlin || !spatial) return 1;
+      if (norm) {
+        if (nw == 2) hipLaunchKernelGGL((conv_strip_f16x3_kernel<2, 4, 3, 1, SMI_, false>), grid, block, 0, st, p);
+        else if (nw == 3) hipLaunchKernelGGL((conv_strip_f16x3_kernel<3, 4, 3, 1, SMI_, false>), grid, block, 0, st, p);
+        else hipLaunchKernelGGL((conv_strip_f16x3_kernel<4, 4, 3, 1, SMI_, false>), grid, block, 0, st, p);
+        return 0;
+      }
       if (nw == 2) hipLaunchKernelGGL((conv_strip_f16x3_kernel<2, 4, 1, 1, SMI_, false>), grid, block, 0, st, p);
       else if (nw == 3) hipLaunchKernelGGL((conv_strip_f16x3_kernel<3, 4, 1, 1, SMI_, false>), grid, block, 0, st, p);
       else hipLaunchKernelGGL((conv_strip_f16x3_kernel<4, 4, 1, 1, SMI_, false>), grid, block, 0, st, p);
diff --git a/rnnpose_amd/engine.py b/rnnpose_amd/engine.py
--- a/rnnpose_amd/engine.py
+++ b/rnnpose_amd/engine.py
@@ -285,6 +285,7 @@
         self.merge_sets = env.flag("RNNPOSE_ENCODER_MERGE", None)
 
     MIN_SET_PIXELS = 800_000
+    LAZY_STAGES = (1, 2, 3)
 
     def _mine(self):
         f = self.fnet
@@ -317,10 +318,17 @@
 
     @staticmethod
     def _conv(pc, x, stride=1, stats=True, in_norm=None, ks=None, sp=False):
+        if isinstance(x, ops.LazyBlock):
+            return ops.conv2d_nhwc_new(pc, x.c2, ops.EPI_LINEAR, stride, stats, x.mean_rstd, src_bounded=True, ksplit_ws=ks, single_product=sp,
+                                       lazy_residual=(x.residual, 0, x.residual_norm, x.residual_relu))
+        """-> (out, tile_stats or None) of ops.conv2d_nhwc_new.
+        src_bounded: every convolution input of the encoder is an instance-normalised map (|.| <= sqrt(H*W)) or a ReLU sum of a
+        few of them (extractor.py:48-58): two orders of magnitude inside the fp16x3 range, so the in-loop range check is skipped
+        (the stem, which sees the raw image, and the update block keep theirs)."""
         return ops.conv2d_nhwc_new(pc, x, ops.EPI_LINEAR, stride, stats, in_norm, src_bounded=True, ksplit_ws=ks, single_product=sp)
 
     @staticmethod
-    def _block_gen(W, name, blk, x, x_norm=None, ks=None, sp=False):
+    def _block_gen(W, name, blk, x, x_norm=None, ks=None, sp=False, lazy=False):
         E = EncoderEngine
         st = blk.conv1.stride[0]
         c1, ts1 = E._conv(W[name + ".c1"], x, st, in_norm=None if x_norm is None else x_norm[0], ks=ks, sp=sp)
@@ -328,6 +336,7 @@
         mr1 = ops.instnorm_tiles_nhwc(c1, ts1, stats_only=True)
         yield
         res, res_norm = x, x_norm
+        assert blk.downsample is not None or not isinstance(x, ops.LazyBlock)
         if blk.downsample is not None:
             assert x_norm is None
             res, tsd = E._conv(W[name + ".down"], x, st, ks=ks, sp=sp)
@@ -336,6 +345,11 @@
             yield
         c2, ts2 = E._conv(W[name + ".c2"], c1, in_norm=mr1, ks=ks, sp=sp)
         yield
+        if lazy:
+            out = ops.LazyBlock(c2, ops.instnorm_tiles_nhwc(c2, ts2, stats_only=True), res, None if res_norm is None else res_norm[0],
+                                bool(res_norm and res_norm[1]))
+            yield
+            return out
         out = ops.instnorm_tiles_nhwc(c2, ts2, relu=True, residual=res, residual_norm=None if res_norm is None else res_norm[0],
                                       residual_relu=bool(res_norm and res_norm[1]))
         yield
@@ -380,6 +394,18 @@
         n, _, H, Wd = x_part.shape
         return ops.ksplit_workspace_in(self._ksws, (ji, str(x_part.device)), self.ksplit, n * ((H + 7) // 8) * ((Wd + 7) // 8), x_part.device)
 
+    def _hands_over_lazy(self, W, li, layers, x):
+        if li not in self.LAZY_STAGES or isinstance(x, ops.LazyBlock):
+            return False
+        B, H, Wd, _ = x.shape
+        if li == len(layers):
+            return W["outr"] is not None and self.resident_1x1 and W["outr"].c_in <= 128
+        nxt = layers[li][0]
+        if nxt.downsample is None:
+            return False
+        st = nxt.conv1.stride[0]
+        return all(ops.conv_takes_lazy_residual(W[f"l{li + 1}.0.{k}"], B, H, Wd, st) for k in ("c1", "down"))
+
     def _forward_gen(self, W, x_nchw, out, normalize, split_out=False, ks=None):
         E = EncoderEngine
         f = self.fnet
@@ -390,17 +416,23 @@
         else:
             x, x_norm = ops.instnorm_nhwc(x, relu=True), None
         yield
-        for li, layer in enumerate((f.layer1, f.layer2, f.layer3), start=1):
+        layers = (f.layer1, f.layer2, f.layer3)
+        for li, layer in enumerate(layers, start=1):
             for bi, blk in enumerate(layer):
-                x = yield from E._block_gen(W, f"l{li}.{bi}", blk, x, x_norm, ks=ks, sp=self.single_product)
+                lazy = bi == len(layer) - 1 and self._hands_over_lazy(W, li, layers, x)
+                x = yield from E._block_gen(W, f"l{li}.{bi}", blk, x, x_norm, ks=ks, sp=self.single_product, lazy=lazy)
                 x_norm = None
         if W["outr"] is not None and self.resident_1x1:
+            lz = {}
+            if isinstance(x, ops.LazyBlock):
+                lz = dict(in_norm=x.mean_rstd, lazy_residual=(x.residual, 0, x.residual_norm, x.residual_relu))
+                x = x.c2
             if split_out:
-                ops.conv1x1_resident(W["outr"], (x, 0), (out, 0), relu=False, dst_split=True)
+                ops.conv1x1_resident(W["outr"], (x, 0), (out, 0), relu=False, dst_split=True, **lz)
                 yield
                 return
             o = torch.empty(*x.shape[:3], 256, device=x.device, dtype=torch.float32)
-            ops.conv1x1_resident(W["outr"], (x, 0), (o, 0), relu=False)
+            ops.conv1x1_resident(W["outr"], (x, 0), (o, 0), relu=False, **lz)
         else:
             o, _ = E._conv(W["out"], x, stats=False, ks=ks, sp=self.single_product)
         yield
diff --git a/rnnpose_amd/ops.py b/rnnpose_amd/ops.py
--- a/rnnpose_amd/ops.py
+++ b/rnnpose_amd/ops.py
@@ -2,6 +2,7 @@
 
 import ctypes as C
 from contextlib import contextmanager
+from typing import NamedTuple
 
 import torch
 
@@ -722,7 +723,7 @@
 def conv2d_nhwc(pc: PackedConv, srcs, dst, epilogue: int = EPI_LINEAR, aux0=None, aux1=None, dst2=None, gru_c: int = 0,
                 stride: int = 1, tile_stats=None, add_map=None, in_norm=None, src_hl: bool = False, dst_hl: bool = False,
                 dst2_hl: bool = False, dst_split=None, tile: int = 0, src_bounded: bool = False, ksplit_ws=None,
-                single_product=None):
+                single_product=None, lazy_residual=None):
     _apply_conv_env()
     d = _lib.ConvDesc()
     if len(srcs) != len(pc.seg_counts):
@@ -760,6 +761,15 @@
         if not (in_norm.is_cuda and in_norm.dtype == F32 and in_norm.is_contiguous() and tuple(in_norm.shape) == (B, srcs[0][0].shape[3], 2)):
             raise ValueError("in_norm must be a contiguous fp32 CUDA tensor of (B, C_source, 2)")
         d.src0_mean_rstd = in_norm.data_ptr()
+    if lazy_residual is not None:
+        rt, roff, rnorm, rrelu = lazy_residual
+        _nhwc(rt, "lazy residual")
+        if in_norm is None or rt.shape[:3] != (B, H, W):
+            raise ValueError("lazy_residual needs in_norm and a residual of the source's (B,H,W)")
+        if rnorm is not None and not (rnorm.is_cuda and rnorm.dtype == F32 and rnorm.is_contiguous() and tuple(rnorm.shape) == (B, rt.shape[3], 2)):
+            raise ValueError("the residual's statistics must be a contiguous fp32 CUDA tensor of (B, C_residual, 2)")
+        d.src0_residual, d.src0_residual_c_stride, d.src0_residual_c_offset = rt.data_ptr(), rt.shape[3], int(roff)
+        d.src0_residual_mean_rstd, d.src0_residual_relu = (None if rnorm is None else rnorm.data_ptr()), int(bool(rrelu))
     d.src_hl, d.dst_hl, d.dst2_hl, d.tile = int(bool(src_hl)), int(bool(dst_hl)), int(bool(dst2_hl)), int(tile)
     if tile_stats is not None:
         tpi = int(_lib.load().rnnpose_conv_tiles_per_image_desc(C.byref(d)))
@@ -780,6 +790,7 @@
     nb = B * H * W * pc.c_in_real + pc.c_out * pc.c_in_real * pc.kh * pc.kw + B * Ho * Wo * pc.c_out
     nb += B * Ho * Wo * pc.c_out * (add_map is not None) + B * Ho * Wo * (gru_c if epilogue == EPI_GRU_ZR else 0)
     nb += 2 * B * Ho * Wo * pc.c_out * (epilogue == EPI_GRU_Q) + B * Ho * Wo * pc.c_out * (dst_split is not None)
+    nb += B * H * W * pc.c_in_real * (lazy_residual is not None)
     products = 3
     if d.single_product and _prof is not None:
         products = int(_lib.load().rnnpose_conv_products_desc(C.byref(d)))
@@ -797,7 +808,8 @@
     return _single_product
 
 
-def conv_tiles_per_image(H, W, kh, kw, stride=1, c_out=None, tile: int = 0, batch: int = 1, src_counts=None, fused_norm: bool = False) -> int:
+def conv_tiles_per_image(H, W, kh, kw, stride=1, c_out=None, tile: int = 0, batch: int = 1, src_counts=None, fused_norm: bool = False,
+                         lazy_residual: bool = False) -> int:
     _apply_conv_env()
     if c_out is None:
         c_out, tile = 64, 1
@@ -809,7 +821,28 @@
     d.n_src = len(src_counts or [32])
     d.B, d.H, d.W, d.kh, d.kw, d.stride, d.c_out, d.tile = int(batch), int(H), int(W), int(kh), int(kw), int(stride), int(c_out), int(tile)
     d.src0_mean_rstd = 16 if fused_norm else None
+    d.src0_residual = 16 if lazy_residual else None
     return int(_lib.load().rnnpose_conv_tiles_per_image_desc(C.byref(d)))
+
+
+class LazyBlock(NamedTuple):
+    c2: torch.Tensor
+    mean_rstd: torch.Tensor
+    residual: torch.Tensor
+    residual_norm: object
+    residual_relu: bool
+
+
+def conv_takes_lazy_residual(pc: PackedConv, B, H, W, stride, tile: int = 0) -> bool:
+    _apply_conv_env()
+    if len(pc.seg_counts) != 1:
+        return False
+    d = _lib.ConvDesc()
+    d.src[0] = _lib.ConvSrc(None, pc.c_in, 0, pc.c_in)
+    d.n_src = 1
+    d.B, d.H, d.W, d.kh, d.kw, d.stride, d.c_out, d.tile = int(B), int(H), int(W), pc.kh, pc.kw, int(stride), pc.c_out, int(tile)
+    d.src0_mean_rstd = d.src0_residual = 16
+    return int(_lib.load().rnnpose_conv_lazy_residual_desc(C.byref(d))) == 1
 
 
 _conv_env_applied = False
@@ -869,7 +902,8 @@
     out = torch.empty(B, -(-H // stride), -(-W // stride), pc.c_out, device=x.device, dtype=F32)
     ts = None
     if stats:
-        tpi = conv_tiles_per_image(H, W, pc.kh, pc.kw, stride, pc.c_out, tile, B, src_counts=pc.seg_counts, fused_norm=in_norm is not None)
+        tpi = conv_tiles_per_image(H, W, pc.kh, pc.kw, stride, pc.c_out, tile, B, src_counts=pc.seg_counts, fused_norm=in_norm is not None,
+                                   lazy_residual=kw.get("lazy_residual") is not None)
         ts = torch.empty(B * tpi, pc.c_out, 2, device=x.device, dtype=F64)
     conv2d_nhwc(pc, [(x, 0)], (out, 0), epilogue, stride=stride, tile_stats=ts, in_norm=in_norm, tile=tile, **kw)
     return out, ts
@@ -1050,15 +1084,26 @@
         _lib.call("rnnpose_conv1x1_resident_pack_f16x3", _ptr(w), 256, self.c_in, self.w_scale, _ptr(self.w_packed), _stream())
 
 
-def conv1x1_resident(pc: PackedConv1x1, src, dst, relu: bool = True, dst_split: bool = False):
+def conv1x1_resident(pc: PackedConv1x1, src, dst, relu: bool = True, dst_split: bool = False, in_norm=None, lazy_residual=None):
     x, xo = src
     y, yo = dst
     _nhwc(x, "src"); _nhwc(y, "dst")
     n = x.shape[0] * x.shape[1] * x.shape[2]
     if y.shape[:3] != x.shape[:3]:
         raise ValueError("src and dst must share (B,h,w)")
+    lz = None
+    if (in_norm is None) != (lazy_residual is None):
+        raise ValueError("in_norm and lazy_residual come together")
+    if lazy_residual is not None:
+        rt, roff, rnorm, rrelu = lazy_residual
+        _nhwc(rt, "lazy residual")
+        ok = lambda t, c: t.is_cuda and t.dtype == F32 and t.is_contiguous() and tuple(t.shape) == (x.shape[0], c, 2)
+        if rt.shape[:3] != x.shape[:3] or not ok(in_norm, x.shape[3]) or (rnorm is not None and not ok(rnorm, rt.shape[3])):
+            raise ValueError("lazy residual: a residual of src's (B,h,w), statistics of (B, C, 2) each")
+        lz = C.byref(_lib.LazyResidual(in_norm.data_ptr(), rt.data_ptr(), rt.shape[3], int(roff), None if rnorm is None else rnorm.data_ptr(),
+                                       int(bool(rrelu)), x.shape[1] * x.shape[2]))
     _launch("rnnpose_conv1x1_resident_f16x3", _ptr(x), x.shape[3], int(xo), pc.c_in, _ptr(pc.w_packed), _ptr(pc.bias), pc.a_scale,
-            pc.w_scale, int(bool(relu)), n, _ptr(y), y.shape[3], int(yo), int(bool(dst_split)), _stream(), work=2.0 * n * 256 * pc.c_in)
+            pc.w_scale, int(bool(relu)), n, _ptr(y), y.shape[3], int(yo), int(bool(dst_split)), lz, _stream(), work=2.0 * n * 256 * pc.c_in)
 
 
 def corr_lookup_convc1(pc: PackedConv1x1, pyramid_buf, coords, dst, B_total, b0, b1, levels=4, radius=4, relu: bool = True,
```

Result: no change. 771.0 (median of 6 runs) (+0.7%).
